# OPPOMKLab/u-LLaVA

Hardware: AMD Instinct MI355X
Metric: images/sec/GPU (ViT-L-336 + LLaMA-7B + SAM RES forward) at 1/2/4/8 MI355X (higher is better)
Workload: dtype bf16; 1 GPU; C4: ViT-L/14-336 + LLaMA-7B instruct forward, 336x336 image + 64-token prompt (S=643), batch 32/GPU; per_gpu_batch=32, global_batch=32, seq_len=643, image=336, parallelism=dp1, weights=random-init N(0,0.02), ViT-L/14 + LLaMA-7B (V=32011) shapes

## Files before the change

include/ullava_hip.h:

```cpp
#ifndef ULLAVA_HIP_H
#define ULLAVA_HIP_H
#include <stdint.h>
#ifdef __cplusplus
extern "C" {
#endif

#define ULL_DT_F32 0
#define ULL_DT_BF16 1
#define ULL_DT_F16 2

#define ULL_OK 0
#define ULL_ERR_ARG (-1)
#define ULL_ERR_SHAPE (-2)
#define ULL_ERR_LAUNCH (-3)
#define ULL_ERR_LDS (-4)

#define ULL_EPI_BIAS 1
#define ULL_EPI_ACT_QUICK_GELU (1 << 1)
#define ULL_EPI_ACT_GELU (2 << 1)
#define ULL_EPI_ACT_RELU (3 << 1)
#define ULL_EPI_RESID 8
#define ULL_EPI_SWIGLU 16
#define ULL_EPI_OUT_F32 32
#define ULL_EPI_W_TILED 64
#define ULL_EPI_X_TILED 128
#define ULL_EPI_BIAS_ROUNDED 256

#define ULL_GEMM_TUNE_GROUP_M(g) (((g) & 15) << 16)
#define ULL_GEMM_TUNE_SMALL_KERNEL (1 << 20)
#define ULL_GEMM_TUNE_WAVES8 (1 << 21)
#define ULL_GEMM_TUNE_WAVES4 (1 << 22)
#define ULL_GEMM_TUNE_STAGED_EPILOGUE 512
int ull_gemm_bf16(const void* X, int64_t ldx, const void* W, int64_t ldw, void* C, int64_t ldc, const void* bias, const void* R,
                  int64_t ldr, int64_t M, int64_t N, int64_t K, int flags, void* ws, int64_t ws_bytes, void* stream);

int ull_gemm_qkv_rope_bf16(const void* X, int64_t ldx, const void* W, int64_t ldw, void* C, int64_t ldc, int64_t M, int64_t N, int64_t K,
                           const void* rope_cos, const void* rope_sin, int64_t rope_cols, int64_t head_dim, int flags, void* ws,
                           int64_t ws_bytes, void* stream);

int ull_rope_table_bf16(const void* positions, const void* inv_freq, int64_t tokens, int64_t half, void* cos_out, void* sin_out,
                        void* stream);

int64_t ull_gemm_streamk_ws_bytes(void);

#define ULL_WF_ELEM 0
#define ULL_WF_FP8 1
#define ULL_WF_MXFP4 2

int ull_gemv_bf16(const void* X, int64_t ldx, const void* W, int64_t ldw, void* C, int64_t ldc, const void* bias, const void* R,
                  int64_t ldr, int64_t M, int64_t N, int64_t K, int flags, void* stream);

int ull_gemm_skinny_bf16(const void* X, int64_t ldx, const void* W, int64_t ldw, void* C, int64_t ldc, const void* bias, const void* R,
                         int64_t ldr, int64_t M, int64_t N, int64_t K, int flags, void* stream);

int ull_gemv_rmsnorm_bf16(const void* X, int64_t ldx, const void* norm_w, float eps, const void* W, int64_t ldw, void* C, int64_t ldc,
                          const void* bias, const void* R, int64_t ldr, int64_t M, int64_t N, int64_t K, int flags, void* stream);

int ull_gemv_qkv_rope_append_bf16(const void* X, int64_t ldx, const void* norm_w, float eps, const void* W, int64_t ldw, void* Q_out, int64_t ldq,
                                  const void* cos_tab, const void* sin_tab, void* k_cache, void* vt_cache, int64_t B, int64_t S, int64_t H,
                                  int64_t hd, int64_t K, int64_t smax, int64_t past, void* stream);

int ull_quantize_rows_fp8_bf16(const void* W, int64_t ldw, int64_t N, int64_t K, void* codes, void* scales, void* stream);
int ull_dequantize_rows_fp8_bf16(const void* codes, int64_t ldq, const void* scales, int64_t N, int64_t K, void* out, int tiled, void* stream);

int ull_quantize_rows_mxfp4_bf16(const void* W, int64_t ldw, int64_t N, int64_t K, void* codes, int64_t ldq, void* scales, int64_t lds, int resident,
                                 void* stream);
int ull_dequantize_rows_mxfp4_bf16(const void* codes, int64_t ldq, const void* scales, int64_t lds, int64_t N, int64_t K, void* out, int tiled,
                                   int resident, void* stream);

int ull_gemv_wq_bf16(const void* X, int64_t ldx, int wfmt, const void* Q, int64_t ldq, const void* scales, int64_t lds, void* C, int64_t ldc,
                     const void* bias, const void* R, int64_t ldr, int64_t M, int64_t N, int64_t K, int flags, void* stream);
int ull_gemm_skinny_wq_bf16(const void* X, int64_t ldx, int wfmt, const void* Q, int64_t ldq, const void* scales, int64_t lds, void* C, int64_t ldc,
                            const void* bias, const void* R, int64_t ldr, int64_t M, int64_t N, int64_t K, int flags, void* stream);
int ull_gemv_rmsnorm_wq_bf16(const void* X, int64_t ldx, const void* norm_w, float eps, int wfmt, const void* Q, int64_t ldq, const void* scales,
                             int64_t lds, void* C, int64_t ldc, const void* bias, const void* R, int64_t ldr, int64_t M, int64_t N, int64_t K,
                             int flags, void* stream);
int ull_gemv_qkv_rope_append_wq_bf16(const void* X, int64_t ldx, const void* norm_w, float eps, int wfmt, const void* Q, int64_t ldq,
                                     const void* scales, int64_t lds, void* Q_out, int64_t ldq_out, const void* cos_tab, const void* sin_tab,
                                     void* k_cache, void* vt_cache, int64_t B, int64_t S, int64_t H, int64_t hd, int64_t K, int64_t smax, int64_t past,
                                     void* stream);

int ull_gemm_a8w8_bf16(const void* Xq, int64_t ldxq, const void* x_scales, const void* Q, int64_t ldq, const void* w_scales, void* C, int64_t ldc,
                       const void* R, int64_t ldr, int64_t M, int64_t N, int64_t K, int flags, void* stream);

int ull_attention_kv8_bf16(const void* Q, int64_t q_bs, int64_t q_hs, int64_t q_ss, const void* k_stage, const void* vt_stage, const void* k8,
                           const void* vt8, const void* k_scale, const void* vt_scale, int64_t smax, void* O, int64_t o_bs, int64_t o_hs, int64_t o_ss,
                           const void* key_mask, int64_t B, int64_t H, int64_t Sq, int64_t Sk, int64_t hd, float scale, const void* zeros, void* stream);
int ull_kv8_quantize_bf16(const void* K, int64_t k_bs, int64_t k_hs, int64_t k_ss, const void* V, int64_t v_bs, int64_t v_hs, int64_t v_ss, int v_image,
                          int64_t src_p0, void* k8, void* vt8, void* k_scale, void* vt_scale, int64_t B, int64_t H, int64_t hd, int64_t smax, int64_t p0,
                          int64_t n, void* stream);
int ull_kv8_dequantize_bf16(const void* k8, const void* vt8, const void* k_scale, const void* vt_scale, int64_t B, int64_t H, int64_t hd, int64_t smax,
                            int64_t n, void* K_out, int64_t k_pitch, void* Vt_out, int64_t vt_pitch, void* stream);

int ull_rmsnorm_bf16(const void* x, int64_t ldx, const void* w, void* y, int64_t ldy, int64_t rows, int64_t D, float eps, void* stream);

int ull_shifted_cross_entropy_bf16(const void* logits, int64_t ld, const void* labels, int64_t B, int64_t S, int64_t V, void* out,
                                   void* stream);

int ull_layernorm_bf16(const void* x, int64_t ldx, const void* w, const void* b, void* y, int64_t ldy, int64_t rows, int64_t D, float eps,
                       void* stream);

int ull_clip_embed_ln_bf16(const void* patch, int64_t ldp, const void* cls, const void* pos, const void* w, const void* b, void* y,
                           int64_t ldy, int64_t n_img, int64_t tokens, int64_t D, float eps, void* stream);

int ull_attention_bf16(const void* Q, int64_t q_bs, int64_t q_hs, int64_t q_ss, const void* K, int64_t k_bs, int64_t k_hs, int64_t k_ss,
                       const void* Vt, int64_t vt_bs, int64_t vt_hs, int64_t vt_ds, int64_t vt_len, void* O, int64_t o_bs, int64_t o_hs,
                       int64_t o_ss, const void* key_mask, int64_t B, int64_t H, int64_t Sq, int64_t Sk, int64_t hd, int causal,
                       int scale_mode, float scale, float q_scale, const void* rel_h, const void* rel_w, int64_t rel_kh,
                       int64_t rel_kw, int rel_mode, const void* zeros, void* stream);

int ull_rope_inplace_bf16(void* x, int64_t row_stride, const void* positions, const void* inv_freq, int64_t tokens, int64_t n_heads,
                          int64_t hd, void* stream);

int ull_rope_append_bf16(void* qkv, int64_t row_stride, const void* positions, const void* inv_freq, int64_t B, int64_t S, int64_t H,
                         int64_t hd, void* k_cache, void* vt_cache, int64_t smax, int64_t past, void* stream);

int ull_transpose_v_bf16(const void* v, int64_t v_bs, int64_t v_ss, void* vt, int64_t B, int64_t S, int64_t H, int64_t hd, int64_t pitch,
                         void* stream);

int ull_im2col_bf16(const void* img, void* out, int64_t n_img, int64_t C, int64_t H, int64_t W, int64_t ps, int64_t Kp, void* stream);

int ull_mm_spans(const void* ids, int64_t B, int64_t S, int64_t img_start, int64_t img_end, int64_t vid_start, int64_t vid_end,
                 int64_t vocab, void* spans, void* stream);

int ull_greedy_step_bf16(const void* logits, int64_t row_stride, int64_t B, int64_t V, void* unfinished, const void* eos, int64_t n_eos,
                         int64_t pad, int has_pad, void* seq, int64_t seq_ld, int64_t pos, void* alive, void* stream);

#define ULL_SAMPLE_MAX_V 36608
int ull_sample_step(const void* logits, int logits_dtype, int64_t row_stride, int64_t B, int64_t V, const void* noise, float temperature,
                    int64_t top_k, float top_p, void* unfinished, const void* eos, int64_t n_eos, int64_t pad, int has_pad, void* seq,
                    int64_t seq_ld, int64_t pos, void* alive, void* stream);

int ull_embed_splice_bf16(const void* ids, const void* table, const void* img_feat, int64_t n_img_tok, int64_t img_pitch,
                          int64_t img_off, const void* vid_feat, int64_t n_vid_tok, const void* spans, void* out, int64_t B, int64_t S,
                          int64_t D, int64_t vocab, void* stream);

int ull_video_pool_bf16(const void* f, void* out, int64_t B, int64_t T, int64_t N, int64_t D, int64_t tok_pitch, int64_t tok_off,
                        void* stream);

int ull_gather_rows_bf16(const void* src, int64_t lds, const void* idx, void* dst, int64_t ldd, int64_t n, int64_t D, void* stream);

int ull_dropout_apply_bf16(const void* x, const void* keep, void* y, int64_t n, float scale, void* stream);

int ull_add_rows_bf16(const void* a, const void* b, void* out, int64_t rows, int64_t D, int64_t b_rows, void* stream);


int ull_window_partition_bf16(const void* x, void* out, int64_t B, int64_t H, int64_t W, int64_t C, int64_t ws, void* stream);

int ull_window_unpartition_add_bf16(const void* win, const void* shortcut, void* out, int64_t B, int64_t H, int64_t W, int64_t C, int64_t ws,
                                    void* stream);

int ull_sam_relpos_bf16(const void* q, int64_t q_bs, int64_t q_hs, int64_t q_ss, const void* rel_pos_h, const void* rel_pos_w, void* out_h,
                        void* out_w, int64_t NB, int64_t nH, int64_t KH, int64_t KW, int64_t hd, void* stream);

int ull_sam_window_attention_bf16(const void* qkv, int64_t ld, const void* pad_row, const void* rel_pos_h, const void* rel_pos_w, void* out,
                                  int64_t ldo, int64_t B, int64_t H, int64_t W, int64_t nH, int64_t hd, int64_t ws, float q_scale,
                                  const void* zeros, void* stream);

int ull_interp_rows_linear_bf16(const void* x, void* y, int64_t L, int64_t M, int64_t C, void* stream);

int ull_layernorm2d_cl_bf16(const void* x, const void* w, const void* b, void* y, int64_t rows, int64_t C, float eps, int gelu, void* stream);

int ull_neck_layernorm2d_f32in_f16(const void* xa, const void* xb, float xb_scale, const void* w, const void* b, void* y_hi, void* y_lo,
                                   int64_t rows, int64_t C, float eps, void* stream);

int ull_im2col3x3_bf16(const void* x, void* out, int64_t B, int64_t H, int64_t W, int64_t C, void* stream);

int ull_mask_matmul_bf16(const void* hyper, const void* up, void* masks, int64_t n, int64_t T, int64_t C, int64_t G, void* stream);

int ull_bilinear_f32(const void* in, int in_dtype, int64_t in_img_stride, int64_t in_row_stride, int64_t in_h, int64_t in_w, void* out,
                     int64_t n, int64_t out_h, int64_t out_w, void* stream);

int ull_patchify_bf16(const void* img, int64_t n_img, int64_t C, int64_t H, int64_t W, int64_t ps, const void* Wp, int64_t Kp,
                      const void* bias, void* out, int64_t ldc, int64_t N, const void* zeros, void* stream);


int ull_resample_u8(const void* src, int64_t H, int64_t W, int64_t C, int axis, int64_t out_size, const void* bounds, const void* coeffs,
                    int64_t ksize, void* dst, void* stream);

int ull_u8_lut_chw(const void* src, int64_t H, int64_t W, int64_t C, int64_t top, int64_t left, const void* lut, void* dst, int64_t OH,
                   int64_t OW, int64_t copy_h, int64_t copy_w, int out_dtype, void* stream);

int ull_mask_iou_counts(const void* logits, const void* target, int64_t n_masks, int64_t hw, int ignore_index, void* counts, void* stream);


int ull_mask_loss_sums_f32(const void* logits, const void* target, int64_t n_masks, int64_t hw, float scale, void* part, void* stream);

int ull_box_losses_f32(const void* pred, int pred_dtype, const void* gt, int64_t n, void* out, void* stream);


int ull_sam_self_attn_heads_bf16(const void* queries, const void* qpe, int64_t n, int64_t T, int first, const void* wq, const void* bq,
                                 const void* wk, const void* bk, const void* wv, const void* bv, void* att, void* stream);

int ull_sam_out_ln_bf16(const void* att, int64_t din, const void* res, const void* qpe, int64_t n, int64_t T, const void* wo, const void* bo,
                        const void* ln_w, const void* ln_b, float eps, void* out, const void* const* projs, const int* add_pe, void* stream);

int ull_sam_token_mlp_ln_bf16(const void* queries, const void* qpe, int64_t n, int64_t T, int64_t hidden, const void* w1, const void* b1,
                              const void* w2, const void* b2, const void* ln_w, const void* ln_b, float eps, void* part_ws, void* out,
                              const void* const* projs, const int* add_pe, void* stream);

int ull_sam_small_mlps_bf16(const void* hs, int64_t n, int64_t T, const void* const* ptrs, int64_t n_mask_tokens, int64_t hyper_out,
                            int64_t n_iou, void* hyper, void* iou, void* stream);

int ull_sam_t2i_attention_bf16(const void* qproj, const void* keys, const void* pos, int64_t n, int64_t T, int64_t P, const void* wk,
                               const void* bk, const void* wv, const void* bv, int late_bias_kv, void* scores_ws, void* vproj_ws, void* att,
                               void* stream);

int ull_sam_i2t_attention_ln_bf16(const void* keys, const void* pos, const void* kproj, const void* vproj, int64_t n, int64_t T, int64_t P,
                                  const void* wq, const void* bq, const void* wo, const void* bo, int late_bias_q, const void* ln_w,
                                  const void* ln_b, float eps, void* out, void* stream);


int ull_rmsnorm_bwd_bf16(const void* x, int64_t ldx, const void* w, const void* dy, int64_t lddy, void* dx, int64_t lddx, void* dw,
                         int64_t rows, int64_t D, float eps, void* stream);

int ull_swiglu_fwd_bf16(const void* gu, void* a, int64_t M, int64_t I, int halves, void* stream);
int ull_swiglu_bwd_bf16(const void* gu, const void* da, void* dgu, int64_t M, int64_t I, int halves, void* stream);

int ull_relu_mask_bf16(const void* y, const void* dy, void* dx, int64_t n, void* stream);

int ull_rope_bwd_inplace_bf16(void* dx, int64_t row_stride, const void* positions, const void* inv_freq, int64_t tokens, int64_t n_heads,
                              int64_t hd, void* stream);

int ull_attention_bwd_bf16(const void* Q, const void* K, const void* V, const void* O, const void* dO, void* dQ, void* dK, void* dV,
                           const int64_t* strides, const void* key_mask, int64_t B, int64_t H, int64_t Sq, int64_t Sk, int64_t hd, int causal,
                           float mult, void* scratch, void* stream);

int ull_attention_bwd_mfma_bf16(const void* Q, const void* K, const void* V, const void* O, const void* dO, const void* Qt, const void* Kt,
                                const void* dOt, int64_t pitch, void* dQ, void* dK, void* dV, const int64_t* strides, const void* key_mask,
                                int64_t B, int64_t H, int64_t Sq, int64_t Sk, int64_t hd, int causal, float mult, void* scratch, void* stream);

int ull_shifted_cross_entropy_bwd_bf16(const void* logits, int64_t ld, const void* labels, int64_t B, int64_t S, int64_t V, const void* stats,
                                       const void* gout, void* dlogits, void* stream);

int ull_embed_splice_bwd_bf16(const void* ids, const void* demb, void* d_table, void* d_img, int64_t n_img_tok, int64_t img_pitch,
                              int64_t img_off, void* d_vid, int64_t n_vid_tok, const void* spans, int64_t B, int64_t S, int64_t D, int64_t vocab,
                              int detach_text, void* stream);

int ull_layernorm_bwd_bf16(const void* x, int64_t ldx, const void* w, const void* dy, int64_t lddy, void* dx, int64_t lddx, void* dw, void* db,
                           int64_t rows, int64_t D, float eps, void* stream);

int ull_layernorm2d_cl_bwd_bf16(const void* x, const void* w, const void* b, const void* dy, void* dx, void* dw, void* db, int64_t rows,
                                int64_t C, float eps, int gelu, void* stream);

int ull_gelu_fwd_bf16(const void* x, void* y, int64_t n, void* stream);
int ull_gelu_bwd_bf16(const void* x, const void* dy, void* dx, int64_t n, void* stream);

int ull_mask_matmul_bwd_bf16(const void* hyper, const void* up, const void* dmasks, void* dhyper, void* dup, int64_t n, int64_t T, int64_t C,
                             int64_t G, void* stream);

int ull_sum_slabs_bf16(const void* x, void* out, int64_t R, int64_t n, float scale, void* stream);

int ull_colsum_bf16(const void* x, int64_t ld, int64_t rows, int64_t N, void* out, void* stream);

int ull_transpose2d_bf16(const void* x, int64_t ldx, void* y, int64_t ldy, int64_t R, int64_t C, void* stream);

int ull_mask_loss_sums_bwd_f32(const void* logits, const void* target, const void* g, int64_t n_masks, int64_t hw, float scale, void* dlogits,
                               void* stream);
int ull_box_losses_bwd_f32(const void* pred, int pred_dtype, const void* gt, int64_t n, const void* gw, void* dpred, void* stream);
int ull_bilinear_bwd_f32(const void* dout, void* din, int64_t in_img_stride, int64_t in_row_stride, int64_t in_h, int64_t in_w, int64_t n,
                         int64_t out_h, int64_t out_w, void* stream);

int ull_adamw_step_f32(void* master, void* m, void* v, const void* grad, int grad_dtype, void* param_out, int param_dtype, int64_t n, float lr,
                       float beta1, float beta2, float eps, float weight_decay, int64_t step, float grad_scale, void* stream);

int ull_sumsq_f32(const void* g, int grad_dtype, int64_t n, void* out, void* stream);

typedef struct ull_linear {
    const void* w;
    const void* w_tiled;
    const void* bias;
    int64_t n, k, ldw;
    int format;
    const void* scales;
    int64_t lds;
} ull_linear;
typedef struct ull_llama_layer {
    const void* ln1;
    const void* ln2;
    ull_linear qkv, o, gu, down;
} ull_llama_layer;
typedef struct ull_clip_layer {
    const void *ln1_w, *ln1_b, *ln2_w, *ln2_b;
    ull_linear qkv, out, fc1, fc2;
} ull_clip_layer;
typedef struct ull_sam_block {
    const void *n1_w, *n1_b, *n2_w, *n2_b;
    ull_linear qkv, proj, lin1, lin2;
    const void* rel_pos_h;
    const void* rel_pos_w;
    int64_t window;
} ull_sam_block;

int ull_llama_prefill_layers_bf16(const ull_llama_layer* layers, int64_t n_layers, const void* x_in, void* const* x_out, void* x_mid, void* xn,
                                  void* qkv, void* att, void* act, const void* rope_cos, const void* rope_sin, const void* key_mask, int64_t B,
                                  int64_t S, int64_t H, int64_t hd, int64_t I, float eps, void* ws, int64_t ws_bytes, int64_t sk_min_k,
                                  const void* zeros, void* stream);

int ull_llama_decode_layers_bf16(const ull_llama_layer* layers, int64_t n_layers, const void* x_in, void* const* x_out, void* x_mid, void* xn,
                                 void* q, void* att, void* act, const void* rope_cos, const void* rope_sin, const void* key_mask,
                                 void* const* k_cache, void* const* vt_cache, int64_t B, int64_t S, int64_t H, int64_t hd, int64_t I, int64_t smax,
                                 int64_t past, float eps, const void* zeros, void* stream);

int ull_llama_decode_layers_kv8_bf16(const ull_llama_layer* layers, int64_t n_layers, const void* x_in, void* const* x_out, void* x_mid, void* xn,
                                     void* q, void* att, void* act, const void* rope_cos, const void* rope_sin, const void* key_mask, void* const* k8,
                                     void* const* vt8, void* const* k_scale, void* const* vt_scale, void* k_stage, void* vt_stage, int64_t B, int64_t S,
                                     int64_t H, int64_t hd, int64_t I, int64_t smax, int64_t past, float eps, const void* zeros, void* stream);

int ull_clip_layers_bf16(const ull_clip_layer* layers, int64_t n_layers, void* h, void* h_mid, void* y, void* qkv, void* att, void* f, int64_t n_img,
                         int64_t S, int64_t H, int64_t hd, int64_t I, float eps, void* ws, int64_t ws_bytes, int64_t sk_min_k, const void* zeros,
                         void* stream);

int ull_sam_blocks_bf16(const ull_sam_block* blocks, int64_t n_blocks, void* x, void* x_mid, void* y, void* qkv, void* att, void* f, int64_t B,
                        int64_t g, int64_t nH, int64_t hd, int64_t I, float eps, void* ws, int64_t ws_bytes, int64_t sk_min_k, const void* zeros,
                        void* stream);

int ull_gemm_f32(const void* X, int64_t ldx, const void* W, int64_t ldw, void* C, int64_t ldc, const void* bias, const void* R, int64_t ldr, int64_t M, int64_t N, int64_t K, int flags, void* ws, int64_t ws_bytes, void* stream);
int ull_attention_f32(const void* Q, int64_t q_bs, int64_t q_hs, int64_t q_ss, const void* K, int64_t k_bs, int64_t k_hs, int64_t k_ss, const void* Vt, int64_t vt_bs, int64_t vt_hs, int64_t vt_ds, int64_t vt_len, void* O, int64_t o_bs, int64_t o_hs, int64_t o_ss, const void* key_mask, int64_t B, int64_t H, int64_t Sq, int64_t Sk, int64_t hd, int causal, int scale_mode, float scale, float q_scale, const void* rel_h, const void* rel_w, int64_t rel_kh, int64_t rel_kw, int rel_mode, const void* zeros, void* stream);
int ull_transpose_v_f32(const void* v, int64_t v_bs, int64_t v_ss, void* vt, int64_t B, int64_t S, int64_t H, int64_t hd, int64_t pitch, void* stream);
int ull_transpose2d_f32(const void* x, int64_t ldx, void* y, int64_t ldy, int64_t R, int64_t C, void* stream);
int ull_rmsnorm_f32(const void* x, int64_t ldx, const void* w, void* y, int64_t ldy, int64_t rows, int64_t D, float eps, void* stream);
int ull_layernorm_f32(const void* x, int64_t ldx, const void* w, const void* b, void* y, int64_t ldy, int64_t rows, int64_t D, float eps, void* stream);
int ull_clip_embed_ln_f32(const void* patch, int64_t ldp, const void* cls, const void* pos, const void* w, const void* b, void* y, int64_t ldy, int64_t n_img, int64_t tokens, int64_t D, float eps, void* stream);
int ull_layernorm2d_cl_f32(const void* x, const void* w, const void* b, void* y, int64_t rows, int64_t C, float eps, int gelu, void* stream);
int ull_rope_inplace_f32(void* x, int64_t row_stride, const void* positions, const void* inv_freq, int64_t tokens, int64_t n_heads, int64_t hd, void* stream);
int ull_rope_append_f32(void* qkv, int64_t row_stride, const void* positions, const void* inv_freq, int64_t B, int64_t S, int64_t H, int64_t hd, void* k_cache, void* vt_cache, int64_t smax, int64_t past, void* stream);
int ull_im2col_f32(const void* img, void* out, int64_t n_img, int64_t C, int64_t H, int64_t W, int64_t ps, int64_t Kp, void* stream);
int ull_im2col3x3_f32(const void* x, void* out, int64_t B, int64_t H, int64_t W, int64_t C, void* stream);
int ull_video_pool_f32(const void* f, void* out, int64_t B, int64_t T, int64_t N, int64_t D, int64_t tok_pitch, int64_t tok_off, void* stream);
int ull_add_rows_f32(const void* a, const void* b, void* out, int64_t rows, int64_t D, int64_t b_rows, void* stream);
int ull_window_unpartition_add_f32(const void* win, const void* shortcut, void* out, int64_t B, int64_t H, int64_t W, int64_t C, int64_t ws, void* stream);
int ull_sam_relpos_f32(const void* q, int64_t q_bs, int64_t q_hs, int64_t q_ss, const void* rel_pos_h, const void* rel_pos_w, void* out_h, void* out_w, int64_t NB, int64_t nH, int64_t KH, int64_t KW, int64_t hd, void* stream);
int ull_interp_rows_linear_f32(const void* x, void* y, int64_t L, int64_t M, int64_t C, void* stream);
int ull_mask_matmul_f32(const void* hyper, const void* up, void* masks, int64_t n, int64_t T, int64_t C, int64_t G, void* stream);
int ull_greedy_step_f32(const void* logits, int64_t row_stride, int64_t B, int64_t V, void* unfinished, const void* eos, int64_t n_eos, int64_t pad, int has_pad, void* seq, int64_t seq_ld, int64_t pos, void* alive, void* stream);
int ull_shifted_cross_entropy_f32(const void* logits, int64_t ld, const void* labels, int64_t B, int64_t S, int64_t V, void* out, void* stream);

int ull_gemm_f16(const void* X, int64_t ldx, const void* W, int64_t ldw, void* C, int64_t ldc, const void* bias, const void* R, int64_t ldr, int64_t M, int64_t N, int64_t K, int flags, void* ws, int64_t ws_bytes, void* stream);
int ull_gemm_qkv_rope_f16(const void* X, int64_t ldx, const void* W, int64_t ldw, void* C, int64_t ldc, int64_t M, int64_t N, int64_t K, const void* rope_cos, const void* rope_sin, int64_t rope_cols, int64_t head_dim, int flags, void* ws, int64_t ws_bytes, void* stream);
int ull_rope_table_f16(const void* positions, const void* inv_freq, int64_t tokens, int64_t half, void* cos_out, void* sin_out, void* stream);
int ull_gemv_f16(const void* X, int64_t ldx, const void* W, int64_t ldw, void* C, int64_t ldc, const void* bias, const void* R, int64_t ldr, int64_t M, int64_t N, int64_t K, int flags, void* stream);
int ull_gemm_skinny_f16(const void* X, int64_t ldx, const void* W, int64_t ldw, void* C, int64_t ldc, const void* bias, const void* R, int64_t ldr, int64_t M, int64_t N, int64_t K, int flags, void* stream);
int ull_gemv_rmsnorm_f16(const void* X, int64_t ldx, const void* norm_w, float eps, const void* W, int64_t ldw, void* C, int64_t ldc, const void* bias, const void* R, int64_t ldr, int64_t M, int64_t N, int64_t K, int flags, void* stream);
int ull_gemv_qkv_rope_append_f16(const void* X, int64_t ldx, const void* norm_w, float eps, const void* W, int64_t ldw, void* Q_out, int64_t ldq, const void* cos_tab, const void* sin_tab, void* k_cache, void* vt_cache, int64_t B, int64_t S, int64_t H, int64_t hd, int64_t K, int64_t smax, int64_t past, void* stream);
int ull_rmsnorm_f16(const void* x, int64_t ldx, const void* w, void* y, int64_t ldy, int64_t rows, int64_t D, float eps, void* stream);
int ull_shifted_cross_entropy_f16(const void* logits, int64_t ld, const void* labels, int64_t B, int64_t S, int64_t V, void* out, void* stream);
int ull_layernorm_f16(const void* x, int64_t ldx, const void* w, const void* b, void* y, int64_t ldy, int64_t rows, int64_t D, float eps, void* stream);
int ull_clip_embed_ln_f16(const void* patch, int64_t ldp, const void* cls, const void* pos, const void* w, const void* b, void* y, int64_t ldy, int64_t n_img, int64_t tokens, int64_t D, float eps, void* stream);
int ull_attention_f16(const void* Q, int64_t q_bs, int64_t q_hs, int64_t q_ss, const void* K, int64_t k_bs, int64_t k_hs, int64_t k_ss, const void* Vt, int64_t vt_bs, int64_t vt_hs, int64_t vt_ds, int64_t vt_len, void* O, int64_t o_bs, int64_t o_hs, int64_t o_ss, const void* key_mask, int64_t B, int64_t H, int64_t Sq, int64_t Sk, int64_t hd, int causal, int scale_mode, float scale, float q_scale, const void* rel_h, const void* rel_w, int64_t rel_kh, int64_t rel_kw, int rel_mode, const void* zeros, void* stream);
int ull_rope_inplace_f16(void* x, int64_t row_stride, const void* positions, const void* inv_freq, int64_t tokens, int64_t n_heads, int64_t hd, void* stream);
int ull_rope_append_f16(void* qkv, int64_t row_stride, const void* positions, const void* inv_freq, int64_t B, int64_t S, int64_t H, int64_t hd, void* k_cache, void* vt_cache, int64_t smax, int64_t past, void* stream);
int ull_transpose_v_f16(const void* v, int64_t v_bs, int64_t v_ss, void* vt, int64_t B, int64_t S, int64_t H, int64_t hd, int64_t pitch, void* stream);
int ull_im2col_f16(const void* img, void* out, int64_t n_img, int64_t C, int64_t H, int64_t W, int64_t ps, int64_t Kp, void* stream);
int ull_greedy_step_f16(const void* logits, int64_t row_stride, int64_t B, int64_t V, void* unfinished, const void* eos, int64_t n_eos, int64_t pad, int has_pad, void* seq, int64_t seq_ld, int64_t pos, void* alive, void* stream);
int ull_embed_splice_f16(const void* ids, const void* table, const void* img_feat, int64_t n_img_tok, int64_t img_pitch, int64_t img_off, const void* vid_feat, int64_t n_vid_tok, const void* spans, void* out, int64_t B, int64_t S, int64_t D, int64_t vocab, void* stream);
int ull_video_pool_f16(const void* f, void* out, int64_t B, int64_t T, int64_t N, int64_t D, int64_t tok_pitch, int64_t tok_off, void* stream);
int ull_gather_rows_f16(const void* src, int64_t lds, const void* idx, void* dst, int64_t ldd, int64_t n, int64_t D, void* stream);
int ull_dropout_apply_f16(const void* x, const void* keep, void* y, int64_t n, float scale, void* stream);
int ull_add_rows_f16(const void* a, const void* b, void* out, int64_t rows, int64_t D, int64_t b_rows, void* stream);
int ull_window_partition_f16(const void* x, void* out, int64_t B, int64_t H, int64_t W, int64_t C, int64_t ws, void* stream);
int ull_window_unpartition_add_f16(const void* win, const void* shortcut, void* out, int64_t B, int64_t H, int64_t W, int64_t C, int64_t ws, void* stream);
int ull_sam_relpos_f16(const void* q, int64_t q_bs, int64_t q_hs, int64_t q_ss, const void* rel_pos_h, const void* rel_pos_w, void* out_h, void* out_w, int64_t NB, int64_t nH, int64_t KH, int64_t KW, int64_t hd, void* stream);
int ull_sam_window_attention_f16(const void* qkv, int64_t ld, const void* pad_row, const void* rel_pos_h, const void* rel_pos_w, void* out, int64_t ldo, int64_t B, int64_t H, int64_t W, int64_t nH, int64_t hd, int64_t ws, float q_scale, const void* zeros, void* stream);
int ull_interp_rows_linear_f16(const void* x, void* y, int64_t L, int64_t M, int64_t C, void* stream);
int ull_layernorm2d_cl_f16(const void* x, const void* w, const void* b, void* y, int64_t rows, int64_t C, float eps, int gelu, void* stream);
int ull_im2col3x3_f16(const void* x, void* out, int64_t B, int64_t H, int64_t W, int64_t C, void* stream);
int ull_mask_matmul_f16(const void* hyper, const void* up, void* masks, int64_t n, int64_t T, int64_t C, int64_t G, void* stream);
int ull_patchify_f16(const void* img, int64_t n_img, int64_t C, int64_t H, int64_t W, int64_t ps, const void* Wp, int64_t Kp, const void* bias, void* out, int64_t ldc, int64_t N, const void* zeros, void* stream);
int ull_sam_self_attn_heads_f16(const void* queries, const void* qpe, int64_t n, int64_t T, int first, const void* wq, const void* bq, const void* wk, const void* bk, const void* wv, const void* bv, void* att, void* stream);
int ull_sam_out_ln_f16(const void* att, int64_t din, const void* res, const void* qpe, int64_t n, int64_t T, const void* wo, const void* bo, const void* ln_w, const void* ln_b, float eps, void* out, const void* const* projs, const int* add_pe, void* stream);
int ull_sam_token_mlp_ln_f16(const void* queries, const void* qpe, int64_t n, int64_t T, int64_t hidden, const void* w1, const void* b1, const void* w2, const void* b2, const void* ln_w, const void* ln_b, float eps, void* part_ws, void* out, const void* const* projs, const int* add_pe, void* stream);
int ull_sam_small_mlps_f16(const void* hs, int64_t n, int64_t T, const void* const* ptrs, int64_t n_mask_tokens, int64_t hyper_out, int64_t n_iou, void* hyper, void* iou, void* stream);
int ull_sam_t2i_attention_f16(const void* qproj, const void* keys, const void* pos, int64_t n, int64_t T, int64_t P, const void* wk, const void* bk, const void* wv, const void* bv, int late_bias_kv, void* scores_ws, void* vproj_ws, void* att, void* stream);
int ull_sam_i2t_attention_ln_f16(const void* keys, const void* pos, const void* kproj, const void* vproj, int64_t n, int64_t T, int64_t P, const void* wq, const void* bq, const void* wo, const void* bo, int late_bias_q, const void* ln_w, const void* ln_b, float eps, void* out, void* stream);
int ull_rmsnorm_bwd_f16(const void* x, int64_t ldx, const void* w, const void* dy, int64_t lddy, void* dx, int64_t lddx, void* dw, int64_t rows, int64_t D, float eps, void* stream);
int ull_swiglu_fwd_f16(const void* gu, void* a, int64_t M, int64_t I, int halves, void* stream);
int ull_swiglu_bwd_f16(const void* gu, const void* da, void* dgu, int64_t M, int64_t I, int halves, void* stream);
int ull_relu_mask_f16(const void* y, const void* dy, void* dx, int64_t n, void* stream);
int ull_rope_bwd_inplace_f16(void* dx, int64_t row_stride, const void* positions, const void* inv_freq, int64_t tokens, int64_t n_heads, int64_t hd, void* stream);
int ull_attention_bwd_f16(const void* Q, const void* K, const void* V, const void* O, const void* dO, void* dQ, void* dK, void* dV, const int64_t* strides, const void* key_mask, int64_t B, int64_t H, int64_t Sq, int64_t Sk, int64_t hd, int causal, float mult, void* scratch, void* stream);
int ull_attention_bwd_mfma_f16(const void* Q, const void* K, const void* V, const void* O, const void* dO, const void* Qt, const void* Kt, const void* dOt, int64_t pitch, void* dQ, void* dK, void* dV, const int64_t* strides, const void* key_mask, int64_t B, int64_t H, int64_t Sq, int64_t Sk, int64_t hd, int causal, float mult, void* scratch, void* stream);
int ull_shifted_cross_entropy_bwd_f16(const void* logits, int64_t ld, const void* labels, int64_t B, int64_t S, int64_t V, const void* stats, const void* gout, void* dlogits, void* stream);
int ull_embed_splice_bwd_f16(const void* ids, const void* demb, void* d_table, void* d_img, int64_t n_img_tok, int64_t img_pitch, int64_t img_off, void* d_vid, int64_t n_vid_tok, const void* spans, int64_t B, int64_t S, int64_t D, int64_t vocab, int detach_text, void* stream);
int ull_layernorm_bwd_f16(const void* x, int64_t ldx, const void* w, const void* dy, int64_t lddy, void* dx, int64_t lddx, void* dw, void* db, int64_t rows, int64_t D, float eps, void* stream);
int ull_layernorm2d_cl_bwd_f16(const void* x, const void* w, const void* b, const void* dy, void* dx, void* dw, void* db, int64_t rows, int64_t C, float eps, int gelu, void* stream);
int ull_gelu_fwd_f16(const void* x, void* y, int64_t n, void* stream);
int ull_gelu_bwd_f16(const void* x, const void* dy, void* dx, int64_t n, void* stream);
int ull_mask_matmul_bwd_f16(const void* hyper, const void* up, const void* dmasks, void* dhyper, void* dup, int64_t n, int64_t T, int64_t C, int64_t G, void* stream);
int ull_sum_slabs_f16(const void* x, void* out, int64_t R, int64_t n, float scale, void* stream);
int ull_colsum_f16(const void* x, int64_t ld, int64_t rows, int64_t N, void* out, void* stream);
int ull_transpose2d_f16(const void* x, int64_t ldx, void* y, int64_t ldy, int64_t R, int64_t C, void* stream);
int ull_llama_prefill_layers_f16(const ull_llama_layer* layers, int64_t n_layers, const void* x_in, void* const* x_out, void* x_mid, void* xn, void* qkv, void* att, void* act, const void* rope_cos, const void* rope_sin, const void* key_mask, int64_t B, int64_t S, int64_t H, int64_t hd, int64_t I, float eps, void* ws, int64_t ws_bytes, int64_t sk_min_k, const void* zeros, void* stream);
int ull_llama_decode_layers_f16(const ull_llama_layer* layers, int64_t n_layers, const void* x_in, void* const* x_out, void* x_mid, void* xn, void* q, void* att, void* act, const void* rope_cos, const void* rope_sin, const void* key_mask, void* const* k_cache, void* const* vt_cache, int64_t B, int64_t S, int64_t H, int64_t hd, int64_t I, int64_t smax, int64_t past, float eps, const void* zeros, void* stream);
int ull_clip_layers_f16(const ull_clip_layer* layers, int64_t n_layers, void* h, void* h_mid, void* y, void* qkv, void* att, void* f, int64_t n_img, int64_t S, int64_t H, int64_t hd, int64_t I, float eps, void* ws, int64_t ws_bytes, int64_t sk_min_k, const void* zeros, void* stream);
int ull_sam_blocks_f16(const ull_sam_block* blocks, int64_t n_blocks, void* x, void* x_mid, void* y, void* qkv, void* att, void* f, int64_t B, int64_t g, int64_t nH, int64_t hd, int64_t I, float eps, void* ws, int64_t ws_bytes, int64_t sk_min_k, const void* zeros, void* stream);

#ifdef __cplusplus
}
#endif
#endif
```

u-llava_amd/_lib.py:

```python
import ctypes
import os

_HERE = os.path.dirname(os.path.abspath(__file__))
LIB_PATH = os.environ.get("ULL_LIB_PATH", os.path.join(_HERE, "csrc", "libullava_hip.so"))

_i64, _i32, _f32, _ptr = ctypes.c_int64, ctypes.c_int, ctypes.c_float, ctypes.c_void_p


WF_ELEM, WF_FP8, WF_MXFP4 = 0, 1, 2


class Linear(ctypes.Structure):
    _fields_ = [("w", _ptr), ("w_tiled", _ptr), ("bias", _ptr), ("n", _i64), ("k", _i64), ("ldw", _i64), ("format", _i32), ("scales", _ptr), ("lds", _i64)]


class LlamaLayer(ctypes.Structure):
    _fields_ = [("ln1", _ptr), ("ln2", _ptr), ("qkv", Linear), ("o", Linear), ("gu", Linear), ("down", Linear)]


class ClipLayer(ctypes.Structure):
    _fields_ = [("ln1_w", _ptr), ("ln1_b", _ptr), ("ln2_w", _ptr), ("ln2_b", _ptr), ("qkv", Linear), ("out", Linear), ("fc1", Linear), ("fc2", Linear)]


class SamBlock(ctypes.Structure):
    _fields_ = [("n1_w", _ptr), ("n1_b", _ptr), ("n2_w", _ptr), ("n2_b", _ptr), ("qkv", Linear), ("proj", Linear), ("lin1", Linear), ("lin2", Linear),
                ("rel_pos_h", _ptr), ("rel_pos_w", _ptr), ("window", _i64)]


SIGNATURES = {
    "ull_gemm_bf16": [_ptr, _i64, _ptr, _i64, _ptr, _i64, _ptr, _ptr, _i64, _i64, _i64, _i64, _i32, _ptr, _i64, _ptr],
    "ull_gemm_streamk_ws_bytes": [],
    "ull_gemm_qkv_rope_bf16": [_ptr, _i64, _ptr, _i64, _ptr, _i64, _i64, _i64, _i64, _ptr, _ptr, _i64, _i64, _i32, _ptr, _i64, _ptr],
    "ull_rope_table_bf16": [_ptr, _ptr, _i64, _i64, _ptr, _ptr, _ptr],
    "ull_sam_self_attn_heads_bf16": [_ptr, _ptr, _i64, _i64, _i32] + [_ptr] * 7 + [_ptr],
    "ull_sam_out_ln_bf16": [_ptr, _i64, _ptr, _ptr, _i64, _i64, _ptr, _ptr, _ptr, _ptr, _f32, _ptr, ctypes.POINTER(_ptr), ctypes.POINTER(_i32), _ptr],
    "ull_sam_token_mlp_ln_bf16": [_ptr, _ptr, _i64, _i64, _i64] + [_ptr] * 6 + [_f32, _ptr, _ptr, ctypes.POINTER(_ptr), ctypes.POINTER(_i32), _ptr],
    "ull_sam_small_mlps_bf16": [_ptr, _i64, _i64, ctypes.POINTER(_ptr), _i64, _i64, _i64, _ptr, _ptr, _ptr],
    "ull_sam_t2i_attention_bf16": [_ptr, _ptr, _ptr, _i64, _i64, _i64, _ptr, _ptr, _ptr, _ptr, _i32, _ptr, _ptr, _ptr, _ptr],
    "ull_sam_i2t_attention_ln_bf16": [_ptr] * 4 + [_i64] * 3 + [_ptr] * 4 + [_i32, _ptr, _ptr, _f32, _ptr, _ptr],
    "ull_rmsnorm_bwd_bf16": [_ptr, _i64, _ptr, _ptr, _i64, _ptr, _i64, _ptr, _i64, _i64, _f32, _ptr],
    "ull_swiglu_fwd_bf16": [_ptr, _ptr, _i64, _i64, _i32, _ptr],
    "ull_swiglu_bwd_bf16": [_ptr, _ptr, _ptr, _i64, _i64, _i32, _ptr],
    "ull_relu_mask_bf16": [_ptr, _ptr, _ptr, _i64, _ptr],
    "ull_rope_bwd_inplace_bf16": [_ptr, _i64, _ptr, _ptr, _i64, _i64, _i64, _ptr],
    "ull_attention_bwd_bf16": [_ptr, _ptr, _ptr, _ptr, _ptr, _ptr, _ptr, _ptr, ctypes.POINTER(_i64), _ptr, _i64, _i64, _i64, _i64, _i64, _i32,
                               _f32, _ptr, _ptr],
    "ull_attention_bwd_mfma_bf16": [_ptr, _ptr, _ptr, _ptr, _ptr, _ptr, _ptr, _ptr, _i64, _ptr, _ptr, _ptr, ctypes.POINTER(_i64), _ptr, _i64, _i64,
                                    _i64, _i64, _i64, _i32, _f32, _ptr, _ptr],
    "ull_shifted_cross_entropy_bwd_bf16": [_ptr, _i64, _ptr, _i64, _i64, _i64, _ptr, _ptr, _ptr, _ptr],
    "ull_embed_splice_bwd_bf16": [_ptr, _ptr, _ptr, _ptr, _i64, _i64, _i64, _ptr, _i64, _ptr, _i64, _i64, _i64, _i64, _i32, _ptr],
    "ull_colsum_bf16": [_ptr, _i64, _i64, _i64, _ptr, _ptr],
    "ull_transpose2d_bf16": [_ptr, _i64, _ptr, _i64, _i64, _i64, _ptr],
    "ull_sum_slabs_bf16": [_ptr, _ptr, _i64, _i64, _f32, _ptr],
    "ull_layernorm_bwd_bf16": [_ptr, _i64, _ptr, _ptr, _i64, _ptr, _i64, _ptr, _ptr, _i64, _i64, _f32, _ptr],
    "ull_layernorm2d_cl_bwd_bf16": [_ptr, _ptr, _ptr, _ptr, _ptr, _ptr, _ptr, _i64, _i64, _f32, _i32, _ptr],
    "ull_gelu_fwd_bf16": [_ptr, _ptr, _i64, _ptr],
    "ull_gelu_bwd_bf16": [_ptr, _ptr, _ptr, _i64, _ptr],
    "ull_mask_matmul_bwd_bf16": [_ptr, _ptr, _ptr, _ptr, _ptr, _i64, _i64, _i64, _i64, _ptr],
    "ull_mask_loss_sums_bwd_f32": [_ptr, _ptr, _ptr, _i64, _i64, _f32, _ptr, _ptr],
    "ull_box_losses_bwd_f32": [_ptr, _i32, _ptr, _i64, _ptr, _ptr, _ptr],
    "ull_bilinear_bwd_f32": [_ptr, _ptr, _i64, _i64, _i64, _i64, _i64, _i64, _i64, _ptr],
    "ull_gemv_bf16": [_ptr, _i64, _ptr, _i64, _ptr, _i64, _ptr, _ptr, _i64, _i64, _i64, _i64, _i32, _ptr],
    "ull_dropout_apply_bf16": [_ptr, _ptr, _ptr, _i64, _f32, _ptr],
    "ull_gemm_skinny_bf16": [_ptr, _i64, _ptr, _i64, _ptr, _i64, _ptr, _ptr, _i64, _i64, _i64, _i64, _i32, _ptr],
    "ull_gemv_rmsnorm_bf16": [_ptr, _i64, _ptr, _f32, _ptr, _i64, _ptr, _i64, _ptr, _ptr, _i64, _i64, _i64, _i64, _i32, _ptr],
    "ull_gemv_qkv_rope_append_bf16": [_ptr, _i64, _ptr, _f32, _ptr, _i64, _ptr, _i64, _ptr, _ptr, _ptr, _ptr, _i64, _i64, _i64, _i64, _i64, _i64, _i64,
                                      _ptr],
    "ull_rmsnorm_bf16": [_ptr, _i64, _ptr, _ptr, _i64, _i64, _i64, _f32, _ptr],
    "ull_llama_prefill_layers_bf16": [_ptr, _i64, _ptr, _ptr, _ptr, _ptr, _ptr, _ptr, _ptr, _ptr, _ptr, _ptr, _i64, _i64, _i64, _i64, _i64, _f32, _ptr,
                                      _i64, _i64, _ptr, _ptr],
    "ull_llama_decode_layers_bf16": [_ptr, _i64, _ptr, _ptr, _ptr, _ptr, _ptr, _ptr, _ptr, _ptr, _ptr, _ptr, _ptr, _ptr, _i64, _i64, _i64, _i64, _i64,
                                     _i64, _i64, _f32, _ptr, _ptr],
    "ull_clip_layers_bf16": [_ptr, _i64, _ptr, _ptr, _ptr, _ptr, _ptr, _ptr, _i64, _i64, _i64, _i64, _i64, _f32, _ptr, _i64, _i64, _ptr, _ptr],
    "ull_sam_blocks_bf16": [_ptr, _i64, _ptr, _ptr, _ptr, _ptr, _ptr, _ptr, _i64, _i64, _i64, _i64, _i64, _f32, _ptr, _i64, _i64, _ptr, _ptr],
    "ull_shifted_cross_entropy_bf16": [_ptr, _i64, _ptr, _i64, _i64, _i64, _ptr, _ptr],
    "ull_layernorm_bf16": [_ptr, _i64, _ptr, _ptr, _ptr, _i64, _i64, _i64, _f32, _ptr],
    "ull_clip_embed_ln_bf16": [_ptr, _i64, _ptr, _ptr, _ptr, _ptr, _ptr, _i64, _i64, _i64, _i64, _f32, _ptr],
    "ull_attention_bf16": [_ptr, _i64, _i64, _i64, _ptr, _i64, _i64, _i64, _ptr, _i64, _i64, _i64, _i64, _ptr, _i64, _i64, _i64,
                           _ptr, _i64, _i64, _i64, _i64, _i64, _i32, _i32, _f32, _f32, _ptr, _ptr, _i64, _i64, _i32, _ptr, _ptr],
    "ull_rope_inplace_bf16": [_ptr, _i64, _ptr, _ptr, _i64, _i64, _i64, _ptr],
    "ull_rope_append_bf16": [_ptr, _i64, _ptr, _ptr, _i64, _i64, _i64, _i64, _ptr, _ptr, _i64, _i64, _ptr],
    "ull_transpose_v_bf16": [_ptr, _i64, _i64, _ptr, _i64, _i64, _i64, _i64, _i64, _ptr],
    "ull_sam_window_attention_bf16": [_ptr, _i64, _ptr, _ptr, _ptr, _ptr, _i64, _i64, _i64, _i64, _i64, _i64, _i64, _f32, _ptr, _ptr],
    "ull_interp_rows_linear_bf16": [_ptr, _ptr, _i64, _i64, _i64, _ptr],
    "ull_im2col_bf16": [_ptr, _ptr, _i64, _i64, _i64, _i64, _i64, _i64, _ptr],
    "ull_mm_spans": [_ptr, _i64, _i64, _i64, _i64, _i64, _i64, _i64, _ptr, _ptr],
    "ull_greedy_step_bf16": [_ptr, _i64, _i64, _i64, _ptr, _ptr, _i64, _i64, _i32, _ptr, _i64, _i64, _ptr, _ptr],
    "ull_embed_splice_bf16": [_ptr, _ptr, _ptr, _i64, _i64, _i64, _ptr, _i64, _ptr, _ptr, _i64, _i64, _i64, _i64, _ptr],
    "ull_video_pool_bf16": [_ptr, _ptr, _i64, _i64, _i64, _i64, _i64, _i64, _ptr],
    "ull_gather_rows_bf16": [_ptr, _i64, _ptr, _ptr, _i64, _i64, _i64, _ptr],
    "ull_add_rows_bf16": [_ptr, _ptr, _ptr, _i64, _i64, _i64, _ptr],
    "ull_window_partition_bf16": [_ptr, _ptr, _i64, _i64, _i64, _i64, _i64, _ptr],
    "ull_window_unpartition_add_bf16": [_ptr, _ptr, _ptr, _i64, _i64, _i64, _i64, _i64, _ptr],
    "ull_sam_relpos_bf16": [_ptr, _i64, _i64, _i64, _ptr, _ptr, _ptr, _ptr, _i64, _i64, _i64, _i64, _i64, _ptr],
    "ull_layernorm2d_cl_bf16": [_ptr, _ptr, _ptr, _ptr, _i64, _i64, _f32, _i32, _ptr],
    "ull_im2col3x3_bf16": [_ptr, _ptr, _i64, _i64, _i64, _i64, _ptr],
    "ull_mask_matmul_bf16": [_ptr, _ptr, _ptr, _i64, _i64, _i64, _i64, _ptr],
    "ull_bilinear_f32": [_ptr, _i32, _i64, _i64, _i64, _i64, _ptr, _i64, _i64, _i64, _ptr],
    "ull_patchify_bf16": [_ptr, _i64, _i64, _i64, _i64, _i64, _ptr, _i64, _ptr, _ptr, _i64, _i64, _ptr, _ptr],
    "ull_resample_u8": [_ptr, _i64, _i64, _i64, _i32, _i64, _ptr, _ptr, _i64, _ptr, _ptr],
    "ull_u8_lut_chw": [_ptr, _i64, _i64, _i64, _i64, _i64, _ptr, _ptr, _i64, _i64, _i64, _i64, _i32, _ptr],
    "ull_mask_iou_counts": [_ptr, _ptr, _i64, _i64, _i32, _ptr, _ptr],
    "ull_mask_loss_sums_f32": [_ptr, _ptr, _i64, _i64, _f32, _ptr, _ptr],
    "ull_box_losses_f32": [_ptr, _i32, _ptr, _i64, _ptr, _ptr],
    "ull_adamw_step_f32": [_ptr, _ptr, _ptr, _ptr, _i32, _ptr, _i32, _i64, _f32, _f32, _f32, _f32, _f32, _i64, _f32, _ptr],
    "ull_sumsq_f32": [_ptr, _i32, _i64, _ptr, _ptr],
    "ull_sample_step": [_ptr, _i32, _i64, _i64, _i64, _ptr, _f32, _i64, _f32, _ptr, _ptr, _i64, _i64, _i32, _ptr, _i64, _i64, _ptr, _ptr],
}

SIGNATURES.update({name[:-4] + "f16": args for name, args in list(SIGNATURES.items()) if name.endswith("_bf16")})

F32_TWINS = ['ull_gemm', 'ull_attention', 'ull_transpose_v', 'ull_transpose2d', 'ull_rmsnorm', 'ull_layernorm', 'ull_clip_embed_ln', 'ull_layernorm2d_cl', 'ull_rope_inplace', 'ull_rope_append', 'ull_im2col', 'ull_im2col3x3', 'ull_video_pool', 'ull_add_rows', 'ull_window_unpartition_add', 'ull_sam_relpos', 'ull_interp_rows_linear', 'ull_mask_matmul', 'ull_greedy_step', 'ull_shifted_cross_entropy']
SIGNATURES.update({name + "_f32": SIGNATURES[name + "_bf16"] for name in F32_TWINS})

SIGNATURES.update({
    "ull_quantize_rows_fp8_bf16": [_ptr, _i64, _i64, _i64, _ptr, _ptr, _ptr],
    "ull_dequantize_rows_fp8_bf16": [_ptr, _i64, _ptr, _i64, _i64, _ptr, _i32, _ptr],
    "ull_attention_kv8_bf16": [_ptr, _i64, _i64, _i64, _ptr, _ptr, _ptr, _ptr, _ptr, _ptr, _i64, _ptr, _i64, _i64, _i64, _ptr, _i64, _i64, _i64, _i64,
                               _i64, _f32, _ptr, _ptr],
    "ull_kv8_quantize_bf16": [_ptr, _i64, _i64, _i64, _ptr, _i64, _i64, _i64, _i32, _i64, _ptr, _ptr, _ptr, _ptr, _i64, _i64, _i64, _i64, _i64, _i64, _ptr],
    "ull_kv8_dequantize_bf16": [_ptr, _ptr, _ptr, _ptr, _i64, _i64, _i64, _i64, _i64, _ptr, _i64, _ptr, _i64, _ptr],
    "ull_llama_decode_layers_kv8_bf16": [_ptr, _i64] + [_ptr] * 16 + [_i64] * 7 + [_f32, _ptr, _ptr],
})

SIGNATURES.update({
    "ull_quantize_rows_mxfp4_bf16": [_ptr, _i64, _i64, _i64, _ptr, _i64, _ptr, _i64, _i32, _ptr],
    "ull_dequantize_rows_mxfp4_bf16": [_ptr, _i64, _ptr, _i64, _i64, _i64, _ptr, _i32, _i32, _ptr],
    "ull_gemv_wq_bf16": [_ptr, _i64, _i32, _ptr, _i64, _ptr, _i64, _ptr, _i64, _ptr, _ptr, _i64, _i64, _i64, _i64, _i32, _ptr],
    "ull_gemm_skinny_wq_bf16": [_ptr, _i64, _i32, _ptr, _i64, _ptr, _i64, _ptr, _i64, _ptr, _ptr, _i64, _i64, _i64, _i64, _i32, _ptr],
    "ull_gemv_rmsnorm_wq_bf16": [_ptr, _i64, _ptr, _f32, _i32, _ptr, _i64, _ptr, _i64, _ptr, _i64, _ptr, _ptr, _i64, _i64, _i64, _i64, _i32, _ptr],
    "ull_gemv_qkv_rope_append_wq_bf16": [_ptr, _i64, _ptr, _f32, _i32, _ptr, _i64, _ptr, _i64, _ptr, _i64, _ptr, _ptr, _ptr, _ptr, _i64, _i64, _i64, _i64,
                                         _i64, _i64, _i64, _ptr],
})

SIGNATURES["ull_gemm_a8w8_bf16"] = [_ptr, _i64, _ptr, _ptr, _i64, _ptr, _ptr, _i64, _ptr, _i64, _i64, _i64, _i64, _i32, _ptr]

SIGNATURES["ull_neck_layernorm2d_f32in_f16"] = [_ptr, _ptr, _f32, _ptr, _ptr, _ptr, _ptr, _i64, _i64, _f32, _ptr]

VALUE_RETURNING = {"ull_gemm_streamk_ws_bytes": _i64}

ERRORS = {-1: "ULL_ERR_ARG (null pointer / bad size)", -2: "ULL_ERR_SHAPE (alignment or shape constraint)",
          -3: "ULL_ERR_LAUNCH (HIP launch failed)", -4: "ULL_ERR_LDS (does not fit the LDS budget)"}

_lib = None


def load():
    global _lib
    if _lib is not None:
        return _lib
    if not os.path.exists(LIB_PATH):
        raise RuntimeError(
            f"u-llava_amd: HIP library not built: {LIB_PATH} is missing. Run `python -c 'import __graft_entry__ as g; g.build()'` "
            "or `make -C u-llava_amd/csrc`. There is no CPU fallback.")
    lib = ctypes.CDLL(LIB_PATH)
    for name, argtypes in SIGNATURES.items():
        fn = getattr(lib, name)
        fn.argtypes = argtypes
        fn.restype = VALUE_RETURNING.get(name, ctypes.c_int)
    _lib = lib
    return lib


def call(name: str, *args):
    fn = getattr(load(), name, None)
    if fn is None or name not in SIGNATURES:
        raise RuntimeError(f"u-llava_amd: the library has no entry point `{name}` (no kernel build of this op for that element type)")
    rc = fn(*args)
    if rc != 0:
        raise RuntimeError(f"u-llava_amd: {name} failed: {ERRORS.get(rc, rc)}")


def query(name: str, *args):
    fn = getattr(load(), name, None)
    if fn is None or name not in SIGNATURES:
        raise RuntimeError(f"u-llava_amd: the library has no entry point `{name}` (no kernel build of this op for that element type)")
    return fn(*args)
```

u-llava_amd/csrc/f32.hip:

```cpp
#include "ull_common.h"

#define ULL_EPI_BIAS 1
#define ULL_EPI_ACT_MASK (3 << 1)
#define ULL_EPI_ACT_QUICK_GELU (1 << 1)
#define ULL_EPI_ACT_GELU (2 << 1)
#define ULL_EPI_ACT_RELU (3 << 1)
#define ULL_EPI_RESID 8
#define ULL_EPI_SWIGLU 16
#define ULL_EPI_W_TILED 64
#define ULL_EPI_X_TILED 128

namespace {

ULL_DEV float gelu_erf32(float x) { return 0.5f * x * (1.0f + erff(x * 0.70710678118654752440f)); }
ULL_DEV float sigmoid32(float x) { return 1.0f / (1.0f + expf(-x)); }
static inline unsigned grid_for(long n, long cap = 65535) { const long b = (n + 255) / 256; return (unsigned)(b < 1 ? 1 : (b < cap ? b : cap)); }

__global__ __launch_bounds__(256) void gemm_f32_kernel(const float* __restrict__ X, long ldx, const float* __restrict__ W, long ldw, float* __restrict__ C,
                                                       long ldc, const float* __restrict__ bias, const float* __restrict__ R, long ldr, int M, int N,
                                                       int K, int flags) {
    __shared__ float Xs[64][17], Ws[64][17];
    const int tid = threadIdx.x, lane = tid & 63, wave = tid >> 6;
    const long m0 = (long)blockIdx.y * 64, n0 = (long)blockIdx.x * 64;
    const int lr = tid >> 2, lk = (tid & 3) * 4;
    f32x4_t acc[4];
#pragma unroll
    for (int j = 0; j < 4; ++j) acc[j] = f32x4_t{0.f, 0.f, 0.f, 0.f};
    for (int k0 = 0; k0 < K; k0 += 16) {
#pragma unroll
        for (int j = 0; j < 4; ++j) {
            const int k = k0 + lk + j;
            Xs[lr][lk + j] = (m0 + lr < M && k < K) ? X[(m0 + lr) * ldx + k] : 0.f;
            Ws[lr][lk + j] = (n0 + lr < N && k < K) ? W[(n0 + lr) * ldw + k] : 0.f;
        }
        __syncthreads();
#pragma unroll
        for (int kk = 0; kk < 4; ++kk) {
            const float a = Xs[wave * 16 + (lane & 15)][kk * 4 + (lane >> 4)];
#pragma unroll
            for (int j = 0; j < 4; ++j) acc[j] = __builtin_amdgcn_mfma_f32_16x16x4f32(a, Ws[j * 16 + (lane & 15)][kk * 4 + (lane >> 4)], acc[j], 0, 0, 0);
        }
        __syncthreads();
    }
    const int act = flags & ULL_EPI_ACT_MASK;
    if (flags & ULL_EPI_SWIGLU) {
#pragma unroll
        for (int pr = 0; pr < 2; ++pr) {
            const long oc = (n0 / 32 + pr) * 16 + (lane & 15);
            if (n0 + pr * 32 + 16 + (lane & 15) >= N) continue;
#pragma unroll
            for (int i = 0; i < 4; ++i) {
                const long m = m0 + wave * 16 + 4 * (lane >> 4) + i;
                if (m >= M) continue;
                const float g = acc[2 * pr][i], u = acc[2 * pr + 1][i];
                float v = (g * sigmoid32(g)) * u;
                if (R) v = R[m * ldr + oc] + v;
                C[m * ldc + oc] = v;
            }
        }
        return;
    }
#pragma unroll
    for (int j = 0; j < 4; ++j) {
        const long n = n0 + j * 16 + (lane & 15);
        if (n >= N) continue;
        const float bv = (flags & ULL_EPI_BIAS) ? bias[n] : 0.f;
#pragma unroll
        for (int i = 0; i < 4; ++i) {
            const long m = m0 + wave * 16 + 4 * (lane >> 4) + i;
            if (m >= M) continue;
            float v = acc[j][i] + bv;
            if (act == ULL_EPI_ACT_QUICK_GELU) v = v * sigmoid32(1.702f * v);
            else if (act == ULL_EPI_ACT_GELU) v = gelu_erf32(v);
            else if (act == ULL_EPI_ACT_RELU) v = fmaxf(v, 0.f);
            if (flags & ULL_EPI_RESID) v = R[m * ldr + n] + v;
            C[m * ldc + n] = v;
        }
    }
}

struct AttnF32 {
    const float *Q, *K, *V;
    float* O;
    const int32_t* key_mask;
    const float *rel_h, *rel_w;
    long q_bs, q_hs, q_ss, k_bs, k_hs, k_ss, v_bs, v_hs, v_ds, v_len, o_bs, o_hs, o_ss;
    int B, H, Sq, Sk, hd, causal, scale_mode, KH, KW;
    float scale, q_scale;
};

ULL_DEV long vt_slot(long key) {
    const int w = (int)(key & 31);
    return (key & ~31L) + 8 * ((w >> 2) & 3) + 4 * (w >> 4) + (w & 3);
}

__global__ __launch_bounds__(256) void attn_f32_kernel(AttnF32 p) {
    constexpr int HDP = 128;
    __shared__ float Qs[16][HDP + 1], KVs[64][HDP + 1], Ss[16][65], alpha[16], rowm[16], rowl[16];
    const int tid = threadIdx.x, lane = tid & 63, wave = tid >> 6;
    const int q0 = blockIdx.x * 16;
    const int b = blockIdx.y / p.H, h = blockIdx.y % p.H;
    const int hd = p.hd, hd4 = (hd + 3) / 4, ndb = (hd + 15) / 16;
    const int koff = p.Sk - p.Sq;
    const float* qb = p.Q + (long)b * p.q_bs + (long)h * p.q_hs;
    const float* kb = p.K + (long)b * p.k_bs + (long)h * p.k_hs;
    const float* vb = p.V + (long)b * p.v_bs + (long)h * p.v_hs;
    for (int i = tid; i < 16 * HDP; i += 256) {
        const int r = i / HDP, d = i % HDP;
        const int q = min(q0 + r, p.Sq - 1);
        Qs[r][d] = d < hd ? qb[(long)q * p.q_ss + d] * p.q_scale : 0.f;
    }
    if (tid < 16) { rowm[tid] = -INFINITY; rowl[tid] = 0.f; }
    f32x4_t acc[2] = {f32x4_t{0.f, 0.f, 0.f, 0.f}, f32x4_t{0.f, 0.f, 0.f, 0.f}};
    int kend = p.Sk;
    if (p.causal) kend = max(1, min(p.Sk, q0 + 16 + koff));
    __syncthreads();
    for (int k0 = 0; k0 < kend; k0 += 64) {
        for (int i = tid; i < 64 * HDP; i += 256) {
            const int r = i / HDP, d = i % HDP;
            KVs[r][d] = (k0 + r < p.Sk && d < hd) ? kb[(long)(k0 + r) * p.k_ss + d] : 0.f;
        }
        __syncthreads();
        {
            f32x4_t s = {0.f, 0.f, 0.f, 0.f};
            for (int k4 = 0; k4 < hd4; ++k4)
                s = __builtin_amdgcn_mfma_f32_16x16x4f32(Qs[lane & 15][k4 * 4 + (lane >> 4)], KVs[wave * 16 + (lane & 15)][k4 * 4 + (lane >> 4)], s, 0, 0, 0);
            const int kl = wave * 16 + (lane & 15), key = k0 + kl;
#pragma unroll
            for (int i = 0; i < 4; ++i) {
                const int r = 4 * (lane >> 4) + i, q = min(q0 + r, p.Sq - 1);
                float v = s[i];
                if (p.scale_mode == 1) v *= p.scale;
                else if (p.scale_mode == 2) v /= p.scale;
                if (key >= p.Sk) v = -INFINITY;
                else {
                    if (p.rel_h) {
                        const long row = ((long)b * p.H + h) * p.Sq + q;
                        v = (v + p.rel_h[row * p.KH + key / p.KW]) + p.rel_w[row * p.KW + key % p.KW];
                    }
                    if ((p.causal && key > q + koff) || (p.key_mask && p.key_mask[(long)b * p.Sk + key] == 0)) v = -3.4028234663852886e38f;
                }
                Ss[r][kl] = v;
            }
        }
        __syncthreads();
        {
            const int r = tid >> 4, c = tid & 15;
            const float s0 = Ss[r][c], s1 = Ss[r][c + 16], s2 = Ss[r][c + 32], s3 = Ss[r][c + 48];
            const float mo = rowm[r];
            const float mn = fmaxf(mo, group_max(fmaxf(fmaxf(s0, s1), fmaxf(s2, s3)), 16));
            const float e0 = expf(s0 - mn), e1 = expf(s1 - mn), e2 = expf(s2 - mn), e3 = expf(s3 - mn);
            Ss[r][c] = e0; Ss[r][c + 16] = e1; Ss[r][c + 32] = e2; Ss[r][c + 48] = e3;
            const float sum = group_sum((e0 + e1) + (e2 + e3), 16);
            if (c == 0) {
                const float al = expf(mo - mn);
                alpha[r] = al;
                rowm[r] = mn;
                rowl[r] = rowl[r] * al + sum;
            }
        }
        for (int i = tid; i < 64 * HDP; i += 256) {
            const int r = i / HDP, d = i % HDP;
            float v = 0.f;
// ... 187 lines not shown
}

__global__ __launch_bounds__(256) void add_rows_f32_kernel(const float* __restrict__ a, const float* __restrict__ b, float* __restrict__ out, long rows,
                                                           int D, long b_rows) {
    const long total = rows * D;
    for (long i = (long)blockIdx.x * 256 + threadIdx.x; i < total; i += (long)gridDim.x * 256) out[i] = a[i] + b[((i / D) % b_rows) * D + i % D];
}

__global__ __launch_bounds__(256) void window_unpartition_add_f32_kernel(const float* __restrict__ win, const float* __restrict__ shortcut,
                                                                         float* __restrict__ out, int H, int W, int C, int ws, int nWh, int nWw, long total) {
    for (long i = (long)blockIdx.x * 256 + threadIdx.x; i < total; i += (long)gridDim.x * 256) {
        const int c = (int)(i % C);
        const long row = i / C;
        const int xx = (int)(row % W), y = (int)((row / W) % H);
        const long b = row / ((long)W * H);
        const long wrow = ((b * nWh + y / ws) * nWw + xx / ws) * (long)(ws * ws) + (y % ws) * ws + xx % ws;
        out[i] = shortcut[i] + win[wrow * C + c];
    }
}

__global__ __launch_bounds__(128) void relpos_f32_kernel(const float* __restrict__ q, long q_bs, long q_hs, long q_ss, const float* __restrict__ rph,
                                                         const float* __restrict__ rpw, float* __restrict__ out_h, float* __restrict__ out_w, int nH, int KH,
                                                         int KW, int hd) {
    __shared__ float qs[256];
    const int S = KH * KW;
    const long blk = blockIdx.x;
    const int s = (int)(blk % S);
    const long bh = blk / S;
    const float* qp = q + (bh / nH) * q_bs + (bh % nH) * q_hs + (long)s * q_ss;
    for (int c = threadIdx.x; c < hd; c += 128) qs[c] = qp[c];
    __syncthreads();
    const int qy = s / KW, qx = s % KW;
    for (int t = threadIdx.x; t < KH + KW; t += 128) {
        const float* r = (t < KH) ? rph + (long)(qy - t + KH - 1) * hd : rpw + (long)(qx - (t - KH) + KW - 1) * hd;
        float acc = 0.f;
        for (int c = 0; c < hd; ++c) acc += qs[c] * r[c];
        if (t < KH) out_h[(bh * S + s) * KH + t] = acc;
        else out_w[(bh * S + s) * KW + (t - KH)] = acc;
    }
}

__global__ __launch_bounds__(256) void interp_rows_f32_kernel(const float* __restrict__ x, float* __restrict__ y, int L, int M, int C) {
    const long i = (long)blockIdx.x * 256 + threadIdx.x;
    if (i >= (long)M * C) return;
    const int m = (int)(i / C), c = (int)(i % C);
    float src = __fsub_rn(__fmul_rn((float)L / (float)M, (float)m + 0.5f), 0.5f);
    if (src < 0.f) src = 0.f;
    const int i0 = min((int)src, L - 1), i1 = min(i0 + 1, L - 1);
    const float l1 = __fsub_rn(src, (float)i0), l0 = __fsub_rn(1.0f, l1);
    y[i] = __fadd_rn(__fmul_rn(l0, x[(long)i0 * C + c]), __fmul_rn(l1, x[(long)i1 * C + c]));
}

__global__ __launch_bounds__(256) void mask_matmul_f32_kernel(const float* __restrict__ hyper, const float* __restrict__ up, float* __restrict__ masks, int T,
                                                              int Cc, int G, long total) {
    for (long i = (long)blockIdx.x * 256 + threadIdx.x; i < total; i += (long)gridDim.x * 256) {
        const int d2 = (int)(i & 3), d1 = (int)((i >> 2) & 3);
        const long cell = i >> 4;
        const int xx = (int)(cell % G), y = (int)((cell / G) % G);
        const long n = cell / ((long)G * G);
        const float* u = up + i * Cc;
        const int Y = 4 * y + 2 * (d1 >> 1) + (d2 >> 1), X = 4 * xx + 2 * (d1 & 1) + (d2 & 1);
        const int HW = 4 * G;
        for (int t = 0; t < T; ++t) {
            const float* hp = hyper + (n * T + t) * Cc;
            float acc = 0.f;
            for (int c = 0; c < Cc; ++c) acc += hp[c] * u[c];
            masks[((n * T + t) * HW + Y) * (long)HW + X] = acc;
        }
    }
}

__global__ __launch_bounds__(1024) void greedy_step_f32_kernel(const float* __restrict__ logits, long row_stride, int V, int32_t* __restrict__ unfinished,
                                                               const int64_t* __restrict__ eos, int n_eos, long pad, int has_pad, int64_t* __restrict__ seq,
                                                               long seq_ld, int pos, int32_t* __restrict__ alive) {
    __shared__ float bv[16];
    __shared__ int bi[16];
    const int b = blockIdx.x;
    const float* row = logits + (long)b * row_stride;
    float best = -INFINITY;
    int idx = 0x7fffffff;
    for (int c = threadIdx.x; c < V; c += 1024) {
        const float v = row[c];
        if (v > best || (v == best && c < idx)) { best = v; idx = c; }
    }
    if (idx == 0x7fffffff) idx = threadIdx.x < V ? threadIdx.x : 0;
#pragma unroll
    for (int o = 32; o > 0; o >>= 1) {
        const float ov = __shfl_xor(best, o, 64);
        const int oi = __shfl_xor(idx, o, 64);
        if (ov > best || (ov == best && oi < idx)) { best = ov; idx = oi; }
    }
    if ((threadIdx.x & 63) == 0) { bv[threadIdx.x >> 6] = best; bi[threadIdx.x >> 6] = idx; }
    __syncthreads();
    if (threadIdx.x == 0) {
        for (int w = 1; w < 16; ++w)
            if (bv[w] > best || (bv[w] == best && bi[w] < idx)) { best = bv[w]; idx = bi[w]; }
        const int live = unfinished[b];
        long tok = idx;
        if (!live && has_pad) tok = pad;
        seq[(long)b * seq_ld + pos] = tok;
        int still = live;
        if (live)
            for (int e = 0; e < n_eos; ++e)
                if (eos[e] == tok) still = 0;
        unfinished[b] = still;
        if (still) atomicAdd(alive, 1);
    }
}

__global__ __launch_bounds__(256) void shifted_ce_f32_kernel(const float* __restrict__ logits, long ld, const int64_t* __restrict__ labels, int B, int S, int V,
                                                             float* __restrict__ out) {
    const int lane = threadIdx.x & 63;
    const long row = (long)blockIdx.x * 4 + (threadIdx.x >> 6);
    if (row >= (long)B * (S - 1)) return;
    const int b = (int)(row / (S - 1)), t = (int)(row % (S - 1));
    const int64_t lab = labels[(long)b * S + t + 1];
    if (lab < 0 || lab >= V) return;
    const float* lp = logits + ((long)b * S + t) * ld;
    float m = -INFINITY;
    for (int i = lane; i < V; i += 64) m = fmaxf(m, lp[i]);
    m = wave_max(m);
    float s = 0.f;
    for (int i = lane; i < V; i += 64) s += expf(lp[i] - m);
    s = wave_sum(s);
    if (lane == 0) {
        atomicAdd(out, m + logf(s) - lp[lab]);
        atomicAdd(out + 1, 1.0f);
    }
}

__global__ __launch_bounds__(256) void transpose2d_f32_kernel(const float* __restrict__ x, long ldx, float* __restrict__ y, long ldy, int R, int C) {
    __shared__ float t[64][65];
    const int r0 = blockIdx.y * 64, c0 = blockIdx.x * 64;
    for (int i = threadIdx.x; i < 64 * 64; i += 256) {
        const int r = i >> 6, c = i & 63;
        if (r0 + r < R && c0 + c < C) t[c][r] = x[(long)(r0 + r) * ldx + c0 + c];
    }
    __syncthreads();
    for (int i = threadIdx.x; i < 64 * 64; i += 256) {
        const int c = i >> 6, r = i & 63;
        if (r0 + r < R && c0 + c < C) y[(long)(c0 + c) * ldy + r0 + r] = t[c][r];
    }
}

}

#define ST ((hipStream_t)stream)

extern "C" int ull_gemm_f32(const void* X, int64_t ldx, const void* W, int64_t ldw, void* C, int64_t ldc, const void* bias, const void* R, int64_t ldr,
                            int64_t M, int64_t N, int64_t K, int flags, void* ws, int64_t ws_bytes, void* stream) {
    (void)ws; (void)ws_bytes;
    if (!X || !W || !C || M <= 0 || N <= 0 || K <= 0) return ULL_ERR_ARG;
    if (((flags & ULL_EPI_BIAS) && !bias) || ((flags & ULL_EPI_RESID) && !R)) return ULL_ERR_ARG;
    if (flags & (ULL_EPI_W_TILED | ULL_EPI_X_TILED)) return ULL_ERR_SHAPE;
    if ((flags & ULL_EPI_SWIGLU) && (N % 32)) return ULL_ERR_SHAPE;
    hipLaunchKernelGGL(gemm_f32_kernel, dim3((unsigned)((N + 63) / 64), (unsigned)((M + 63) / 64)), dim3(256), 0, ST, (const float*)X, (long)ldx,
                       (const float*)W, (long)ldw, (float*)C, (long)ldc, (const float*)bias, (flags & ULL_EPI_RESID) ? (const float*)R : nullptr, (long)ldr,
                       (int)M, (int)N, (int)K, flags);
    return ull_check_launch();
}

extern "C" int ull_attention_f32(const void* Q, int64_t q_bs, int64_t q_hs, int64_t q_ss, const void* K, int64_t k_bs, int64_t k_hs, int64_t k_ss,
                                 const void* Vt, int64_t vt_bs, int64_t vt_hs, int64_t vt_ds, int64_t vt_len, void* O, int64_t o_bs, int64_t o_hs,
                                 int64_t o_ss, const void* key_mask, int64_t B, int64_t H, int64_t Sq, int64_t Sk, int64_t hd, int causal, int scale_mode,
                                 float scale, float q_scale, const void* rel_h, const void* rel_w, int64_t rel_kh, int64_t rel_kw, int rel_mode,
                                 const void* zeros, void* stream) {
    (void)zeros;
    if (!Q || !K || !Vt || !O || B <= 0 || H <= 0 || Sq <= 0 || Sk <= 0 || hd <= 0) return ULL_ERR_ARG;
    if (hd > 128 || (rel_h && rel_mode != 1) || (rel_h && (!rel_w || rel_kh * rel_kw != Sk))) return ULL_ERR_SHAPE;
    AttnF32 p;
    p.Q = (const float*)Q; p.K = (const float*)K; p.V = (const float*)Vt; p.O = (float*)O;
    p.key_mask = (const int32_t*)key_mask;
    p.rel_h = (const float*)rel_h; p.rel_w = (const float*)rel_w;
    p.q_bs = q_bs; p.q_hs = q_hs; p.q_ss = q_ss; p.k_bs = k_bs; p.k_hs = k_hs; p.k_ss = k_ss;
    p.v_bs = vt_bs; p.v_hs = vt_hs; p.v_ds = vt_ds; p.v_len = vt_len; p.o_bs = o_bs; p.o_hs = o_hs; p.o_ss = o_ss;
    p.B = (int)B; p.H = (int)H; p.Sq = (int)Sq; p.Sk = (int)Sk; p.hd = (int)hd; p.causal = causal; p.scale_mode = scale_mode;
    p.KH = (int)rel_kh; p.KW = (int)(rel_kw > 0 ? rel_kw : 1);
    p.scale = scale; p.q_scale = q_scale;
    hipLaunchKernelGGL(attn_f32_kernel, dim3((unsigned)((Sq + 15) / 16), (unsigned)(B * H)), dim3(256), 0, ST, p);
    return ull_check_launch();
}

extern "C" int ull_transpose_v_f32(const void* v, int64_t v_bs, int64_t v_ss, void* vt, int64_t B, int64_t S, int64_t H, int64_t hd, int64_t pitch,
                                   void* stream) {
    if (!v || !vt || B <= 0 || S <= 0 || H <= 0 || hd <= 0) return ULL_ERR_ARG;
    if (pitch % 64 || pitch < S) return ULL_ERR_SHAPE;
    const long total = B * H * hd * pitch;
    hipLaunchKernelGGL(transpose_v_f32_kernel, dim3(grid_for(total)), dim3(256), 0, ST, (const float*)v, (long)v_bs, (long)v_ss, (float*)vt, (int)S, (int)H,
                       (int)hd, (int)pitch, total);
    return ull_check_launch();
}

extern "C" int ull_transpose2d_f32(const void* x, int64_t ldx, void* y, int64_t ldy, int64_t R, int64_t C, void* stream) {
    if (!x || !y || R <= 0 || C <= 0 || ldx < C || ldy < R) return ULL_ERR_ARG;
    if (R > 65535 * 64 || C > (1 << 30)) return ULL_ERR_SHAPE;
    hipLaunchKernelGGL(transpose2d_f32_kernel, dim3((unsigned)((C + 63) / 64), (unsigned)((R + 63) / 64)), dim3(256), 0, ST, (const float*)x, (long)ldx,
                       (float*)y, (long)ldy, (int)R, (int)C);
    return ull_check_launch();
}

extern "C" int ull_rmsnorm_f32(const void* x, int64_t ldx, const void* w, void* y, int64_t ldy, int64_t rows, int64_t D, float eps, void* stream) {
    if (!x || !w || !y || rows <= 0 || D <= 0) return ULL_ERR_ARG;
    hipLaunchKernelGGL((rownorm_f32_kernel<0>), dim3((unsigned)((rows + 3) / 4)), dim3(256), 0, ST, (const float*)x, (long)ldx, (const float*)w, nullptr,
                       (float*)y, (long)ldy, (long)rows, (int)D, eps, nullptr, nullptr, 0);
    return ull_check_launch();
}

extern "C" int ull_layernorm_f32(const void* x, int64_t ldx, const void* w, const void* b, void* y, int64_t ldy, int64_t rows, int64_t D, float eps,
                                 void* stream) {
    if (!x || !w || !b || !y || rows <= 0 || D <= 0) return ULL_ERR_ARG;
    hipLaunchKernelGGL((rownorm_f32_kernel<1>), dim3((unsigned)((rows + 3) / 4)), dim3(256), 0, ST, (const float*)x, (long)ldx, (const float*)w,
                       (const float*)b, (float*)y, (long)ldy, (long)rows, (int)D, eps, nullptr, nullptr, 0);
    return ull_check_launch();
}

extern "C" int ull_clip_embed_ln_f32(const void* patch, int64_t ldp, const void* cls, const void* pos, const void* w, const void* b, void* y, int64_t ldy,
                                     int64_t n_img, int64_t tokens, int64_t D, float eps, void* stream) {
    if (!patch || !cls || !pos || !w || !b || !y || tokens < 2 || n_img <= 0) return ULL_ERR_ARG;
    const long rows = n_img * tokens;
    hipLaunchKernelGGL((rownorm_f32_kernel<1>), dim3((unsigned)((rows + 3) / 4)), dim3(256), 0, ST, (const float*)patch, (long)ldp, (const float*)w,
                       (const float*)b, (float*)y, (long)ldy, rows, (int)D, eps, (const float*)cls, (const float*)pos, (int)tokens);
    return ull_check_launch();
}

extern "C" int ull_layernorm2d_cl_f32(const void* x, const void* w, const void* b, void* y, int64_t rows, int64_t C, float eps, int gelu, void* stream) {
    if (!x || !w || !b || !y || rows <= 0 || C <= 0) return ULL_ERR_ARG;
    hipLaunchKernelGGL(layernorm2d_f32_kernel, dim3((unsigned)((rows + 3) / 4)), dim3(256), 0, ST, (const float*)x, (const float*)w, (const float*)b,
                       (float*)y, (long)rows, (int)C, eps, gelu);
    return ull_check_launch();
}

extern "C" int ull_rope_inplace_f32(void* x, int64_t row_stride, const void* positions, const void* inv_freq, int64_t tokens, int64_t n_heads, int64_t hd,
                                    void* stream) {
    if (!x || !positions || !inv_freq || tokens <= 0 || n_heads <= 0) return ULL_ERR_ARG;
    if (hd & 1) return ULL_ERR_SHAPE;
    hipLaunchKernelGGL(rope_inplace_f32_kernel, dim3((unsigned)tokens), dim3(256), 0, ST, (float*)x, (long)row_stride, (const int64_t*)positions,
                       (const float*)inv_freq, (int)n_heads, (int)hd);
    return ull_check_launch();
}

extern "C" int ull_rope_append_f32(void* qkv, int64_t row_stride, const void* positions, const void* inv_freq, int64_t B, int64_t S, int64_t H, int64_t hd,
                                   void* k_cache, void* vt_cache, int64_t smax, int64_t past, void* stream) {
    if (!qkv || !positions || !inv_freq || !k_cache || !vt_cache || B <= 0 || S <= 0 || H <= 0) return ULL_ERR_ARG;
    if ((hd & 1) || past + S > smax) return ULL_ERR_SHAPE;
    hipLaunchKernelGGL(rope_append_f32_kernel, dim3((unsigned)(B * S), (unsigned)H), dim3(128), 0, ST, (float*)qkv, (long)row_stride,
                       (const int64_t*)positions, (const float*)inv_freq, (int)S, (int)H, (int)hd, (float*)k_cache, (float*)vt_cache, (int)smax, (int)past);
    return ull_check_launch();
}

extern "C" int ull_im2col_f32(const void* img, void* out, int64_t n_img, int64_t C, int64_t H, int64_t W, int64_t ps, int64_t Kp, void* stream) {
    if (!img || !out || n_img <= 0 || ps <= 0) return ULL_ERR_ARG;
    if (H % ps || W % ps || Kp < C * ps * ps) return ULL_ERR_SHAPE;
    const int gh = (int)(H / ps), gw = (int)(W / ps);
    const long total = n_img * gh * gw * Kp;
    hipLaunchKernelGGL(im2col_f32_kernel, dim3(grid_for(total)), dim3(256), 0, ST, (const float*)img, (float*)out, (int)C, (int)H, (int)W, (int)ps, gh, gw,
                       (int)Kp, total);
    return ull_check_launch();
}

extern "C" int ull_im2col3x3_f32(const void* x, void* out, int64_t B, int64_t H, int64_t W, int64_t C, void* stream) {
    if (!x || !out || B <= 0 || H <= 0 || W <= 0 || C <= 0) return ULL_ERR_ARG;
    const long total = B * H * W * 9 * C;
    hipLaunchKernelGGL(im2col3x3_f32_kernel, dim3(grid_for(total)), dim3(256), 0, ST, (const float*)x, (float*)out, (int)H, (int)W, (int)C, total);
    return ull_check_launch();
}

extern "C" int ull_video_pool_f32(const void* f, void* out, int64_t B, int64_t T, int64_t N, int64_t D, int64_t tok_pitch, int64_t tok_off, void* stream) {
    if (!f || !out || B <= 0 || T <= 0 || N <= 0 || D <= 0) return ULL_ERR_ARG;
    hipLaunchKernelGGL(video_pool_f32_kernel, dim3((unsigned)(T + N), (unsigned)B), dim3(256), 0, ST, (const float*)f, (float*)out, (int)T, (int)N, (int)D,
                       (int)tok_pitch, (int)tok_off);
    return ull_check_launch();
}

extern "C" int ull_add_rows_f32(const void* a, const void* b, void* out, int64_t rows, int64_t D, int64_t b_rows, void* stream) {
    if (!a || !b || !out || rows <= 0 || D <= 0 || b_rows <= 0) return ULL_ERR_ARG;
    hipLaunchKernelGGL(add_rows_f32_kernel, dim3(grid_for(rows * D)), dim3(256), 0, ST, (const float*)a, (const float*)b, (float*)out, (long)rows, (int)D,
                       (long)b_rows);
    return ull_check_launch();
}

extern "C" int ull_window_unpartition_add_f32(const void* win, const void* shortcut, void* out, int64_t B, int64_t H, int64_t W, int64_t C, int64_t ws,
                                              void* stream) {
    if (!win || !shortcut || !out || B <= 0 || ws <= 0) return ULL_ERR_ARG;
    const int nWh = (int)((H + ws - 1) / ws), nWw = (int)((W + ws - 1) / ws);
    const long total = B * H * W * C;
    hipLaunchKernelGGL(window_unpartition_add_f32_kernel, dim3(grid_for(total)), dim3(256), 0, ST, (const float*)win, (const float*)shortcut, (float*)out,
                       (int)H, (int)W, (int)C, (int)ws, nWh, nWw, total);
    return ull_check_launch();
}

extern "C" int ull_sam_relpos_f32(const void* q, int64_t q_bs, int64_t q_hs, int64_t q_ss, const void* rel_pos_h, const void* rel_pos_w, void* out_h,
                                  void* out_w, int64_t NB, int64_t nH, int64_t KH, int64_t KW, int64_t hd, void* stream) {
    if (!q || !rel_pos_h || !rel_pos_w || !out_h || !out_w || NB <= 0) return ULL_ERR_ARG;
    if (hd > 256) return ULL_ERR_SHAPE;
    hipLaunchKernelGGL(relpos_f32_kernel, dim3((unsigned)(NB * nH * KH * KW)), dim3(128), 0, ST, (const float*)q, (long)q_bs, (long)q_hs, (long)q_ss,
                       (const float*)rel_pos_h, (const float*)rel_pos_w, (float*)out_h, (float*)out_w, (int)nH, (int)KH, (int)KW, (int)hd);
    return ull_check_launch();
}

extern "C" int ull_interp_rows_linear_f32(const void* x, void* y, int64_t L, int64_t M, int64_t C, void* stream) {
    if (!x || !y || L <= 0 || M <= 0 || C <= 0) return ULL_ERR_ARG;
    hipLaunchKernelGGL(interp_rows_f32_kernel, dim3((unsigned)((M * C + 255) / 256)), dim3(256), 0, ST, (const float*)x, (float*)y, (int)L, (int)M, (int)C);
    return ull_check_launch();
}

extern "C" int ull_mask_matmul_f32(const void* hyper, const void* up, void* masks, int64_t n, int64_t T, int64_t C, int64_t G, void* stream) {
    if (!hyper || !up || !masks || n <= 0 || T <= 0 || C <= 0 || G <= 0) return ULL_ERR_ARG;
// ... 22 lines not shown
```

u-llava_amd/csrc/gemm.hip:

```cpp
#include "ull_common.h"
#include <stdlib.h>
#include <type_traits>

namespace {

constexpr int BM = 128, BN = 128, BK = 64;
constexpr int TILE_BYTES = BM * BK * 2;
constexpr int BUF_BYTES = 2 * TILE_BYTES;
constexpr int GEMM_LDS = 2 * BUF_BYTES;
constexpr int GROUP_M = 8;

constexpr int EPI_BIAS = 1, EPI_ACT_SHIFT = 1, EPI_ACT_MASK = 3 << 1;
constexpr int EPI_RESID = 8, EPI_SWIGLU = 16, EPI_OUT_F32 = 32;
constexpr int EPI_W_TILED = 64, EPI_X_TILED = 128;
constexpr int EPI_BIAS_ROUNDED = 256;
constexpr int ULL_W4_FORCE_STAGED = 512;

struct GemmArgs {
    const elem_t* X; const elem_t* W; void* C;
    const elem_t* bias; const elem_t* R;
    long ldx, ldw, ldc, ldr;
    int M, N, K, flags;
    int nbm, nbn;
    int t_full, sk;
    float* ws;
    int group_m;
    const elem_t* rope_cos; const elem_t* rope_sin;
    int rope_cols;
};

ULL_DEV void glds16(const void* gsrc, uint32_t lds_byte_addr ) {
    uint32_t keep;
    asm volatile("s_mov_b32 %0, m0\n\ts_mov_b32 m0, %2\n\ts_nop 0\n\tglobal_load_lds_dwordx4 %1, off\n\ts_mov_b32 m0, %0"
                 : "=&s"(keep) : "v"(gsrc), "s"(lds_byte_addr) : "memory");
}

ULL_DEV void glds16s(const void* sbase , uint32_t voff, uint32_t lds_byte_addr ) {
    uint32_t keep;
    asm volatile("s_mov_b32 %0, m0\n\ts_mov_b32 m0, %3\n\ts_nop 0\n\tglobal_load_lds_dwordx4 %1, %2\n\ts_mov_b32 m0, %0"
                 : "=&s"(keep) : "v"(voff), "s"(sbase), "s"(lds_byte_addr) : "memory");
}

struct EpiCtx {
    const GemmArgs& p;
    int act, n_out;
    bool out_f32, has_res, bias_late, c_al, r_al;
};
ULL_DEV EpiCtx epi_ctx(const GemmArgs& p, bool swiglu) {
    const int flags = p.flags;
    const bool out_f32 = flags & EPI_OUT_F32;
    return EpiCtx{p, (flags & EPI_ACT_MASK) >> EPI_ACT_SHIFT, swiglu ? p.N / 2 : p.N, out_f32, (flags & EPI_RESID) != 0,
                  !swiglu && (flags & EPI_BIAS) && (flags & EPI_BIAS_ROUNDED), out_f32 ? (p.ldc & 3) == 0 : (p.ldc & 7) == 0, (p.ldr & 7) == 0};
}
ULL_DEV void big_finish8(const EpiCtx& c, float (&a)[8], int m, int n, bool has_pre = false, uint4 res_pre = uint4{0, 0, 0, 0}) {
        if (c.bias_late) {
#pragma unroll
            for (int e = 0; e < 8; ++e)
                if (n + e < c.n_out) a[e] = rnd(a[e] + e2f(c.p.bias[n + e]));
        }
        if (c.act == 1) {
#pragma unroll
            for (int e = 0; e < 8; ++e) a[e] = act_quick_gelu_e(a[e]);
        } else if (c.act == 2) {
#pragma unroll
            for (int e = 0; e < 8; e += 2) {
                const f32x2_t r = act_gelu_erf2(f32x2_t{a[e], a[e + 1]});
                a[e] = rnd(r.x); a[e + 1] = rnd(r.y);
            }
        } else if (c.act == 3) {
#pragma unroll
            for (int e = 0; e < 8; ++e) a[e] = fmaxf(a[e], 0.f);
        }
        const bool full = n + 8 <= c.n_out;
        if (c.has_res) {
            const elem_t* rp = c.p.R + (long)m * c.p.ldr + n;
            if (full && c.r_al) {
                float b[8];
                unpack8(has_pre ? res_pre : *(const uint4*)rp, b);
#pragma unroll
                for (int e = 0; e < 8; ++e) a[e] = rnd(b[e] + a[e]);
            } else {
#pragma unroll
                for (int e = 0; e < 8; ++e)
                    if (n + e < c.n_out) a[e] = rnd(e2f(rp[e]) + a[e]);
            }
        }
        if (c.out_f32) {
            float* cp = (float*)c.p.C + (long)m * c.p.ldc + n;
            if (full && c.c_al) {
                *(float4*)cp = make_float4(a[0], a[1], a[2], a[3]);
                *(float4*)(cp + 4) = make_float4(a[4], a[5], a[6], a[7]);
            } else {
#pragma unroll
                for (int e = 0; e < 8; ++e)
                    if (n + e < c.n_out) cp[e] = a[e];
            }
        } else {
            elem_t* cp = (elem_t*)c.p.C + (long)m * c.p.ldc + n;
            if (full && c.c_al) {
                *(uint4*)cp = pack8(a);
            } else if (full) {
                const uint4 pk = pack8(a);
                if ((((long)m * c.p.ldc + n) & 1) == 0) {
                    uint32_t* c4 = (uint32_t*)cp;
                    c4[0] = pk.x; c4[1] = pk.y; c4[2] = pk.z; c4[3] = pk.w;
                } else {
                    cp[0] = (elem_t)(pk.x & 0xffff);
                    uint32_t* c4 = (uint32_t*)(cp + 1);
                    c4[0] = (pk.x >> 16) | (pk.y << 16);
                    c4[1] = (pk.y >> 16) | (pk.z << 16);
                    c4[2] = (pk.z >> 16) | (pk.w << 16);
                    cp[7] = (elem_t)(pk.w >> 16);
                }
            } else {
#pragma unroll
                for (int e = 0; e < 8; ++e)
                    if (n + e < c.n_out) cp[e] = f2e(a[e]);
            }
        }
    }

template <bool SWIGLU, int JT, bool ROPE = false, int PHASE = 0, bool RAW1 = false, int UNR = 2, bool SW2 = false, int PERM = 0>
ULL_DEV void staged_epilogue(const GemmArgs& p, f32x4_t (&acc)[4][JT], char* reg, int lane, int mrow0, int nw0, const char* reg_partner = nullptr,
                             int sw_half = 0) {
    constexpr int ROWS = JT * 16;
    const int fr = lane & 15, fg = lane >> 4;
    const int flags = p.flags;
    const int act = (flags & EPI_ACT_MASK) >> EPI_ACT_SHIFT;
    const bool out_f32 = flags & EPI_OUT_F32;
    const bool has_res = flags & EPI_RESID;
    const int n_out = SWIGLU ? p.N / 2 : p.N;
    const bool bias_late = !SWIGLU && (flags & EPI_BIAS) && (flags & EPI_BIAS_ROUNDED);
    const bool raw_f32 = (PHASE == 0 || RAW1) && !SWIGLU && out_f32 && !act && !has_res && !bias_late;
    const bool c_al = out_f32 ? (p.ldc & 3) == 0 : (p.ldc & 7) == 0;
    const bool r_al = (p.ldr & 7) == 0;
    const int ncol0 = SWIGLU ? nw0 / 2 : nw0;

    const EpiCtx ectx = epi_ctx(p, SWIGLU);
    auto finish8 = [&](float (&a)[8], int m, int n) { big_finish8(ectx, a, m, n); };
    auto col_of = [&](int i) { return PERM ? 32 * (i >> 1) + 8 * fg + 4 * (i & 1) : i * 16 + fg * 4; };
    float bias_v[4][4];
#pragma unroll
    for (int i = 0; i < 4; ++i)
#pragma unroll
        for (int r = 0; r < 4; ++r) {
            const int n = nw0 + col_of(i) + r;
            bias_v[i][r] = (!SWIGLU && (flags & EPI_BIAS) && !bias_late && n < p.N) ? e2f(p.bias[n]) : -0.0f;
        }

    if (!raw_f32) {
        constexpr int WCOLS = (SWIGLU && !SW2) ? 32 : 64;
        constexpr int PITCH = WCOLS * 2 + 16;
        if constexpr (PHASE != 2) {
        auto park_all = [&](auto with_bias) {
        constexpr bool WB = decltype(with_bias)::value;
#pragma clang loop unroll(full)
        for (int j = 0; j < JT; ++j) {
            if constexpr (SWIGLU) {
#pragma clang loop unroll(full)
                for (int ip = 0; ip < 2; ++ip) {
                    float v[4];
#pragma unroll
                    for (int r = 0; r < 4; ++r) {
                        const float g = rnd(acc[2 * ip][j][r]);
                        const float u = rnd(acc[2 * ip + 1][j][r]);
                        v[r] = rnd(act_silu(g)) * u;
                    }
// ... 534 lines not shown
        const int r = (wave * 4 + i) * 8 + srow;
        xsrc[i] = x_tiled ? p.X + (((long)bm * nk_total) * BM + r) * BK + schunk * 8
                          : p.X + (long)min(m0 + r, p.M - 1) * p.ldx + schunk * 8;
        wsrc[i] = w_tiled ? p.W + (((long)bn * nk_total) * BN + r) * BK + schunk * 8
                          : p.W + (long)min(n0 + r, p.N - 1) * p.ldw + schunk * 8;
    }
    const long xstep = x_tiled ? BM * BK : BK, wstep = w_tiled ? BN * BK : BK;
    const uint32_t lds_base = __builtin_amdgcn_readfirstlane((uint32_t)(uintptr_t)(__attribute__((address_space(3))) char*)smem);
    const uint32_t piece_off = wave * 4 * 1024;
    auto stage = [&](int kt) {
        const uint32_t bx = lds_base + (kt & 1) * SLOT_BYTES + piece_off;
        const long kox = (long)kt * xstep, kow = (long)kt * wstep;
#pragma unroll
        for (int i = 0; i < 4; ++i) {
            glds16(xsrc[i] + kox, bx + i * 1024);
            glds16(wsrc[i] + kow, bx + OP_BYTES + i * 1024);
        }
    };

    const int fr = lane & 15, fg = lane >> 4;
    int swz[2];
    swz[0] = ((0 + fg) ^ (lane & 7)) << 4;
    swz[1] = ((4 + fg) ^ (lane & 7)) << 4;
    const int xoff = (wm * 128 + fr) * (BK * 2);
    const int woff = OP_BYTES + (wn * 64 + fr) * (BK * 2);
    auto read_frags = [&](int kt, int kk, Frags& f) {
        const char* base = smem + (kt & 1) * SLOT_BYTES + swz[kk];
#pragma unroll
        for (int i = 0; i < 4; ++i) f.w[i] = *(const uint4*)(base + woff + i * 16 * (BK * 2));
#pragma unroll
        for (int j = 0; j < 8; ++j) f.x[j] = *(const uint4*)(base + xoff + j * 16 * (BK * 2));
    };

    f32x4_t acc[4][8];
#pragma unroll
    for (int i = 0; i < 4; ++i)
#pragma unroll
        for (int j = 0; j < 8; ++j) acc[i][j] = f32x4_t{0.f, 0.f, 0.f, 0.f};
    int nk = p.K / BK;
    if (split) {
        const int kt0 = (int)((long)nk * slice / p.sk), kt1 = (int)((long)nk * (slice + 1) / p.sk);
#pragma unroll
        for (int i = 0; i < 4; ++i) { xsrc[i] += (long)kt0 * xstep; wsrc[i] += (long)kt0 * wstep; }
        nk = kt1 - kt0;
    }
constexpr int ULL_W8_BAR_A = 14;
constexpr int ULL_W8_DMA_STRIDE = 6;
constexpr int ULL_W8_BAR_B = 40;
constexpr int ULL_W8_FA_STRIDE = 2;
    constexpr int W8_BAR_A = ULL_W8_BAR_A, W8_DMA_STRIDE = ULL_W8_DMA_STRIDE, W8_BAR_B = ULL_W8_BAR_B, W8_FA_STRIDE = ULL_W8_FA_STRIDE;
    constexpr int W8_ISSUED = (W8_BAR_B - W8_BAR_A + W8_DMA_STRIDE - 1) / W8_DMA_STRIDE;
    constexpr int W8_INFLIGHT = W8_ISSUED > 8 ? 8 : W8_ISSUED;
    static_assert(W8_BAR_A >= 12 && W8_BAR_B >= W8_BAR_A && W8_BAR_A + 7 * W8_DMA_STRIDE < 64 && W8_BAR_B + 11 * W8_FA_STRIDE < 64, "schedule");
    constexpr int USE_ORDER[12] = {0, 4, 1, 2, 3, 5, 6, 7, 8, 9, 10, 11};
    auto read1 = [&](int kt, int kk, Frags& f, int r) {
        const char* base = smem + (kt & 1) * SLOT_BYTES + swz[kk];
        if (r < 4) f.w[r] = *(const uint4*)(base + woff + r * 16 * (BK * 2));
        else f.x[r - 4] = *(const uint4*)(base + xoff + (r - 4) * 16 * (BK * 2));
    };
    auto mma1 = [&](const Frags& f, int s) {
        const int j = s >> 2, i = s & 3;
        acc[i][j] = mfma16(f.w[i], f.x[j], acc[i][j]);
    };
    stage(0);
    stage(1);
    asm volatile("s_waitcnt vmcnt(8)" ::: "memory");
    __builtin_amdgcn_s_barrier();
    Frags fa, fb;
    read_frags(0, 0, fa);
    const uint32_t dump = lds_base + LDS_BYTES;
#pragma clang loop unroll(disable)
    for (int kt = 0; kt < nk; ++kt) {
        const bool with_dma = kt + 2 < nk;
        const int ktd = with_dma ? kt + 2 : nk - 1;
        const long kox = (long)ktd * xstep, kow = (long)ktd * wstep;
        const uint32_t bx = with_dma ? lds_base + (kt & 1) * SLOT_BYTES + piece_off : dump;
        const uint32_t bw = with_dma ? bx + OP_BYTES : dump + 4096;
#pragma clang loop unroll(full)
        for (int s = 0; s < 64; ++s) {
            if (s == W8_BAR_A) {
                asm volatile("s_waitcnt lgkmcnt(0)" ::: "memory");
                __builtin_amdgcn_s_barrier();
            }
            if (s == W8_BAR_B) {
                asm volatile("s_waitcnt vmcnt(%0)" :: "n"(W8_INFLIGHT) : "memory");
                __builtin_amdgcn_s_barrier();
            }
            if (s < 12) read1(kt, 1, fb, s);
            if (s >= W8_BAR_B && (s - W8_BAR_B) % W8_FA_STRIDE == 0 && (s - W8_BAR_B) / W8_FA_STRIDE < 12)
                read1(kt + 1, 0, fa, USE_ORDER[(s - W8_BAR_B) / W8_FA_STRIDE]);
            if (s >= W8_BAR_A && (s - W8_BAR_A) % W8_DMA_STRIDE == 0 && (s - W8_BAR_A) / W8_DMA_STRIDE < 8) {
                const int pc = (s - W8_BAR_A) / W8_DMA_STRIDE;
                if (pc < 4) glds16(xsrc[pc] + kox, bx + pc * 1024);
                else glds16(wsrc[pc - 4] + kow, bw + (pc - 4) * 1024);
            }
            mma1(s < 32 ? fa : fb, s & 31);
            __builtin_amdgcn_sched_barrier(0);
        }
    }

    if (split) {
        float* slab = p.ws + ((long)(bid - p.t_full) * p.sk + slice) * (BM * BN);
#pragma clang loop unroll(full)
        for (int j = 0; j < 8; ++j)
#pragma clang loop unroll(full)
            for (int i = 0; i < 4; ++i)
                *(f32x4_t*)(slab + (wm * 128 + j * 16 + fr) * BN + wn * 64 + i * 16 + fg * 4) = acc[i][j];
        return;
    }
    __builtin_amdgcn_s_barrier();
    staged_epilogue<SWIGLU, 8, ROPE>(p, acc, smem + wave * (128 * 144), lane, m0 + wm * 128, n0 + wn * 64, smem + (wave ^ 1) * (128 * 144));
}


struct Frags4 { uint4 w[8]; uint4 x[8]; };

#ifdef ULL_ELEM_F16
#define ULL_MFMA16_ASM "v_mfma_f32_16x16x32_f16"
#else
#define ULL_MFMA16_ASM "v_mfma_f32_16x16x32_bf16"
#endif
typedef uint32_t u32x4_t __attribute__((ext_vector_type(4)));
ULL_DEV void mfma16_inplace(f32x4_t& c, const uint4& a, const uint4& b) {
    const u32x4_t av = {a.x, a.y, a.z, a.w}, bv = {b.x, b.y, b.z, b.w};
    asm volatile(ULL_MFMA16_ASM " %0, %1, %2, %0" : "+a"(c) : "v"(av), "v"(bv));
}


template <bool SWIGLU> ULL_DEV int w4_row_swizzle(int row) {
    return SWIGLU ? (((row >> 1) & 1) | (((row >> 3) & 1) << 1) | (((row >> 5) & 1) << 2)) : (((row >> 1) & 1) | (((row >> 3) & 3) << 1));
}
template <bool SWIGLU> ULL_DEV constexpr int w4_frag_row(int c) {
    return SWIGLU ? 64 * (c >> 2) + 16 * (c & 1) + 4 * ((c >> 1) & 1) : 32 * (c >> 1) + 4 * (c & 1);
}
template <bool SWIGLU> ULL_DEV int w4_lane_row(int fr) {
    return SWIGLU ? 32 * (fr >> 3) + 8 * ((fr >> 2) & 1) + (fr & 3) : 8 * (fr >> 2) + (fr & 3);
}
template <bool SWIGLU> ULL_DEV int w4_acc_row(int h, int i, int fg) {
    return SWIGLU ? h * 64 + 32 * (fg >> 1) + 16 * (i & 1) + 8 * (fg & 1) + 4 * (i >> 1) : h * 64 + 32 * (i >> 1) + 8 * fg + 4 * (i & 1);
}

ULL_DEV f32x4_t w4_acc_to_vgpr(const f32x4_t& a) {
    f32x4_t t = a;
    asm volatile("" : "+v"(t));
    return t;
}

template <bool SWIGLU, bool ROPE, int NH = 2, int RPF = 8>
ULL_DEV void w4_direct_epilogue(const GemmArgs& p, f32x4_t (&acc)[NH][4][8], int lane, int mrow0, int nw0) {
    static_assert(NH == 2 || (!SWIGLU && !ROPE), "SwiGLU and RoPE pair columns across the two halves");
    const int fr = lane & 15, fg = lane >> 4;
    if constexpr (SWIGLU) {
        const int n_out = p.N / 2, nb = nw0 / 2 + 8 * fg;
        elem_t* cb = (elem_t*)p.C + nb;
#pragma clang loop unroll(full)
        for (int j = 0; j < 8; ++j) {
            const int m = mrow0 + j * 16 + fr;
#pragma clang loop unroll(full)
            for (int h = 0; h < 2; ++h) {
                float v[8];
#pragma clang loop unroll(full)
                for (int pp = 0; pp < 2; ++pp) {
                    const f32x4_t ag = w4_acc_to_vgpr(acc[h][2 * pp][j]), au = w4_acc_to_vgpr(acc[h][2 * pp + 1][j]);
#pragma unroll
                    for (int r = 0; r < 4; ++r) {
                        const float g = rnd(ag[r]);
                        const float u = rnd(au[r]);
                        v[4 * pp + r] = rnd(act_silu(g)) * u;
                    }
                }
                if (m < p.M && nb + h * 32 + 8 <= n_out) *(uint4*)(cb + (long)m * p.ldc + h * 32) = pack8(v);
            }
            __builtin_amdgcn_sched_barrier(0);
        }
    } else {
        const int flags = p.flags;
        const bool has_bias = flags & EPI_BIAS, has_res = flags & EPI_RESID;
        const bool rope_on = ROPE && nw0 < p.rope_cols;
        const int nb = nw0 + 8 * fg;
        uint4 bvp[NH][2];
#pragma unroll
        for (int h = 0; h < NH; ++h)
#pragma unroll
            for (int pp = 0; pp < 2; ++pp) {
                const int n = nb + h * 64 + pp * 32;
                bvp[h][pp] = (has_bias && n + 8 <= p.N) ? *(const uint4*)(p.bias + n) : uint4{0, 0, 0, 0};
            }
        elem_t* cb = (elem_t*)p.C + nb;
        const elem_t* rb = p.R + nb;
        auto body = [&](auto with_bias, auto with_res, auto act_kind) {
            constexpr bool WB = decltype(with_bias)::value, WR = decltype(with_res)::value;
            constexpr int ACT = decltype(act_kind)::value;
            constexpr int NB_ = ROPE ? 2 : RPF;
            uint4 rv[NB_][NH][2], tc[NB_][2], ts[NB_][2];
            auto fetch = [&](int j, int buf) {
                const long mc = min(mrow0 + j * 16 + fr, p.M - 1);
                if constexpr (WR) {
#pragma unroll
                    for (int h = 0; h < NH; ++h)
#pragma unroll
                        for (int pp = 0; pp < 2; ++pp) rv[buf][h][pp] = *(const uint4*)(rb + mc * p.ldr + h * 64 + pp * 32);
                }
                if constexpr (ROPE) {
                    if (rope_on) {
#pragma unroll
                        for (int pp = 0; pp < 2; ++pp) {
                            tc[buf][pp] = *(const uint4*)(p.rope_cos + mc * 64 + pp * 32 + 8 * fg);
                            ts[buf][pp] = *(const uint4*)(p.rope_sin + mc * 64 + pp * 32 + 8 * fg);
                        }
                    }
                }
            };
            if constexpr (ROPE || NB_ < 8) fetch(0, 0);
            else if constexpr (WR) {
#pragma clang loop unroll(full)
                for (int j = 0; j < 8; ++j) fetch(j, j);
                __builtin_amdgcn_sched_barrier(0);
            }
#pragma clang loop unroll(full)
            for (int j = 0; j < 8; ++j) {
                const int m = mrow0 + j * 16 + fr;
                if constexpr (ROPE || NB_ < 8) { if (j + 1 < 8) fetch(j + 1, (j + 1) % NB_); }
                uint4 o[NH][2];
#pragma unroll
                for (int h = 0; h < NH; ++h)
#pragma unroll
                    for (int pp = 0; pp < 2; ++pp) {
                        float v[8], bv[8];
                        if constexpr (WB) unpack8(bvp[h][pp], bv);
                        const f32x4_t a0 = w4_acc_to_vgpr(acc[h][2 * pp][j]), a1 = w4_acc_to_vgpr(acc[h][2 * pp + 1][j]);
#pragma unroll
                        for (int e = 0; e < 8; ++e) {
                            const float a = e < 4 ? a0[e & 3] : a1[e & 3];
                            v[e] = WB ? a + bv[e] : a;
                        }
                        o[h][pp] = pack8(v);
                        if constexpr (ACT != 0) {
                            float a[8];
                            unpack8(o[h][pp], a);
                            if constexpr (ACT == 2) {
#pragma unroll
                                for (int e = 0; e < 8; e += 2) {
                                    const f32x2_t r = act_gelu_erf2(f32x2_t{a[e], a[e + 1]});
                                    a[e] = r.x; a[e + 1] = r.y;
                                }
                            } else {
#pragma unroll
                                for (int e = 0; e < 8; ++e) a[e] = ACT == 1 ? act_quick_gelu_e(a[e]) : fmaxf(a[e], 0.f);
                            }
                            o[h][pp] = pack8(a);
                        }
                    }
                if constexpr (ROPE) {
                    if (rope_on) {
#pragma unroll
                        for (int pp = 0; pp < 2; ++pp) {
                            float x0[8], x1[8], cs[8], sn[8];
                            unpack8(o[0][pp], x0); unpack8(o[1][pp], x1);
                            unpack8(tc[j % NB_][pp], cs); unpack8(ts[j % NB_][pp], sn);
                            float y0[8], y1[8];
#pragma unroll
                            for (int e = 0; e < 8; ++e) {
                                y0[e] = rnd(x0[e] * cs[e]) + rnd(-x1[e] * sn[e]);
                                y1[e] = rnd(x1[e] * cs[e]) + rnd(x0[e] * sn[e]);
                            }
                            o[0][pp] = pack8(y0); o[1][pp] = pack8(y1);
                        }
                    }
                }
#pragma unroll
                for (int h = 0; h < NH; ++h)
#pragma unroll
                    for (int pp = 0; pp < 2; ++pp) {
                        if constexpr (WR) {
                            float a[8], b[8];
                            unpack8(o[h][pp], a); unpack8(rv[j % NB_][h][pp], b);
#pragma unroll
                            for (int e = 0; e < 8; ++e) a[e] = rnd(b[e] + a[e]);
                            o[h][pp] = pack8(a);
                        }
                        if (m < p.M && nb + h * 64 + pp * 32 + 8 <= p.N) *(uint4*)(cb + (long)m * p.ldc + h * 64 + pp * 32) = o[h][pp];
                    }
                __builtin_amdgcn_sched_barrier(0);
            }
        };
        using I0 = std::integral_constant<int, 0>;
        const int act = (flags & EPI_ACT_MASK) >> EPI_ACT_SHIFT;
        if constexpr (!ROPE) {
            if (act) {
                if (act == 1) { if (has_bias) body(std::true_type{}, std::false_type{}, std::integral_constant<int, 1>{}); else body(std::false_type{}, std::false_type{}, std::integral_constant<int, 1>{}); }
                else if (act == 2) { if (has_bias) body(std::true_type{}, std::false_type{}, std::integral_constant<int, 2>{}); else body(std::false_type{}, std::false_type{}, std::integral_constant<int, 2>{}); }
                else { if (has_bias) body(std::true_type{}, std::false_type{}, std::integral_constant<int, 3>{}); else body(std::false_type{}, std::false_type{}, std::integral_constant<int, 3>{}); }
                return;
            }
        }
        if (has_bias) { if (has_res) body(std::true_type{}, std::true_type{}, I0{}); else body(std::true_type{}, std::false_type{}, I0{}); }
        else { if (has_res) body(std::false_type{}, std::true_type{}, I0{}); else body(std::false_type{}, std::false_type{}, I0{}); }
    }
}

template <bool SWIGLU, bool ROPE = false>
__global__ __launch_bounds__(256) void gemm256w4_kernel(GemmArgs p) {
    extern __shared__ __attribute__((aligned(16))) char smem[];
    ULL_STAMP(0); ULL_STAMP(7);
    const int tid = threadIdx.x, lane = tid & 63;
    const int wave = __builtin_amdgcn_readfirstlane(tid >> 6);
    const int wn = wave & 1, wm = wave >> 1;
    int bid = blockIdx.x;
    int slice = 0;
    const bool split = bid >= p.t_full;
    if (!split) {
        const int nwg = p.t_full;
        const int q = nwg >> 3, r = nwg & 7, xcd = bid & 7, k = bid >> 3;
        bid = (xcd < r ? xcd * (q + 1) : r * (q + 1) + (xcd - r) * q) + k;
    } else {
        const int r = bid - p.t_full;
        bid = p.t_full + r / p.sk;
        slice = r % p.sk;
    }
    const int per_group = p.group_m * p.nbn;
    const int gid = bid / per_group;
    const int first_m = gid * p.group_m;
    const int gsz = min(p.nbm - first_m, p.group_m);
    const int bm = first_m + (bid % per_group) % gsz;
// ... 401 lines not shown
        const char* base = smem + (kt & 1) * SLOT_BYTES;
        if (r < 4) f.w[r] = *(const uint4*)(base + wswz[kk] + woff + w4_frag_row<false>(r) * (BK * 2));
        else f.x[r - 4] = *(const uint4*)(base + swz[kk] + xoff + (r - 4) * 16 * (BK * 2));
    };
    auto mma1 = [&](const Frags& f, int s) {
        const int j = s >> 2, i = s & 3;
        acc[0][i][j] = mfma16(f.w[i], f.x[j], acc[0][i][j]);
    };
    stage(0);
    stage(1);
    asm volatile("s_waitcnt vmcnt(8)" ::: "memory");
    __builtin_amdgcn_s_barrier();
    Frags fa, fb;
    read_frags(0, 0, fa);
    const uint32_t dump = lds_base + LDS_BYTES;
#pragma clang loop unroll(disable)
    for (int kt = 0; kt < nk; ++kt) {
        const bool with_dma = kt + 2 < nk;
        const int ktd = with_dma ? kt + 2 : nk - 1;
        const long kox = (long)ktd * xstep, kow = (long)ktd * wstep;
        const uint32_t bx = with_dma ? lds_base + (kt & 1) * SLOT_BYTES + piece_off : dump;
        const uint32_t bw = with_dma ? bx + OP_BYTES : dump + 4096;
#pragma clang loop unroll(full)
        for (int s = 0; s < 64; ++s) {
            if (s == W8_BAR_A) {
                asm volatile("s_waitcnt lgkmcnt(0)" ::: "memory");
                __builtin_amdgcn_s_barrier();
            }
            if (s == W8_BAR_B) {
                asm volatile("s_waitcnt vmcnt(%0)" :: "n"(W8_INFLIGHT) : "memory");
                __builtin_amdgcn_s_barrier();
            }
            if (s < 12) read1(kt, 1, fb, s);
            if (s >= W8_BAR_B && (s - W8_BAR_B) % W8_FA_STRIDE == 0 && (s - W8_BAR_B) / W8_FA_STRIDE < 12)
                read1(kt + 1, 0, fa, USE_ORDER[(s - W8_BAR_B) / W8_FA_STRIDE]);
            if (s >= W8_BAR_A && (s - W8_BAR_A) % W8_DMA_STRIDE == 0 && (s - W8_BAR_A) / W8_DMA_STRIDE < 8) {
                const int pc = (s - W8_BAR_A) / W8_DMA_STRIDE;
                if (pc < 4) glds16(xsrc[pc] + kox, bx + pc * 1024);
                else glds16(wsrc[pc - 4] + kow, bw + (pc - 4) * 1024);
            }
            mma1(s < 32 ? fa : fb, s & 31);
            __builtin_amdgcn_sched_barrier(0);
        }
    }

    if (split) {
        float* slab = p.ws + ((long)(bid - p.t_full) * p.sk + slice) * (BM * BN);
#pragma clang loop unroll(full)
        for (int j = 0; j < 8; ++j)
#pragma clang loop unroll(full)
            for (int i = 0; i < 4; ++i)
                *(f32x4_t*)(slab + (wm * 128 + j * 16 + fr) * BN + wn * 64 + w4_acc_row<false>(0, i, fg)) = acc[0][i][j];
        return;
    }
    {
        const int fl = p.flags;
        const bool direct = !(fl & (EPI_OUT_F32 | EPI_BIAS_ROUNDED)) && (!(fl & EPI_ACT_MASK) || !(fl & EPI_RESID)) && (p.ldc & 7) == 0 && (p.N & 7) == 0 &&
                            (!(fl & EPI_RESID) || (p.ldr & 7) == 0) && !(fl & ULL_W4_FORCE_STAGED);
        if (direct) {
            w4_direct_epilogue<false, false, 1>(p, acc, lane, m0 + wm * 128, n0 + wn * 64);
            return;
        }
    }
    __builtin_amdgcn_s_barrier();
    staged_epilogue<false, 8, false, 0, false, 2, false, 1>(p, acc[0], smem + wave * (128 * 144), lane, m0 + wm * 128, n0 + wn * 64);
}




template <int BM, int BN, bool LINEAR>
__global__ __launch_bounds__(256) void splitk_finalize_any_kernel(GemmArgs p) {
    const int flags = p.flags;
    const bool swiglu = flags & EPI_SWIGLU;
    const int act = (flags & EPI_ACT_MASK) >> EPI_ACT_SHIFT;
    const bool out_f32 = flags & EPI_OUT_F32;
    const int n_out_total = swiglu ? p.N / 2 : p.N;
    const int tile_r = blockIdx.y;
    int m0, n0;
    if constexpr (LINEAR) {
        m0 = (tile_r / p.nbn) * BM;
        n0 = (tile_r % p.nbn) * BN;
    } else {
        const int pid = p.t_full + tile_r;
        const int per_group = p.group_m * p.nbn;
        const int gid = pid / per_group;
        const int first_m = gid * p.group_m;
        const int gsz = min(p.nbm - first_m, p.group_m);
        m0 = (first_m + (pid % per_group) % gsz) * BM;
        n0 = ((pid % per_group) / gsz) * BN;
    }
    const float* slab0 = p.ws + (long)tile_r * p.sk * (BM * BN);
    const int quads_per_row = swiglu ? BN / 8 : BN / 4;
    for (int q = blockIdx.x * 256 + threadIdx.x; q < BM * quads_per_row; q += gridDim.x * 256) {
        const int ml = q / quads_per_row, qc = q % quads_per_row;
        const int m = m0 + ml;
        if (m >= p.M) continue;
        float v[4];
        int n;
        if (swiglu) {
            const int grp = qc / 4, off = (qc % 4) * 4;
            float g[4] = {0.f, 0.f, 0.f, 0.f}, u[4] = {0.f, 0.f, 0.f, 0.f};
            for (int s = 0; s < p.sk; ++s) {
                const float* row = slab0 + (long)s * (BM * BN) + ml * BN + grp * 32 + off;
                const f32x4_t a = *(const f32x4_t*)row, b = *(const f32x4_t*)(row + 16);
#pragma unroll
                for (int r = 0; r < 4; ++r) { g[r] += a[r]; u[r] += b[r]; }
            }
            n = n0 / 2 + grp * 16 + off;
#pragma unroll
            for (int r = 0; r < 4; ++r) v[r] = rnd(rnd(act_silu(rnd(g[r]))) * rnd(u[r]));
        } else {
            float a4[4] = {0.f, 0.f, 0.f, 0.f};
            for (int s = 0; s < p.sk; ++s) {
                const f32x4_t a = *(const f32x4_t*)(slab0 + (long)s * (BM * BN) + ml * BN + qc * 4);
#pragma unroll
                for (int r = 0; r < 4; ++r) a4[r] += a[r];
            }
            n = n0 + qc * 4;
            if (p.rope_cos != nullptr && n < p.rope_cols) {
                const bool first_half = (n & 64) == 0;
                const int qp = first_half ? qc + 16 : qc - 16;
                float b4[4] = {0.f, 0.f, 0.f, 0.f};
                for (int s = 0; s < p.sk; ++s) {
                    const f32x4_t b = *(const f32x4_t*)(slab0 + (long)s * (BM * BN) + ml * BN + qp * 4);
#pragma unroll
                    for (int r = 0; r < 4; ++r) b4[r] += b[r];
                }
#pragma unroll
                for (int r = 0; r < 4; ++r) {
                    const float c = e2f(p.rope_cos[(long)m * 64 + ((n + r) & 63)]), sn = e2f(p.rope_sin[(long)m * 64 + ((n + r) & 63)]);
                    const float x = rnd(a4[r]), xp = rnd(b4[r]);
                    a4[r] = rnd(x * c) + rnd((first_half ? -xp : xp) * sn);
                }
            }
#pragma unroll
            for (int r = 0; r < 4; ++r) {
                float t = a4[r];
                if ((flags & EPI_BIAS) && (flags & EPI_BIAS_ROUNDED)) t = rnd(t);
                if ((flags & EPI_BIAS) && n + r < p.N) t += e2f(p.bias[n + r]);
                if (!out_f32 || act || (flags & EPI_RESID)) t = rnd(t);
                if (act == 1) t = act_quick_gelu_e(t);
                else if (act == 2) t = rnd(act_gelu_erf(t));
                else if (act == 3) t = fmaxf(t, 0.f);
                v[r] = t;
            }
        }
#pragma unroll
        for (int r = 0; r < 4; ++r) {
            if (n + r >= n_out_total) continue;
            float t = v[r];
            if (flags & EPI_RESID) t = rnd(e2f(p.R[(long)m * p.ldr + n + r]) + t);
            if (out_f32) ((float*)p.C)[(long)m * p.ldc + n + r] = t;
            else ((elem_t*)p.C)[(long)m * p.ldc + n + r] = f2e(t);
        }
    }
}

}

}

static int gemm_device_state(int* n_cu_out) {
    constexpr int MAX_DEV = 64;
    static int n_cu[MAX_DEV];
    int dev = 0;
    if (hipGetDevice(&dev) != hipSuccess || dev < 0 || dev >= MAX_DEV) return ULL_ERR_LAUNCH;
    if (!n_cu[dev]) {
        hipDeviceProp_t prop;
        const int n = (hipGetDeviceProperties(&prop, dev) == hipSuccess && prop.multiProcessorCount > 0) ? prop.multiProcessorCount : 256;
        (void)hipFuncSetAttribute((const void*)big::gemm256_kernel<false>, hipFuncAttributeMaxDynamicSharedMemorySize, big::LDS_BYTES_W4);
        (void)hipFuncSetAttribute((const void*)big::gemm256_kernel<true>, hipFuncAttributeMaxDynamicSharedMemorySize, big::LDS_BYTES_W4);
        (void)hipFuncSetAttribute((const void*)big::gemm256_kernel<false, true>, hipFuncAttributeMaxDynamicSharedMemorySize, big::LDS_BYTES_W4);
        (void)hipFuncSetAttribute((const void*)big::gemm256d_kernel, hipFuncAttributeMaxDynamicSharedMemorySize, big::LDS_BYTES_W4);
        (void)hipFuncSetAttribute((const void*)big::gemm256w4_kernel<false>, hipFuncAttributeMaxDynamicSharedMemorySize, big::LDS_BYTES_W4);
        (void)hipFuncSetAttribute((const void*)big::gemm256w4_kernel<true>, hipFuncAttributeMaxDynamicSharedMemorySize, big::LDS_BYTES_W4);
        (void)hipFuncSetAttribute((const void*)big::gemm256w4_kernel<false, true>, hipFuncAttributeMaxDynamicSharedMemorySize, big::LDS_BYTES_W4);
        (void)hipFuncSetAttribute((const void*)gemm128_kernel<false, true>, hipFuncAttributeMaxDynamicSharedMemorySize, GEMM_LDS);
        (void)hipFuncSetAttribute((const void*)gemm128_kernel<false>, hipFuncAttributeMaxDynamicSharedMemorySize, GEMM_LDS);
        (void)hipFuncSetAttribute((const void*)gemm128_kernel<true>, hipFuncAttributeMaxDynamicSharedMemorySize, GEMM_LDS);
        (void)hipFuncSetAttribute((const void*)patchify_gemm_kernel<0>, hipFuncAttributeMaxDynamicSharedMemorySize, GEMM_LDS);
#ifndef ULL_ELEM_F16
        (void)hipFuncSetAttribute((const void*)gemm128_a8w8_kernel<false>, hipFuncAttributeMaxDynamicSharedMemorySize, GEMM_LDS);
        (void)hipFuncSetAttribute((const void*)gemm128_a8w8_kernel<true>, hipFuncAttributeMaxDynamicSharedMemorySize, GEMM_LDS);
#endif
        (void)hipFuncSetAttribute((const void*)big::patchify_strip_kernel<9>, hipFuncAttributeMaxDynamicSharedMemorySize, 2 * (288 + 256) * 128 + 256);
        (void)hipFuncSetAttribute((const void*)big::patchify_strip_kernel<4>, hipFuncAttributeMaxDynamicSharedMemorySize, 2 * (128 + 256) * 128 + 256);
        n_cu[dev] = n;
    }
    *n_cu_out = n_cu[dev];
    return ULL_OK;
}

#ifndef ULL_ELEM_F16
extern "C" int64_t ull_gemm_streamk_ws_bytes(void) { return (int64_t)256 * big::BM * big::BN * sizeof(float); }
#endif

static int gemm_dispatch(const void* X, int64_t ldx, const void* W, int64_t ldw, void* C, int64_t ldc, const void* bias, const void* R,
                         int64_t ldr, int64_t M, int64_t N, int64_t K, int flags, void* ws, int64_t ws_bytes, void* stream,
                         const elem_t* rope_cos, const elem_t* rope_sin, int rope_cols) {
    if (!X || !W || !C || M <= 0 || N <= 0 || K <= 0 || ws_bytes < 0) return ULL_ERR_ARG;
    if (K % BK != 0 || (ldx & 7) || (ldw & 7)) return ULL_ERR_SHAPE;
    if ((flags & EPI_BIAS) && !bias) return ULL_ERR_ARG;
    if ((flags & EPI_RESID) && !R) return ULL_ERR_ARG;
    if ((flags & EPI_SWIGLU) && ((N & 31) || (flags & (EPI_BIAS | EPI_ACT_MASK)))) return ULL_ERR_SHAPE;
    if (M > (1 << 30) || N > (1 << 30)) return ULL_ERR_SHAPE;
    int n_cu = 0;
    if (const int rc = gemm_device_state(&n_cu)) return rc;
    const int tune_group_m = (flags >> 16) & 15;
    const bool force_small = flags & (1 << 20);
    const bool force_waves8 = flags & (1 << 21);
    const bool force_waves4 = (flags & (1 << 22)) && ldx < (1 << 21) && ldw < (1 << 21);
    flags &= 0xffff;
    if ((flags & EPI_BIAS_ROUNDED) && (flags & EPI_SWIGLU)) return ULL_ERR_SHAPE;
    GemmArgs a;
    a.X = (const elem_t*)X; a.W = (const elem_t*)W; a.C = C;
    a.bias = (const elem_t*)bias; a.R = (const elem_t*)R;
    a.ldx = ldx; a.ldw = ldw; a.ldc = ldc; a.ldr = ldr;
    a.M = (int)M; a.N = (int)N; a.K = (int)K; a.flags = flags;
    a.rope_cos = rope_cos; a.rope_sin = rope_sin; a.rope_cols = rope_cols;
    const bool rope = rope_cos != nullptr;
    const bool short_and_few = K <= 768 && ((M + 255) / 256) * ((N + 255) / 256) < 512 && !(flags & (EPI_W_TILED | EPI_X_TILED));
    if (!force_small && !short_and_few && M >= 1024 && N >= 512 && K >= 128) {
        a.nbm = (int)((M + big::BM - 1) / big::BM); a.nbn = (int)((N + big::BN - 1) / big::BN);
        constexpr long SLAB = (long)big::BM * big::BN * sizeof(float);
        const int max_slabs = ws ? (int)(ws_bytes / SLAB < 4096 ? ws_bytes / SLAB : 4096) : 0;
        const int T = a.nbm * a.nbn;
        const int rem = T % n_cu;
        int sk = 1;
        if (max_slabs && T > n_cu && rem > 0 && rem <= n_cu / 2 && rem <= max_slabs) {
            sk = n_cu / rem;
            if (sk > 16) sk = 16;
            const int nk = (int)(K / big::BK);
            while (sk > 1 && nk / sk < 2) --sk;
            if (rem * sk > max_slabs) sk = max_slabs / rem;
        }
        a.sk = sk > 1 ? sk : 1;
        a.t_full = sk > 1 ? T - rem : T;
        a.ws = (float*)ws;
        a.group_m = tune_group_m ? tune_group_m : 4;
        const int grid = a.sk > 1 ? a.t_full + rem * a.sk : T;
        const bool c_rows_aligned = (flags & EPI_OUT_F32) ? (ldc & 3) == 0 : (ldc & 7) == 0;
        const int n_out_cols = (flags & EPI_SWIGLU) ? (int)(N / 2) : (int)N;
        const bool direct = rope || (!(flags & (EPI_OUT_F32 | EPI_BIAS_ROUNDED | ULL_W4_FORCE_STAGED)) && (!(flags & EPI_ACT_MASK) || !(flags & EPI_RESID)) &&
                                     (ldc & 7) == 0 && (n_out_cols & 7) == 0 && (!(flags & EPI_RESID) || (ldr & 7) == 0));
        const bool fits32 = ldx < (1 << 21) && ldw < (1 << 21);
        const bool waves4 = force_waves4 || (!force_waves8 && fits32 && (direct || (K >= 3072 && c_rows_aligned)));
        const bool waves8_direct = !force_waves4 && !force_waves8 && direct && !rope && !(flags & EPI_SWIGLU) && (flags & EPI_ACT_MASK) &&
                                   ((flags & EPI_ACT_MASK) >> EPI_ACT_SHIFT) != 3 && K < 3072;
        if (waves8_direct) {
            hipLaunchKernelGGL(big::gemm256d_kernel, dim3(grid), dim3(512), big::LDS_BYTES_W4, (hipStream_t)stream, a);
        } else if (waves4) {
            if (flags & EPI_SWIGLU)
                hipLaunchKernelGGL(big::gemm256w4_kernel<true>, dim3(grid), dim3(256), big::LDS_BYTES_W4, (hipStream_t)stream, a);
            else if (rope)
                hipLaunchKernelGGL((big::gemm256w4_kernel<false, true>), dim3(grid), dim3(256), big::LDS_BYTES_W4, (hipStream_t)stream, a);
            else
                hipLaunchKernelGGL(big::gemm256w4_kernel<false>, dim3(grid), dim3(256), big::LDS_BYTES_W4, (hipStream_t)stream, a);
        } else if (flags & EPI_SWIGLU)
            hipLaunchKernelGGL(big::gemm256_kernel<true>, dim3(grid), dim3(512), big::LDS_BYTES_W4, (hipStream_t)stream, a);
        else if (rope)
            hipLaunchKernelGGL((big::gemm256_kernel<false, true>), dim3(grid), dim3(512), big::LDS_BYTES_W4, (hipStream_t)stream, a);
        else
            hipLaunchKernelGGL(big::gemm256_kernel<false>, dim3(grid), dim3(512), big::LDS_BYTES_W4, (hipStream_t)stream, a);
        if (a.sk > 1) hipLaunchKernelGGL((big::splitk_finalize_any_kernel<big::BM, big::BN, false>), dim3(32, rem), dim3(256), 0, (hipStream_t)stream, a);
        return ull_check_launch();
    }
    if (flags & (EPI_W_TILED | EPI_X_TILED)) return ULL_ERR_SHAPE;
    a.nbm = (int)((M + BM - 1) / BM); a.nbn = (int)((N + BN - 1) / BN);
    a.t_full = 0; a.sk = 1; a.ws = nullptr; a.group_m = GROUP_M;
    const int T = a.nbm * a.nbn, nk = (int)(K / BK), slots = 2 * n_cu;
    if (ws && !force_small && T <= slots / 2 && nk >= 16) {
        constexpr long SLAB = (long)BM * BN * sizeof(float);
        int sk = slots / T;
        if (sk > nk / 8) sk = nk / 8;
        if (sk > 8) sk = 8;
        if ((long)T * sk * SLAB > ws_bytes) sk = (int)(ws_bytes / (T * SLAB));
        if (sk > 1) { a.sk = sk; a.ws = (float*)ws; }
    }
    const int grid = T * a.sk;
    if (flags & EPI_SWIGLU)
        hipLaunchKernelGGL(gemm128_kernel<true>, dim3(grid), dim3(256), GEMM_LDS, (hipStream_t)stream, a);
    else if (rope)
        hipLaunchKernelGGL((gemm128_kernel<false, true>), dim3(grid), dim3(256), GEMM_LDS, (hipStream_t)stream, a);
    else
        hipLaunchKernelGGL(gemm128_kernel<false>, dim3(grid), dim3(256), GEMM_LDS, (hipStream_t)stream, a);
    if (a.sk > 1) hipLaunchKernelGGL((big::splitk_finalize_any_kernel<BM, BN, true>), dim3(16, T), dim3(256), 0, (hipStream_t)stream, a);
    return ull_check_launch();
}

extern "C" int ULL_FN(ull_gemm_)(const void* X, int64_t ldx, const void* W, int64_t ldw, void* C, int64_t ldc,
                             const void* bias, const void* R, int64_t ldr,
                             int64_t M, int64_t N, int64_t K, int flags, void* ws, int64_t ws_bytes, void* stream) {
    return gemm_dispatch(X, ldx, W, ldw, C, ldc, bias, R, ldr, M, N, K, flags, ws, ws_bytes, stream, nullptr, nullptr, 0);
}

#ifndef ULL_ELEM_F16
extern "C" int ull_gemm_a8w8_bf16(const void* Xq, int64_t ldxq, const void* x_scales, const void* Q, int64_t ldq, const void* w_scales, void* C,
                                  int64_t ldc, const void* R, int64_t ldr, int64_t M, int64_t N, int64_t K, int flags, void* stream) {
    if (!Xq || !x_scales || !Q || !w_scales || !C || M <= 0 || N <= 0 || K <= 0) return ULL_ERR_ARG;
    if (flags & ~(EPI_RESID | EPI_SWIGLU | EPI_OUT_F32)) return ULL_ERR_ARG;
    if ((flags & EPI_RESID) && !R) return ULL_ERR_ARG;
    if (K % BK8 != 0 || (ldxq & 15) || (ldq & 15) || ldxq < K || ldq < K || (((uintptr_t)Xq | (uintptr_t)Q) & 15)) return ULL_ERR_SHAPE;
    if ((flags & EPI_SWIGLU) && (N & 31)) return ULL_ERR_SHAPE;
    if (ldc < ((flags & EPI_SWIGLU) ? N / 2 : N) || ((flags & EPI_RESID) && ldr < ((flags & EPI_SWIGLU) ? N / 2 : N))) return ULL_ERR_SHAPE;
    if (M > (1 << 30) || N > (1 << 30) || K > (1 << 30)) return ULL_ERR_SHAPE;
    int n_cu = 0;
    if (const int rc = gemm_device_state(&n_cu)) return rc;
    GemmArgs a;
    a.X = nullptr; a.W = nullptr; a.C = C; a.bias = nullptr; a.R = (const elem_t*)R;
    a.ldx = 0; a.ldw = 0; a.ldc = ldc; a.ldr = ldr;
    a.M = (int)M; a.N = (int)N; a.K = (int)K; a.flags = flags;
    a.nbm = (int)((M + BM - 1) / BM); a.nbn = (int)((N + BN - 1) / BN);
    a.t_full = 0; a.sk = 1; a.ws = nullptr; a.group_m = GROUP_M;
    a.rope_cos = a.rope_sin = nullptr; a.rope_cols = 0;
    if ((long)a.nbm * a.nbn > (1L << 30)) return ULL_ERR_SHAPE;
    const A8Args q{(const uint8_t*)Xq, (const uint8_t*)Q, (const float*)x_scales, (const float*)w_scales, (long)ldxq, (long)ldq};
    if (flags & EPI_SWIGLU)
        hipLaunchKernelGGL(gemm128_a8w8_kernel<true>, dim3(a.nbm * a.nbn), dim3(256), GEMM_LDS, (hipStream_t)stream, a, q);
    else
        hipLaunchKernelGGL(gemm128_a8w8_kernel<false>, dim3(a.nbm * a.nbn), dim3(256), GEMM_LDS, (hipStream_t)stream, a, q);
    return ull_check_launch();
}
#endif

extern "C" int ULL_FN(ull_gemm_qkv_rope_)(const void* X, int64_t ldx, const void* W, int64_t ldw, void* C, int64_t ldc, int64_t M, int64_t N,
                                      int64_t K, const void* rope_cos, const void* rope_sin, int64_t rope_cols, int64_t head_dim, int flags,
                                      void* ws, int64_t ws_bytes, void* stream) {
    if (!rope_cos || !rope_sin) return ULL_ERR_ARG;
    if (head_dim != 128 || rope_cols <= 0 || rope_cols > N || (rope_cols & 127) || (N & 127) || (ldc & 7)) return ULL_ERR_SHAPE;
    if (flags & (EPI_BIAS | EPI_ACT_MASK | EPI_RESID | EPI_SWIGLU | EPI_OUT_F32 | EPI_BIAS_ROUNDED)) return ULL_ERR_ARG;
    return gemm_dispatch(X, ldx, W, ldw, C, ldc, nullptr, nullptr, 0, M, N, K, flags, ws, ws_bytes, stream, (const elem_t*)rope_cos,
                         (const elem_t*)rope_sin, (int)rope_cols);
}

extern "C" int ULL_FN(ull_patchify_)(const void* img, int64_t n_img, int64_t C, int64_t H, int64_t W, int64_t ps, const void* Wp, int64_t Kp,
                                 const void* bias, void* out, int64_t ldc, int64_t N, const void* zeros, void* stream) {
    if (!img || !Wp || !out || !zeros || n_img <= 0 || C <= 0 || H <= 0 || W < 16 || N <= 0) return ULL_ERR_ARG;
    if (ps <= 0 || ps > 16 || (ps & 1) || H % ps || W % ps || Kp % BK || Kp < C * ps * 16 || (ldc & 7)) return ULL_ERR_SHAPE;
    GemmArgs a;
    PatchArgs q;
    q.img = (const elem_t*)img; q.zeros = (const elem_t*)zeros;
    q.img_end = (const elem_t*)img + n_img * C * H * W;
    q.C = (int)C; q.H = (int)H; q.W = (int)W; q.ps = (int)ps; q.gw = (int)(W / ps); q.gh = (int)(H / ps); q.nseg = (int)(C * ps);
    q.xcd_raster = 0;
    const int64_t M = n_img * q.gw * q.gh;
    if (M > (1 << 30)) return ULL_ERR_SHAPE;
    a.X = nullptr; a.W = (const elem_t*)Wp; a.C = out; a.bias = (const elem_t*)bias; a.R = nullptr;
    a.ldx = 0; a.ldw = Kp; a.ldc = ldc; a.ldr = 0;
    a.M = (int)M; a.N = (int)N; a.K = (int)Kp; a.flags = bias ? EPI_BIAS : 0;
    a.nbm = (int)((M + BM - 1) / BM); a.nbn = (int)((N + BN - 1) / BN);
    a.t_full = 0; a.sk = 1; a.ws = nullptr; a.group_m = GROUP_M;
    a.rope_cos = a.rope_sin = nullptr; a.rope_cols = 0;
    int n_cu = 0;
    if (const int rc = gemm_device_state(&n_cu)) return rc;
    if ((N & 255) == 0 && (ldc & 7) == 0 && Kp <= 1024 && C * H * W < (1LL << 31)) {
        const int nbn = (int)(N / 256);
        for (const int wmb : {9}) {
            const int tm = 32 * wmb;
            if (M % tm) continue;
            const long tiles = (M / tm) * nbn;
            if (tiles > n_cu || tiles * 2 <= n_cu) continue;
            a.nbm = (int)(M / tm); a.nbn = nbn;
            q.xcd_raster = a.nbm % 8 == 0;
            const int lds = 2 * (tm + 256) * 128 + 256;
            if (wmb == 9) hipLaunchKernelGGL(big::patchify_strip_kernel<9>, dim3((unsigned)tiles), dim3(512), lds, (hipStream_t)stream, a, q);
            else hipLaunchKernelGGL(big::patchify_strip_kernel<4>, dim3((unsigned)tiles), dim3(512), lds, (hipStream_t)stream, a, q);
            return ull_check_launch();
        }
    }
    hipLaunchKernelGGL(patchify_gemm_kernel<0>, dim3(a.nbm * a.nbn), dim3(256), GEMM_LDS, (hipStream_t)stream, a, q);
    return ull_check_launch();
}
```

u-llava_amd/csrc/layers.hip:

```cpp
#include <stdint.h>
#include <math.h>

#include "../../include/ullava_hip.h"

#ifdef ULL_ELEM_F16
#define FN(base) base##f16
#else
#define FN(base) base##bf16
#endif
#define TRY(call)                 \
    do {                          \
        const int rc_ = (call);   \
        if (rc_ != ULL_OK) return rc_; \
    } while (0)

namespace {

struct SK {
    void* ws;
    int64_t bytes;
    int64_t min_k;
};

struct Tiled {
    const void* w;
    int64_t ldw;
    int flags;
    void* ws;
    int64_t wsb;
};
inline Tiled tiled(const ull_linear* L, int64_t M, const SK& sk) {
    const bool big = M >= 1024 && L->n >= 512 && L->k >= 128;
    Tiled t{L->w, L->ldw, 0, nullptr, 0};
    if (big && L->w_tiled) { t.w = L->w_tiled; t.ldw = L->k; t.flags = ULL_EPI_W_TILED; }
    if (big && sk.min_k >= 0 && L->k >= sk.min_k) { t.ws = sk.ws; t.wsb = sk.bytes; }
    return t;
}

inline int lin(const void* x, int64_t ldx, const ull_linear* L, void* out, int64_t ldc, const void* R, int64_t ldr, int64_t M, int flags,
               const SK& sk, void* stream) {
    const Tiled t = tiled(L, M, sk);
    if (L->bias) flags |= ULL_EPI_BIAS;
    if (R) flags |= ULL_EPI_RESID;
    return FN(ull_gemm_)(x, ldx, t.w, t.ldw, out, ldc, L->bias, R, ldr, M, L->n, L->k, flags | t.flags, t.ws, t.wsb, stream);
}

inline bool quantized(const ull_linear* L) { return L->format != ULL_WF_ELEM; }
inline bool format_ok(const ull_linear* L) {
#ifndef ULL_ELEM_F16
    if (L->format == ULL_WF_FP8 || L->format == ULL_WF_MXFP4) return true;
#endif
    return !quantized(L);
}
inline bool has_weight(const ull_linear* L) { return L->w && (!quantized(L) || L->scales); }
inline bool pitch_ok(const ull_linear* L) {
    if (L->format == ULL_WF_MXFP4) return L->k % 32 == 0 && L->ldw >= L->k / 2 && L->ldw % 16 == 0 && L->lds >= L->k / 32 && L->lds % 4 == 0;
    return L->ldw >= L->k;
}
inline const void* bias_of(const ull_linear* L) { return quantized(L) ? nullptr : L->bias; }
inline int64_t ldw_of(const ull_linear* L) { return L->format == ULL_WF_MXFP4 ? L->k : L->ldw; }
inline int gemm_skinny(const void* x, int64_t ldx, const ull_linear* L, void* out, int64_t ldc, const void* R, int64_t ldr, int64_t M, int flags,
                       void* stream) {
#ifndef ULL_ELEM_F16
    if (quantized(L))
        return ull_gemm_skinny_wq_bf16(x, ldx, L->format, L->w, L->ldw, L->scales, L->lds, out, ldc, bias_of(L), R, ldr, M, L->n, L->k, flags, stream);
#endif
    return FN(ull_gemm_skinny_)(x, ldx, L->w, L->ldw, out, ldc, bias_of(L), R, ldr, M, L->n, L->k, flags, stream);
}
inline int gemv(const void* x, int64_t ldx, const ull_linear* L, void* out, int64_t ldc, const void* R, int64_t ldr, int64_t M, int flags, void* stream) {
#ifndef ULL_ELEM_F16
    if (quantized(L)) return ull_gemv_wq_bf16(x, ldx, L->format, L->w, L->ldw, L->scales, L->lds, out, ldc, bias_of(L), R, ldr, M, L->n, L->k, flags, stream);
#endif
    return FN(ull_gemv_)(x, ldx, L->w, L->ldw, out, ldc, bias_of(L), R, ldr, M, L->n, L->k, flags, stream);
}
inline int gemv_rmsnorm(const void* x, int64_t ldx, const void* rms_w, float eps, const ull_linear* L, void* out, int64_t ldc, const void* R,
                        int64_t ldr, int64_t M, int flags, void* stream) {
#ifndef ULL_ELEM_F16
    if (quantized(L))
        return ull_gemv_rmsnorm_wq_bf16(x, ldx, rms_w, eps, L->format, L->w, L->ldw, L->scales, L->lds, out, ldc, bias_of(L), R, ldr, M, L->n, L->k, flags,
                                        stream);
#endif
    return FN(ull_gemv_rmsnorm_)(x, ldx, rms_w, eps, L->w, L->ldw, out, ldc, bias_of(L), R, ldr, M, L->n, L->k, flags, stream);
}
inline int gemv_qkv_rope_append(const void* x, int64_t ldx, const void* rms_w, float eps, const ull_linear* L, void* q, int64_t ldq, const void* cs,
                                const void* sn, void* kc, void* vtc, int64_t B, int64_t S, int64_t H, int64_t hd, int64_t smax, int64_t past,
                                void* stream) {
#ifndef ULL_ELEM_F16
    if (quantized(L))
        return ull_gemv_qkv_rope_append_wq_bf16(x, ldx, rms_w, eps, L->format, L->w, L->ldw, L->scales, L->lds, q, ldq, cs, sn, kc, vtc, B, S, H, hd, L->k,
                                                smax, past, stream);
#endif
    return FN(ull_gemv_qkv_rope_append_)(x, ldx, rms_w, eps, L->w, L->ldw, q, ldq, cs, sn, kc, vtc, B, S, H, hd, L->k, smax, past, stream);
}

inline int lin_decode(const void* x, int64_t ldx, const void* rms_w, float eps, void* xn_scratch, const ull_linear* L, void* out, int64_t ldc,
                      const void* R, int64_t ldr, int64_t M, int flags, void* stream) {
    const bool skinny = M >= 3 && L->k % 32 == 0 && L->n * L->k >= ((int64_t)1 << 22) && ldw_of(L) % 8 == 0;
    if (bias_of(L)) flags |= ULL_EPI_BIAS;
    if (R) flags |= ULL_EPI_RESID;
    if (rms_w && (skinny || !(L->k % 8 == 0 && M * L->k <= 16384))) {
        TRY(FN(ull_rmsnorm_)(x, ldx, rms_w, xn_scratch, L->k, M, L->k, eps, stream));
        x = xn_scratch;
        ldx = L->k;
        rms_w = nullptr;
    }
    if (skinny) return gemm_skinny(x, ldx, L, out, ldc, R, ldr, M, flags, stream);
    if (rms_w) return gemv_rmsnorm(x, ldx, rms_w, eps, L, out, ldc, R, ldr, M, flags, stream);
    return gemv(x, ldx, L, out, ldc, R, ldr, M, flags, stream);
}

}

extern "C" int FN(ull_llama_prefill_layers_)(const ull_llama_layer* layers, int64_t n_layers, const void* x_in, void* const* x_out, void* x_mid,
                                             void* xn, void* qkv, void* att, void* act, const void* rope_cos, const void* rope_sin,
                                             const void* key_mask, int64_t B, int64_t S, int64_t H, int64_t hd, int64_t I, float eps, void* ws,
                                             int64_t ws_bytes, int64_t sk_min_k, const void* zeros, void* stream) {
    if (!layers || !x_in || !x_out || !x_mid || !xn || !qkv || !att || !act || !rope_cos || !rope_sin || !zeros || n_layers <= 0) return ULL_ERR_ARG;
    const int64_t D = H * hd, T = B * S;
    if (hd != 128 || T <= 16 || S <= 16 || S > 1024 || D % 64 || I % 64) return ULL_ERR_SHAPE;
    const SK sk{ws, ws_bytes, sk_min_k};
    const float scale = 1.0f / sqrtf((float)hd);
    const char* q = (const char*)qkv;
    const void* x = x_in;
    for (int64_t l = 0; l < n_layers; ++l) {
        const ull_llama_layer& w = layers[l];
        if (w.qkv.n != 3 * D || w.qkv.k != D || w.o.n != D || w.o.k != D || w.gu.n != 2 * I || w.gu.k != D || w.down.n != D || w.down.k != I || !x_out[l] ||
            quantized(&w.qkv) || quantized(&w.o) || quantized(&w.gu) || quantized(&w.down))
            return ULL_ERR_ARG;
        TRY(FN(ull_rmsnorm_)(x, D, w.ln1, xn, D, T, D, eps, stream));
        {
            const Tiled t = tiled(&w.qkv, T, sk);
            TRY(FN(ull_gemm_qkv_rope_)(xn, D, t.w, t.ldw, qkv, 3 * D, T, 3 * D, D, rope_cos, rope_sin, 2 * D, hd, t.flags, t.ws, t.wsb, stream));
        }
        TRY(FN(ull_attention_)(q, S * 3 * D, hd, 3 * D, q + D * 2, S * 3 * D, hd, 3 * D, q + 2 * D * 2, S * 3 * D, hd, 3 * D, 0, att, S * D, hd, D, key_mask,
                               B, H, S, S, hd, 1, 1, scale, 1.0f, nullptr, nullptr, 0, 0, 0, zeros, stream));
        TRY(lin(att, D, &w.o, x_mid, D, x, D, T, 0, sk, stream));
        TRY(FN(ull_rmsnorm_)(x_mid, D, w.ln2, xn, D, T, D, eps, stream));
        TRY(lin(xn, D, &w.gu, act, I, nullptr, 0, T, ULL_EPI_SWIGLU, sk, stream));
        TRY(lin(act, I, &w.down, x_out[l], D, x_mid, D, T, 0, sk, stream));
        x = x_out[l];
    }
    return ULL_OK;
}

namespace {

struct BfCache {
    void* const* k; void* const* vt;
};
inline bool cache_layer_ok(const BfCache& c, int64_t l) { return c.k[l] && c.vt[l]; }
inline bool cache_shape_ok(const BfCache& c, int64_t, int64_t) { return c.k && c.vt; }
inline int append_and_attend(const BfCache& c, int64_t l, const void* x, int64_t D, const void* ln1, float eps, const ull_linear* qkv, void* q, const void* cs,
                             const void* sn, void* att, const void* key_mask, int64_t B, int64_t S, int64_t H, int64_t hd, int64_t smax, int64_t past,
                             float scale, const void* zeros, void* stream) {
    TRY(gemv_qkv_rope_append(x, D, ln1, eps, qkv, q, D, cs, sn, c.k[l], c.vt[l], B, S, H, hd, smax, past, stream));
    return FN(ull_attention_)(q, S * D, hd, D, c.k[l], H * smax * hd, smax * hd, hd, c.vt[l], H * hd * smax, hd * smax, smax, smax, att, S * D, hd, D,
                              key_mask, B, H, S, past + S, hd, 1, 1, scale, 1.0f, nullptr, nullptr, 0, 0, 0, zeros, stream);
}

#ifndef ULL_ELEM_F16
struct Kv8Cache {
    void* const* k8; void* const* vt8; void* const* ks; void* const* vs;
    void* k_stage; void* vt_stage;
};
inline bool cache_layer_ok(const Kv8Cache& c, int64_t l) { return c.k8[l] && c.vt8[l] && c.ks[l] && c.vs[l]; }
inline bool cache_shape_ok(const Kv8Cache& c, int64_t S, int64_t past) {
    return c.k8 && c.vt8 && c.ks && c.vs && c.k_stage && c.vt_stage && S <= 16 && past + S > 64 && past + S <= 4096;
}
inline int append_and_attend(const Kv8Cache& c, int64_t l, const void* x, int64_t D, const void* ln1, float eps, const ull_linear* qkv, void* q, const void* cs,
                             const void* sn, void* att, const void* key_mask, int64_t B, int64_t S, int64_t H, int64_t hd, int64_t smax, int64_t past,
                             float scale, const void* zeros, void* stream) {
    TRY(gemv_qkv_rope_append(x, D, ln1, eps, qkv, q, D, cs, sn, c.k_stage, c.vt_stage, B, S, H, hd, 128, past & 63, stream));
    return ull_attention_kv8_bf16(q, S * D, hd, D, c.k_stage, c.vt_stage, c.k8[l], c.vt8[l], c.ks[l], c.vs[l], smax, att, S * D, hd, D, key_mask, B, H, S,
                                  past + S, hd, scale, zeros, stream);
}
#endif

template <class Cache>
int llama_decode_layers(const ull_llama_layer* layers, int64_t n_layers, const void* x_in, void* const* x_out, void* x_mid, void* xn, void* q, void* att, void* act,
                        const void* rope_cos, const void* rope_sin, const void* key_mask, const Cache& cache, int64_t B, int64_t S, int64_t H,
                        int64_t hd, int64_t I, int64_t smax, int64_t past, float eps, const void* zeros, void* stream) {
    if (!layers || !x_in || !x_out || !x_mid || !xn || !q || !att || !act || !rope_cos || !rope_sin || !zeros || n_layers <= 0) return ULL_ERR_ARG;
    const int64_t D = H * hd, T = B * S;
    if (T > 4 || T <= 0 || past <= 0 || (hd & 1) || D % 8 || I <= 0 || I % 8 || T * D * 2 > 32768 || past + S > smax) return ULL_ERR_SHAPE;
    if (!cache_shape_ok(cache, S, past)) return ULL_ERR_ARG;
    for (int64_t l = 0; l < n_layers; ++l) {
        const ull_llama_layer& w = layers[l];
        if (w.qkv.n != 3 * D || w.qkv.k != D || w.o.n != D || w.o.k != D || w.gu.n != 2 * I || w.gu.k != D || w.down.n != D || w.down.k != I)
            return ULL_ERR_SHAPE;
        for (const auto* L : {&w.qkv, &w.o, &w.gu, &w.down})
            if (!format_ok(L) || !has_weight(L) || !pitch_ok(L)) return ULL_ERR_ARG;
        if (!w.ln1 || !w.ln2 || !cache_layer_ok(cache, l) || !x_out[l]) return ULL_ERR_ARG;
    }
    const float scale = 1.0f / sqrtf((float)hd);
    const void* x = x_in;
    for (int64_t l = 0; l < n_layers; ++l) {
        const ull_llama_layer& w = layers[l];
        TRY(append_and_attend(cache, l, x, D, w.ln1, eps, &w.qkv, q, rope_cos, rope_sin, att, key_mask, B, S, H, hd, smax, past, scale, zeros, stream));
        TRY(lin_decode(att, D, nullptr, 0.f, xn, &w.o, x_mid, D, x, D, T, 0, stream));
        TRY(lin_decode(x_mid, D, w.ln2, eps, xn, &w.gu, act, I, nullptr, 0, T, ULL_EPI_SWIGLU, stream));
        TRY(lin_decode(act, I, nullptr, 0.f, xn, &w.down, x_out[l], D, x_mid, D, T, 0, stream));
        x = x_out[l];
    }
    return ULL_OK;
}

}

extern "C" int FN(ull_llama_decode_layers_)(const ull_llama_layer* layers, int64_t n_layers, const void* x_in, void* const* x_out, void* x_mid,
                                            void* xn, void* q, void* att, void* act, const void* rope_cos, const void* rope_sin,
                                            const void* key_mask, void* const* k_cache, void* const* vt_cache, int64_t B, int64_t S, int64_t H,
                                            int64_t hd, int64_t I, int64_t smax, int64_t past, float eps, const void* zeros, void* stream) {
    return llama_decode_layers(layers, n_layers, x_in, x_out, x_mid, xn, q, att, act, rope_cos, rope_sin, key_mask, BfCache{k_cache, vt_cache}, B, S, H,
                               hd, I, smax, past, eps, zeros, stream);
}

#ifndef ULL_ELEM_F16
extern "C" int ull_llama_decode_layers_kv8_bf16(const ull_llama_layer* layers, int64_t n_layers, const void* x_in, void* const* x_out, void* x_mid,
                                                void* xn, void* q, void* att, void* act, const void* rope_cos, const void* rope_sin,
                                                const void* key_mask, void* const* k8, void* const* vt8, void* const* k_scale, void* const* vt_scale,
                                                void* k_stage, void* vt_stage, int64_t B, int64_t S, int64_t H, int64_t hd, int64_t I, int64_t smax,
                                                int64_t past, float eps, const void* zeros, void* stream) {
    return llama_decode_layers(layers, n_layers, x_in, x_out, x_mid, xn, q, att, act, rope_cos, rope_sin, key_mask,
                               Kv8Cache{k8, vt8, k_scale, vt_scale, k_stage, vt_stage}, B, S, H, hd, I, smax, past, eps, zeros, stream);
}

#endif

extern "C" int FN(ull_clip_layers_)(const ull_clip_layer* layers, int64_t n_layers, void* h, void* h_mid, void* y, void* qkv, void* att, void* f,
                                    int64_t n_img, int64_t S, int64_t H, int64_t hd, int64_t I, float eps, void* ws, int64_t ws_bytes,
                                    int64_t sk_min_k, const void* zeros, void* stream) {
    if (!layers || !h || !h_mid || !y || !qkv || !att || !f || !zeros || n_layers < 0) return ULL_ERR_ARG;
    const int64_t D = H * hd, T = n_img * S;
    if (hd != 64 || T <= 16 || S <= 16 || S > 704 || D % 64 || I % 64) return ULL_ERR_SHAPE;
    const SK sk{ws, ws_bytes, sk_min_k};
    const float scale = 1.0f / sqrtf((float)hd);
    const char* q = (const char*)qkv;
    for (int64_t l = 0; l < n_layers; ++l) {
        const ull_clip_layer& w = layers[l];
        if (w.qkv.n != 3 * D || w.qkv.k != D || w.out.n != D || w.out.k != D || w.fc1.n != I || w.fc1.k != D || w.fc2.n != D || w.fc2.k != I ||
            quantized(&w.qkv) || quantized(&w.out) || quantized(&w.fc1) || quantized(&w.fc2))
            return ULL_ERR_ARG;
        TRY(FN(ull_layernorm_)(h, D, w.ln1_w, w.ln1_b, y, D, T, D, eps, stream));
        TRY(lin(y, D, &w.qkv, qkv, 3 * D, nullptr, 0, T, 0, sk, stream));
        TRY(FN(ull_attention_)(q, S * 3 * D, hd, 3 * D, q + D * 2, S * 3 * D, hd, 3 * D, q + 2 * D * 2, S * 3 * D, hd, 3 * D, 0, att, S * D, hd, D, nullptr,
                               n_img, H, S, S, hd, 0, 1, scale, 1.0f, nullptr, nullptr, 0, 0, 0, zeros, stream));
        TRY(lin(att, D, &w.out, h_mid, D, h, D, T, 0, sk, stream));
        TRY(FN(ull_layernorm_)(h_mid, D, w.ln2_w, w.ln2_b, y, D, T, D, eps, stream));
        TRY(lin(y, D, &w.fc1, f, I, nullptr, 0, T, ULL_EPI_ACT_QUICK_GELU, sk, stream));
        TRY(lin(f, I, &w.fc2, h, D, h_mid, D, T, 0, sk, stream));
    }
    return ULL_OK;
}

extern "C" int FN(ull_sam_blocks_)(const ull_sam_block* blocks, int64_t n_blocks, void* x, void* x_mid, void* y, void* qkv, void* att, void* f,
                                   int64_t B, int64_t g, int64_t nH, int64_t hd, int64_t I, float eps, void* ws, int64_t ws_bytes, int64_t sk_min_k,
                                   const void* zeros, void* stream) {
    if (!blocks || !x || !x_mid || !y || !qkv || !att || !f || !zeros || n_blocks <= 0) return ULL_ERR_ARG;
    const int64_t C = nH * hd, T = B * g * g, S = g * g;
    if (hd != 80 || g != 64 || C % 64 || I % 64) return ULL_ERR_SHAPE;
    const SK sk{ws, ws_bytes, sk_min_k};
    const float q_scale = 1.0f / sqrtf((float)hd);
    const char* q = (const char*)qkv;
    for (int64_t i = 0; i < n_blocks; ++i) {
        const ull_sam_block& w = blocks[i];
        if (w.qkv.n != 3 * C || w.qkv.k != C || !w.qkv.bias || w.proj.n != C || w.proj.k != C || w.lin1.n != I || w.lin1.k != C || w.lin2.n != C ||
            w.lin2.k != I || !w.rel_pos_h || !w.rel_pos_w || (w.window != 0 && w.window != 14) || quantized(&w.qkv) || quantized(&w.proj) || quantized(&w.lin1) ||
            quantized(&w.lin2))
            return ULL_ERR_ARG;
        TRY(FN(ull_layernorm_)(x, C, w.n1_w, w.n1_b, y, C, T, C, eps, stream));
        TRY(lin(y, C, &w.qkv, qkv, 3 * C, nullptr, 0, T, 0, sk, stream));
        if (w.window)
            TRY(FN(ull_sam_window_attention_)(qkv, 3 * C, w.qkv.bias, w.rel_pos_h, w.rel_pos_w, att, C, B, g, g, nH, hd, w.window, q_scale, zeros, stream));
        else
            TRY(FN(ull_attention_)(q, S * 3 * C, hd, 3 * C, q + C * 2, S * 3 * C, hd, 3 * C, q + 2 * C * 2, S * 3 * C, hd, 3 * C, 0, att, S * C, hd, C,
                                   nullptr, B, nH, S, S, hd, 0, 0, 1.0f, q_scale, w.rel_pos_h, w.rel_pos_w, g, g, 2, zeros, stream));
        TRY(lin(att, C, &w.proj, x_mid, C, x, C, T, 0, sk, stream));
        TRY(FN(ull_layernorm_)(x_mid, C, w.n2_w, w.n2_b, y, C, T, C, eps, stream));
        TRY(lin(y, C, &w.lin1, f, I, nullptr, 0, T, ULL_EPI_ACT_GELU, sk, stream));
        TRY(lin(f, I, &w.lin2, x, C, x_mid, C, T, 0, sk, stream));
    }
    return ULL_OK;
}
```

u-llava_amd/csrc/norm.hip:

```cpp
#include "ull_common.h"

namespace {

template <int NCH, int MODE>
__global__ __launch_bounds__(256) void rownorm_kernel(const elem_t* __restrict__ x, long ldx, const elem_t* __restrict__ w,
                                                      const elem_t* __restrict__ b, elem_t* __restrict__ y, long ldy,
                                                      long rows, int D, float eps, int lpr,
                                                      const elem_t* __restrict__ cls, const elem_t* __restrict__ pos, int tokens) {
    const int lane = threadIdx.x & 63;
    const int sub = lane & (lpr - 1);
    const int rows_per_wave = 64 / lpr;
    const long row = ((long)blockIdx.x * 4 + (threadIdx.x >> 6)) * rows_per_wave + lane / lpr;
    const bool row_ok = row < rows;
    const int nchunk = D >> 3;
    float v[NCH][8];
    const elem_t* xr;
    const elem_t* pr = nullptr;
    if (cls != nullptr) {
        const long img = row / tokens;
        const int t = (int)(row - img * tokens);
        xr = (t == 0) ? cls : x + (img * (tokens - 1) + (t - 1)) * ldx;
        pr = pos + (long)t * D;
    } else {
        xr = x + row * ldx;
    }
    float s1 = 0.f, s2 = 0.f;
#pragma unroll
    for (int i = 0; i < NCH; ++i) {
        const int c = sub + i * lpr;
        if (row_ok && c < nchunk) {
            unpack8(*(const uint4*)(xr + c * 8), v[i]);
            if (pr != nullptr) {
                float pv[8];
                unpack8(*(const uint4*)(pr + c * 8), pv);
#pragma unroll
                for (int j = 0; j < 8; ++j) v[i][j] = rnd(v[i][j] + pv[j]);
            }
        } else {
#pragma unroll
            for (int j = 0; j < 8; ++j) v[i][j] = 0.f;
        }
#pragma unroll
        for (int j = 0; j < 8; ++j) { s1 += v[i][j]; s2 += v[i][j] * v[i][j]; }
    }
    const float invD = 1.0f / (float)D;
    float mean = 0.f, rstd;
    if (MODE == 0) {
        s2 = group_sum(s2, lpr);
        rstd = rsqrtf(s2 * invD + eps);
    } else {
        s1 = group_sum(s1, lpr);
        mean = s1 * invD;
        float q = 0.f;
#pragma unroll
        for (int i = 0; i < NCH; ++i) {
            const int c = sub + i * lpr;
            if (c < nchunk) {
#pragma unroll
                for (int j = 0; j < 8; ++j) { const float d = v[i][j] - mean; q += d * d; }
            }
        }
        q = group_sum(q, lpr);
        rstd = 1.0f / sqrtf(q * invD + eps);
    }
    if (!row_ok) return;
    elem_t* yr = y + row * ldy;
#pragma unroll
    for (int i = 0; i < NCH; ++i) {
        const int c = sub + i * lpr;
        if (c < nchunk) {
            float wv[8], o[8];
            unpack8(*(const uint4*)(w + c * 8), wv);
            if (MODE == 0) {
#pragma unroll
                for (int j = 0; j < 8; ++j) o[j] = wv[j] * rnd(v[i][j] * rstd);
            } else {
                float bv[8];
                unpack8(*(const uint4*)(b + c * 8), bv);
#pragma unroll
                for (int j = 0; j < 8; ++j) o[j] = ((v[i][j] - mean) * rstd) * wv[j] + bv[j];
            }
            *(uint4*)(yr + c * 8) = pack8(o);
        }
    }
}

template <int MODE>
int launch_rownorm(const elem_t* x, long ldx, const elem_t* w, const elem_t* b, elem_t* y, long ldy, long rows, int D, float eps,
                   const elem_t* cls, const elem_t* pos, int tokens, hipStream_t st) {
    if (D <= 0 || (D & 7) || (ldx & 7) || (ldy & 7) || rows <= 0) return ULL_ERR_SHAPE;
    const int nchunk = D >> 3;
    int lpr = 1;
    while (lpr < 64 && lpr < nchunk) lpr <<= 1;
    const int nch = (nchunk + lpr - 1) / lpr;
    const long rows_per_block = 4 * (64 / lpr);
    const dim3 grid((unsigned)((rows + rows_per_block - 1) / rows_per_block));
#define ULL_RN(N) hipLaunchKernelGGL((rownorm_kernel<N, MODE>), grid, dim3(256), 0, st, x, ldx, w, b, y, ldy, rows, D, eps, lpr, cls, pos, tokens)
    if (nch <= 1) ULL_RN(1);
    else if (nch <= 2) ULL_RN(2);
    else if (nch <= 4) ULL_RN(4);
    else if (nch <= 8) ULL_RN(8);
    else if (nch <= 16) ULL_RN(16);
    else return ULL_ERR_SHAPE;
#undef ULL_RN
    return ull_check_launch();
}

}

extern "C" int ULL_FN(ull_rmsnorm_)(const void* x, int64_t ldx, const void* w, void* y, int64_t ldy, int64_t rows, int64_t D, float eps,
                                void* stream) {
    if (!x || !w || !y) return ULL_ERR_ARG;
    return launch_rownorm<0>((const elem_t*)x, ldx, (const elem_t*)w, nullptr, (elem_t*)y, ldy, rows, (int)D, eps, nullptr, nullptr, 0,
                             (hipStream_t)stream);
}

extern "C" int ULL_FN(ull_layernorm_)(const void* x, int64_t ldx, const void* w, const void* b, void* y, int64_t ldy, int64_t rows, int64_t D,
                                  float eps, void* stream) {
    if (!x || !w || !b || !y) return ULL_ERR_ARG;
    return launch_rownorm<1>((const elem_t*)x, ldx, (const elem_t*)w, (const elem_t*)b, (elem_t*)y, ldy, rows, (int)D, eps, nullptr, nullptr,
                             0, (hipStream_t)stream);
}

extern "C" int ULL_FN(ull_clip_embed_ln_)(const void* patch, int64_t ldp, const void* cls, const void* pos, const void* w, const void* b,
                                      void* y, int64_t ldy, int64_t n_img, int64_t tokens, int64_t D, float eps, void* stream) {
    if (!patch || !cls || !pos || !w || !b || !y || tokens < 2) return ULL_ERR_ARG;
    return launch_rownorm<1>((const elem_t*)patch, ldp, (const elem_t*)w, (const elem_t*)b, (elem_t*)y, ldy, n_img * tokens, (int)D, eps,
                             (const elem_t*)cls, (const elem_t*)pos, (int)tokens, (hipStream_t)stream);
}

namespace {
__global__ __launch_bounds__(256) void shifted_ce_kernel(const elem_t* __restrict__ logits, long ld, const int64_t* __restrict__ labels, int B,
                                                         int S, int V, float* __restrict__ out ) {
    const int lane = threadIdx.x & 63;
    const long row = (long)blockIdx.x * 4 + (threadIdx.x >> 6);
    if (row >= (long)B * (S - 1)) return;
    const int b = (int)(row / (S - 1)), t = (int)(row % (S - 1));
    const int64_t lab = labels[(long)b * S + t + 1];
    if (lab < 0 || lab >= V) return;
    const elem_t* lp = logits + ((long)b * S + t) * ld;
    float m = -INFINITY;
    for (int i = lane; i < V; i += 64) m = fmaxf(m, e2f(lp[i]));
    m = wave_max(m);
    float s = 0.f;
    for (int i = lane; i < V; i += 64) s += __expf(e2f(lp[i]) - m);
    s = wave_sum(s);
    if (lane == 0) {
        atomicAdd(out, m + __logf(s) - e2f(lp[lab]));
        atomicAdd(out + 1, 1.0f);
    }
}
}

extern "C" int ULL_FN(ull_shifted_cross_entropy_)(const void* logits, int64_t ld, const void* labels, int64_t B, int64_t S, int64_t V, void* out,
                                              void* stream) {
    if (!logits || !labels || !out || B <= 0 || S <= 1 || V <= 0) return ULL_ERR_ARG;
    const long rows = B * (S - 1);
    hipLaunchKernelGGL(shifted_ce_kernel, dim3((unsigned)((rows + 3) / 4)), dim3(256), 0, (hipStream_t)stream, (const elem_t*)logits, ld,
                       (const int64_t*)labels, (int)B, (int)S, (int)V, (float*)out);
    return ull_check_launch();
}
```

u-llava_amd/ops.py:

```python
import weakref
from typing import Optional


import torch

from . import _lib

BF16 = torch.bfloat16
F16 = torch.float16
F32 = torch.float32
_SFX = {BF16: "bf16", F16: "f16", F32: "f32"}
DT_CODE = {torch.float32: 0, BF16: 1, F16: 2}
EPI_BIAS, EPI_QGELU, EPI_GELU, EPI_RELU, EPI_RESID, EPI_SWIGLU, EPI_F32 = 1, 1 << 1, 2 << 1, 3 << 1, 8, 16, 32
EPI_BIAS_ROUNDED = 256
ACTS = {None: 0, "quick_gelu": EPI_QGELU, "gelu": EPI_GELU, "relu": EPI_RELU}


_ZEROS = {}


def _zeros(device):
    z = _ZEROS.get(device)
    if z is None:
        z = _ZEROS[device] = torch.zeros(256, device=device, dtype=BF16)
    return z


def vt_unpermute_index(pitch: int) -> torch.Tensor:
    key = torch.arange(pitch)
    w = key % 32
    a, g, r = w // 16, (w % 16) // 4, w % 4
    return (key // 32) * 32 + 8 * g + 4 * a + r


def _stream():
    return torch.cuda.current_stream().cuda_stream


def _copy_sfx(dtype, D: int):
    if dtype == F32:
        if D % 4:
            raise RuntimeError("u-llava_amd: fp32 rows must be a multiple of 4 elements wide")
        return "bf16", 2 * D
    return _SFX[dtype], D


def _p(t: Optional[torch.Tensor]):
    return None if t is None else t.data_ptr()


def _chk(t: torch.Tensor, name: str, dtype=None):
    if not t.is_cuda:
        raise RuntimeError(f"u-llava_amd: `{name}` must live on the GPU (no CPU path exists)")
    if dtype is None:
        if t.dtype not in _SFX:
            raise RuntimeError(f"u-llava_amd: `{name}` must be torch.bfloat16, torch.float16 or torch.float32, got {t.dtype}")
    elif t.dtype != dtype:
        raise RuntimeError(f"u-llava_amd: `{name}` must be {dtype}, got {t.dtype}")
    if t.dim() and t.stride(-1) != 1:
        raise RuntimeError(f"u-llava_amd: `{name}` must be contiguous in its last dim")


def _rows(t: torch.Tensor):
    if t.dim() == 1:
        return 1, t.shape[0]
    if t.dim() == 2:
        return t.shape[0], t.stride(0)
    if t.is_contiguous():
        return t.numel() // t.shape[-1], t.shape[-1]
    if t.stride(-1) != 1 or any(t.stride(i) != t.shape[i + 1] * t.stride(i + 1) for i in range(t.dim() - 2)):
        raise RuntimeError("u-llava_amd: >2-D operands must be contiguous, or rows of one common pitch")
    return t.numel() // t.shape[-1], t.stride(-2)


EPI_W_TILED = 64
_TILED = {}


def tile_major(w: torch.Tensor) -> torch.Tensor:
    N, K = w.shape
    Np = (N + 255) // 256 * 256
    if Np != N:
        w = torch.cat([w, w.new_zeros(Np - N, K)])
    return w.view(Np // 256, 256, K // 64, 64).permute(0, 2, 1, 3).contiguous()


def register_tiled(w: torch.Tensor) -> None:
    if w.dim() == 2 and w.shape[1] % 64 == 0 and w.shape[0] >= 512 and w.shape[1] >= 128 and w.is_contiguous() and w.dtype != F32:
        ptr = w.data_ptr()
        _TILED[ptr] = [weakref.ref(w, lambda _r, _p=ptr: _TILED.pop(_p, None) if (_TILED.get(_p) or (None,))[0] is _r else None),
                       tile_major(w.detach()), w._version]


def _tiled_of(w: torch.Tensor):
    e = _TILED.get(w.data_ptr())
    if e is None:
        return None
    if e[0]() is not w:
        _TILED.pop(w.data_ptr(), None)
        return None
    if e[2] != w._version:
        N, K = w.shape
        if not e[1].is_inference() and not torch.is_inference_mode_enabled() and N % 256 == 0 and tuple(e[1].shape) == (N // 256, K // 64, 256, 64):
            with torch.no_grad():
                e[1].copy_(w.detach().view(N // 256, 256, K // 64, 64).permute(0, 2, 1, 3))
        else:
            e[1] = tile_major(w.detach())
        e[2] = w._version
    return e[1]


def unregister_tiled(w: torch.Tensor) -> None:
    e = _TILED.get(w.data_ptr())
    if e is not None and e[0]() is w:
        del _TILED[w.data_ptr()]


class Fp8Weight:
    __slots__ = ("codes", "scales", "_kpad")
    fmt_name, wf = "fp8", _lib.WF_FP8

    def __init__(self, codes: torch.Tensor, scales: torch.Tensor):
        if codes.dtype != torch.uint8 or codes.dim() != 2 or codes.stride(1) != 1 or scales.dtype != F32 or scales.shape != (codes.shape[0],):
            raise RuntimeError("u-llava_amd.Fp8Weight: codes uint8 [N, K] (rows contiguous), scales fp32 [N]")
        self.codes, self.scales = codes, scales
        self._kpad = None

    @property
    def shape(self):
        return self.codes.shape

    @property
    def device(self):
        return self.codes.device

    def nbytes(self) -> int:
        return self.codes.numel() + 4 * self.scales.numel()

    @property
    def route_pitch(self) -> int:
        return self.codes.stride(0)

    def c_args(self):
        return self.wf, self.codes.data_ptr(), self.codes.stride(0), self.scales.data_ptr(), 0

    def dequantize_into(self, out: torch.Tensor, tiled: bool) -> None:
        N, K = self.shape
        _lib.call("ull_dequantize_rows_fp8_bf16", _p(self.codes), self.codes.stride(0), _p(self.scales), N, K, _p(out), int(tiled), _stream())


def quantize_fp8(w: torch.Tensor) -> Fp8Weight:
    _chk(w, "w", BF16)
    if w.dim() != 2:
        raise RuntimeError("u-llava_amd.quantize_fp8: w must be 2-D")
    N, K = w.shape
    codes = torch.empty(N, K, device=w.device, dtype=torch.uint8)
    scales = torch.empty(N, device=w.device, dtype=F32)
    _lib.call("ull_quantize_rows_fp8_bf16", _p(w), w.stride(0), N, K, _p(codes), _p(scales), _stream())
    return Fp8Weight(codes, scales)


def dequantize(q, tiled: bool = False, out: Optional[torch.Tensor] = None) -> torch.Tensor:
    N, K = q.shape
    rows = -(-N // 256) * 256 if tiled else N
    if out is None:
        out = torch.empty(rows * K, device=q.device, dtype=BF16)
    elif out.dtype != BF16 or out.numel() < rows * K or not out.is_contiguous():
        raise RuntimeError(f"u-llava_amd.dequantize_{q.fmt_name}: `out` must be a contiguous bf16 buffer of at least the result's size")
    q.dequantize_into(out, tiled)
    return out[:rows * K].view(rows // 256, K // 64, 256, 64) if tiled else out[:N * K].view(N, K)


dequantize_fp8 = dequantize_mxfp4 = dequantize


_MX_PERM = {}


def _mx_perm(K: int, device):
    key = (K, str(device))
    e = _MX_PERM.get(key)
    if e is None:
        nsb = K // 2048
        c = torch.arange(K // 8, device=device)
        cpos = torch.where(c < nsb * 256, (c >> 8) * 1024 + (c & 63) * 16 + ((c >> 6) & 3) * 4, c * 4)
        cidx = (cpos[:, None] + torch.arange(4, device=device)).reshape(-1)
        b = torch.arange(K // 32, device=device)
        sidx = torch.where(b < nsb * 64, (b >> 6) * 64 + (b & 15) * 4 + ((b >> 4) & 3), b)
        e = _MX_PERM[key] = (cidx, sidx)
    return e


class Mxfp4Weight:
    __slots__ = ("codes", "scales", "K")
    fmt_name, wf = "mxfp4", _lib.WF_MXFP4

    def __init__(self, codes: torch.Tensor, scales: torch.Tensor, K: int):
        if (codes.dtype != torch.uint8 or codes.dim() != 2 or K % 32 or codes.shape[1] != K // 2 or not codes.is_contiguous() or
                scales.dtype != torch.uint8 or scales.shape != (codes.shape[0], self.scale_pitch(K)) or not scales.is_contiguous()):
            raise RuntimeError("u-llava_amd.Mxfp4Weight: codes uint8 [N, K / 2], scales uint8 [N, K / 32 rounded up to 4], contiguous, K % 32 == 0")
        self.codes, self.scales, self.K = codes, scales, K

    @staticmethod
    def scale_pitch(K: int) -> int:
        return -(-(K // 32) // 4) * 4

    @property
    def shape(self):
        return torch.Size((self.codes.shape[0], self.K))

    @property
    def device(self):
        return self.codes.device

    def nbytes(self) -> int:
        return self.codes.numel() + self.scales.numel()

    @property
    def route_pitch(self) -> int:
        return self.K

    def c_args(self):
        return self.wf, self.codes.data_ptr(), self.codes.stride(0), self.scales.data_ptr(), self.scales.stride(0)

    def dequantize_into(self, out: torch.Tensor, tiled: bool) -> None:
        N, K = self.shape
        _lib.call("ull_dequantize_rows_mxfp4_bf16", _p(self.codes), self.codes.stride(0), _p(self.scales), self.scales.stride(0), N, K, _p(out),
                  int(tiled), 1, _stream())
# ... 947 lines not shown
              float(eps), _p(ws), _p(out), pa, fa, _stream())
    return out, outs


def sam_small_mlps(hs, hyper_mlps, iou_head):
    import ctypes
    _chk(hs, "hs")
    n, T, _ = hs.shape
    ptrs = []
    for m in list(hyper_mlps) + [iou_head]:
        ptrs += _lin_ptrs(*m.layers)
    arr = (ctypes.c_void_p * 30)(*ptrs)
    C, n_iou = hyper_mlps[0].layers[2].weight.shape[0], iou_head.layers[2].weight.shape[0]
    hyper = torch.empty(n, 4, C, device=hs.device, dtype=hs.dtype)
    iou = torch.empty(n, n_iou, device=hs.device, dtype=hs.dtype)
    _lib.call("ull_sam_small_mlps_" + _SFX[hs.dtype], _p(hs), n, T, arr, 4, C, n_iou, _p(hyper), _p(iou), _stream())
    return hyper, iou


def sam_t2i_attention(qproj, keys, pos, a, late_bias_kv: bool):
    _chk(qproj, "qproj"); _chk(keys, "keys", qproj.dtype); _chk(pos, "pos", qproj.dtype)
    n, T, _ = qproj.shape
    P = keys.shape[1]
    ws_s = torch.empty(n * 8 * 8 * P, device=keys.device, dtype=keys.dtype)
    ws_v = torch.empty(n * P * 128, device=keys.device, dtype=keys.dtype)
    att = torch.empty(n, T, 128, device=keys.device, dtype=keys.dtype)
    _lib.call("ull_sam_t2i_attention_" + _SFX[qproj.dtype], _p(qproj), _p(keys), _p(pos), n, T, P, *_lin_ptrs(a.k_proj, a.v_proj), int(late_bias_kv),
              _p(ws_s), _p(ws_v), _p(att), _stream())
    return att


def sam_i2t_attention_ln(keys, pos, kproj, vproj, a, ln, late_bias_q: bool, eps: float = 1e-5):
    _chk(keys, "keys"); _chk(pos, "pos", keys.dtype); _chk(kproj, "kproj", keys.dtype); _chk(vproj, "vproj", keys.dtype)
    n, T, _ = kproj.shape
    P = keys.shape[1]
    out = torch.empty_like(keys)
    _lib.call("ull_sam_i2t_attention_ln_" + _SFX[keys.dtype], _p(keys), _p(pos), _p(kproj), _p(vproj), n, T, P, *_lin_ptrs(a.q_proj, a.out_proj),
              int(late_bias_q), _p(ln.weight), _p(ln.bias), float(eps), _p(out), _stream())
    return out


def adamw_step(master: torch.Tensor, m: torch.Tensor, v: torch.Tensor, grad: torch.Tensor, param_out: Optional[torch.Tensor], lr: float,
               beta1: float, beta2: float, eps: float, weight_decay: float, step: int, grad_scale: float = 1.0) -> None:
    for t, n in ((master, "master"), (m, "m"), (v, "v")):
        _chk(t, n, torch.float32)
    if not grad.is_cuda or grad.dtype not in DT_CODE or not grad.is_contiguous() or grad.numel() != master.numel():
        raise RuntimeError("u-llava_amd.adamw_step: grad must be a contiguous GPU tensor of the shard's size (fp32 / bf16 / fp16)")
    pd = 0
    if param_out is not None:
        if not param_out.is_cuda or param_out.dtype not in DT_CODE or not param_out.is_contiguous() or param_out.numel() != master.numel():
            raise RuntimeError("u-llava_amd.adamw_step: param_out must be a contiguous GPU tensor of the shard's size")
        pd = DT_CODE[param_out.dtype]
    _lib.call("ull_adamw_step_f32", _p(master), _p(m), _p(v), _p(grad), DT_CODE[grad.dtype], _p(param_out), pd, master.numel(), float(lr), float(beta1),
              float(beta2), float(eps), float(weight_decay), int(step), float(grad_scale), _stream())


def sumsq(g: torch.Tensor, out: torch.Tensor) -> None:
    _chk(out, "out", torch.float32)
    if not g.is_cuda or g.dtype not in DT_CODE or not g.is_contiguous():
        raise RuntimeError("u-llava_amd.sumsq: contiguous GPU tensor (fp32 / bf16 / fp16) required")
    if g.numel():
        _lib.call("ull_sumsq_f32", _p(g), DT_CODE[g.dtype], g.numel(), _p(out), _stream())


COARSE = [True]


class per_op_layers:
    def __init__(self, on: bool = True):
        self.on = on

    def __enter__(self):
        self.prev = COARSE[0]
        COARSE[0] = not self.on
        return self

    def __exit__(self, *exc):
        COARSE[0] = self.prev
        return False


def coarse_ok() -> bool:
    return COARSE[0] and not _SMALL_M_SPLIT_K[0]


class LayerStack:

    def __init__(self, kind, layers):
        self.kind, self.layers = kind, layers
        self.arr = (kind * len(layers))()
        lin = [(d, n) for d in layers for n, t in kind._fields_ if t is _lib.Linear]
        self._w16 = [(d, n) for d, n in lin if not isinstance(d[n][0] if type(d[n]) is tuple else d[n], QuantWeight)]
        self.quantized = len(self._w16) < len(lin)
        self._seen = None
        self.refresh()

    def _fingerprint(self):
        fp = []
        for d, n in self._w16:
            w = d[n]
            if type(w) is tuple:
                w = w[0]
            fp += (w.data_ptr(), w._version)
        return fp

    @staticmethod
    def _linear(v):
        w, b = v if type(v) is tuple else (v, None)
        if isinstance(w, QuantWeight):
            wf, q, ldq, scales, lds = w.c_args()
            return _lib.Linear(q, None, None, w.shape[0], w.shape[1], ldq, wf, scales, lds)
        if w.dim() != 2 or w.stride(1) != 1:
            raise RuntimeError("u-llava_amd: coarse entries need row-major 2-D weights")
        wt = _tiled_of(w)
        return _lib.Linear(w.data_ptr(), None if wt is None else wt.data_ptr(), _p(b), w.shape[0], w.shape[1], w.stride(0))

    def refresh(self):
        fp = self._fingerprint()
        if fp == self._seen:
            return self.arr
        for i, d in enumerate(self.layers):
            s = self.arr[i]
            for n, t in self.kind._fields_:
                v = d[n]
                if t is _lib.Linear:
                    setattr(s, n, self._linear(v))
                elif isinstance(v, int):
                    setattr(s, n, v)
                else:
                    setattr(s, n, v.data_ptr())
        self._seen = fp
        return self.arr


def _sk_args(device):
    min_k = _SK_MIN_K[0]
    if min_k is None:
        return None, 0, -1
    ws = _streamk_ws(device, _stream())
    return ws.data_ptr(), ws.numel(), int(min_k)


def _ptr_array(tensors):
    import ctypes
    return (ctypes.c_void_p * len(tensors))(*[t.data_ptr() for t in tensors])


def llama_prefill_layers(stack: LayerStack, x_in: torch.Tensor, x_out, rope_cos, rope_sin, key_mask, B: int, S: int, H: int, hd: int, I: int,
                         eps: float):
    _chk(x_in, "x_in")
    T, D = x_in.shape
    dev, dt = x_in.device, x_in.dtype
    x_mid = torch.empty(T, D, device=dev, dtype=dt)
    xn = torch.empty(T, D, device=dev, dtype=dt)
    qkv = torch.empty(T, 3 * D, device=dev, dtype=dt)
    att = torch.empty(T, D, device=dev, dtype=dt)
    act = torch.empty(T, I, device=dev, dtype=dt)
    ws, wsb, mk = _sk_args(dev)
    _lib.call("ull_llama_prefill_layers_" + _SFX[dt], stack.refresh(), len(stack.layers), _p(x_in), _ptr_array(x_out), _p(x_mid), _p(xn), _p(qkv), _p(att),
              _p(act), _p(rope_cos), _p(rope_sin), _p(key_mask), B, S, H, hd, I, float(eps), ws, wsb, mk, _zeros(dev).data_ptr(), _stream())


def llama_decode_layers(stack: LayerStack, x_in: torch.Tensor, x_out, rope_cos, rope_sin, key_mask, k_ptrs, vt_ptrs, B: int, S: int, H: int, hd: int,
                        I: int, smax: int, past: int, eps: float, kv8=None):
    _chk(x_in, "x_in", BF16 if (stack.quantized or kv8 is not None) else None)
    T, D = x_in.shape
    dev, dt = x_in.device, x_in.dtype
    scratch = torch.empty(T * (4 * D + 2 * max(D, I)), device=dev, dtype=dt)
    x_mid, q, att = scratch[:T * D], scratch[T * D:2 * T * D], scratch[2 * T * D:3 * T * D]
    xn = scratch[3 * T * D:3 * T * D + T * max(D, I)]
    act = scratch[3 * T * D + T * max(D, I):3 * T * D + T * max(D, I) + T * I]
    if kv8 is not None:
        k8, vt8, ks, vs, k_stage, vt_stage = kv8
        _lib.call("ull_llama_decode_layers_kv8_bf16", stack.refresh(), len(stack.layers), _p(x_in), _ptr_array(x_out),
                  _p(x_mid), _p(xn), _p(q), _p(att), _p(act), _p(rope_cos), _p(rope_sin), _p(key_mask), k8, vt8, ks, vs, _p(k_stage), _p(vt_stage),
                  B, S, H, hd, I, smax, past, float(eps), _zeros(dev).data_ptr(), _stream())
        return
    _lib.call("ull_llama_decode_layers_" + _SFX[dt], stack.refresh(), len(stack.layers), _p(x_in), _ptr_array(x_out), _p(x_mid),
              _p(xn), _p(q), _p(att), _p(act), _p(rope_cos), _p(rope_sin), _p(key_mask), k_ptrs, vt_ptrs, B, S, H, hd, I, smax, past, float(eps),
              _zeros(dev).data_ptr(), _stream())


def clip_layers(stack: LayerStack, n_layers: int, h: torch.Tensor, n_img: int, S: int, H: int, hd: int, I: int, eps: float):
    _chk(h, "h")
    T, D = h.shape
    dev, dt = h.device, h.dtype
    h_mid = torch.empty(T, D, device=dev, dtype=dt)
    y = torch.empty(T, D, device=dev, dtype=dt)
    qkv = torch.empty(T, 3 * D, device=dev, dtype=dt)
    att = torch.empty(T, D, device=dev, dtype=dt)
    f = torch.empty(T, I, device=dev, dtype=dt)
    ws, wsb, mk = _sk_args(dev)
    _lib.call("ull_clip_layers_" + _SFX[dt], stack.refresh(), n_layers, _p(h), _p(h_mid), _p(y), _p(qkv), _p(att), _p(f), n_img, S, H, hd, I, float(eps),
              ws, wsb, mk, _zeros(dev).data_ptr(), _stream())


def sam_blocks(stack: LayerStack, x: torch.Tensor, B: int, g: int, nH: int, hd: int, I: int, eps: float = 1e-6):
    _chk(x, "x")
    T, C = x.shape
    dev, dt = x.device, x.dtype
    x_mid = torch.empty(T, C, device=dev, dtype=dt)
    y = torch.empty(T, C, device=dev, dtype=dt)
    qkv = torch.empty(T, 3 * C, device=dev, dtype=dt)
    att = torch.empty(T, C, device=dev, dtype=dt)
    f = torch.empty(T, I, device=dev, dtype=dt)
    ws, wsb, mk = _sk_args(dev)
    _lib.call("ull_sam_blocks_" + _SFX[dt], stack.refresh(), len(stack.layers), _p(x), _p(x_mid), _p(y), _p(qkv), _p(att), _p(f), B, g, nH, hd, I, float(eps),
              ws, wsb, mk, _zeros(dev).data_ptr(), _stream())
```

Measured before the change: 141.3 images/sec (whole job, all GPUs).

## Write RMSNorm and SwiGLU outputs in tile-major layout for LLaMA prefill GEMMs

The LLaMA prefill layers now have RMSNorm write its output directly in the 256x64 tile-major layout the big GEMM reads via X_TILED. The gate/up SwiGLU GEMM writes its activation in the same tiled layout (new C_TILED epilogue flag), so the down projection can consume it as tiled input. The intent is cheaper, more contiguous A-operand loads in the 256-tile GEMMs, with no extra layout-conversion pass. It adds padded scratch buffers and a shared tile256 predicate, and C_TILED is restricted to the waves4 direct path, which errors if dispatch picks otherwise.

```diff
diff --git a/include/ullava_hip.h b/include/ullava_hip.h
--- a/include/ullava_hip.h
+++ b/include/ullava_hip.h
@@ -24,6 +24,7 @@
 #define ULL_EPI_OUT_F32 32
 #define ULL_EPI_W_TILED 64
 #define ULL_EPI_X_TILED 128
+#define ULL_EPI_C_TILED 1024
 #define ULL_EPI_BIAS_ROUNDED 256
 
 #define ULL_GEMM_TUNE_GROUP_M(g) (((g) & 15) << 16)
@@ -40,6 +41,8 @@
 
 int ull_rope_table_bf16(const void* positions, const void* inv_freq, int64_t tokens, int64_t half, void* cos_out, void* sin_out,
                         void* stream);
+
+int ull_gemm_tile256(int64_t M, int64_t N, int64_t K, int flags);
 
 int64_t ull_gemm_streamk_ws_bytes(void);
 
@@ -93,6 +96,7 @@
                             int64_t n, void* K_out, int64_t k_pitch, void* Vt_out, int64_t vt_pitch, void* stream);
 
 int ull_rmsnorm_bf16(const void* x, int64_t ldx, const void* w, void* y, int64_t ldy, int64_t rows, int64_t D, float eps, void* stream);
+int ull_rmsnorm_tiled_bf16(const void* x, int64_t ldx, const void* w, void* y, int64_t rows, int64_t D, float eps, void* stream);
 
 int ull_shifted_cross_entropy_bf16(const void* logits, int64_t ld, const void* labels, int64_t B, int64_t S, int64_t V, void* out,
                                    void* stream);
@@ -344,6 +348,7 @@
 int ull_gemv_rmsnorm_f16(const void* X, int64_t ldx, const void* norm_w, float eps, const void* W, int64_t ldw, void* C, int64_t ldc, const void* bias, const void* R, int64_t ldr, int64_t M, int64_t N, int64_t K, int flags, void* stream);
 int ull_gemv_qkv_rope_append_f16(const void* X, int64_t ldx, const void* norm_w, float eps, const void* W, int64_t ldw, void* Q_out, int64_t ldq, const void* cos_tab, const void* sin_tab, void* k_cache, void* vt_cache, int64_t B, int64_t S, int64_t H, int64_t hd, int64_t K, int64_t smax, int64_t past, void* stream);
 int ull_rmsnorm_f16(const void* x, int64_t ldx, const void* w, void* y, int64_t ldy, int64_t rows, int64_t D, float eps, void* stream);
+int ull_rmsnorm_tiled_f16(const void* x, int64_t ldx, const void* w, void* y, int64_t rows, int64_t D, float eps, void* stream);
 int ull_shifted_cross_entropy_f16(const void* logits, int64_t ld, const void* labels, int64_t B, int64_t S, int64_t V, void* out, void* stream);
 int ull_layernorm_f16(const void* x, int64_t ldx, const void* w, const void* b, void* y, int64_t ldy, int64_t rows, int64_t D, float eps, void* stream);
 int ull_clip_embed_ln_f16(const void* patch, int64_t ldp, const void* cls, const void* pos, const void* w, const void* b, void* y, int64_t ldy, int64_t n_img, int64_t tokens, int64_t D, float eps, void* stream);
diff --git a/u-llava_amd/_lib.py b/u-llava_amd/_lib.py
--- a/u-llava_amd/_lib.py
+++ b/u-llava_amd/_lib.py
@@ -30,6 +30,7 @@
 SIGNATURES = {
     "ull_gemm_bf16": [_ptr, _i64, _ptr, _i64, _ptr, _i64, _ptr, _ptr, _i64, _i64, _i64, _i64, _i32, _ptr, _i64, _ptr],
     "ull_gemm_streamk_ws_bytes": [],
+    "ull_gemm_tile256": [_i64, _i64, _i64, _i32],
     "ull_gemm_qkv_rope_bf16": [_ptr, _i64, _ptr, _i64, _ptr, _i64, _i64, _i64, _i64, _ptr, _ptr, _i64, _i64, _i32, _ptr, _i64, _ptr],
     "ull_rope_table_bf16": [_ptr, _ptr, _i64, _i64, _ptr, _ptr, _ptr],
     "ull_sam_self_attn_heads_bf16": [_ptr, _ptr, _i64, _i64, _i32] + [_ptr] * 7 + [_ptr],
@@ -67,6 +68,7 @@
     "ull_gemv_qkv_rope_append_bf16": [_ptr, _i64, _ptr, _f32, _ptr, _i64, _ptr, _i64, _ptr, _ptr, _ptr, _ptr, _i64, _i64, _i64, _i64, _i64, _i64, _i64,
                                       _ptr],
     "ull_rmsnorm_bf16": [_ptr, _i64, _ptr, _ptr, _i64, _i64, _i64, _f32, _ptr],
+    "ull_rmsnorm_tiled_bf16": [_ptr, _i64, _ptr, _ptr, _i64, _i64, _f32, _ptr],
     "ull_llama_prefill_layers_bf16": [_ptr, _i64, _ptr, _ptr, _ptr, _ptr, _ptr, _ptr, _ptr, _ptr, _ptr, _ptr, _i64, _i64, _i64, _i64, _i64, _f32, _ptr,
                                       _i64, _i64, _ptr, _ptr],
     "ull_llama_decode_layers_bf16": [_ptr, _i64, _ptr, _ptr, _ptr, _ptr, _ptr, _ptr, _ptr, _ptr, _ptr, _ptr, _ptr, _ptr, _i64, _i64, _i64, _i64, _i64,
@@ -137,7 +139,7 @@
 
 SIGNATURES["ull_neck_layernorm2d_f32in_f16"] = [_ptr, _ptr, _f32, _ptr, _ptr, _ptr, _ptr, _i64, _i64, _f32, _ptr]
 
-VALUE_RETURNING = {"ull_gemm_streamk_ws_bytes": _i64}
+VALUE_RETURNING = {"ull_gemm_streamk_ws_bytes": _i64, "ull_gemm_tile256": _i32}
 
 ERRORS = {-1: "ULL_ERR_ARG (null pointer / bad size)", -2: "ULL_ERR_SHAPE (alignment or shape constraint)",
           -3: "ULL_ERR_LAUNCH (HIP launch failed)", -4: "ULL_ERR_LDS (does not fit the LDS budget)"}
diff --git a/u-llava_amd/csrc/f32.hip b/u-llava_amd/csrc/f32.hip
--- a/u-llava_amd/csrc/f32.hip
+++ b/u-llava_amd/csrc/f32.hip
@@ -9,6 +9,7 @@
 #define ULL_EPI_SWIGLU 16
 #define ULL_EPI_W_TILED 64
 #define ULL_EPI_X_TILED 128
+#define ULL_EPI_C_TILED 1024
 
 namespace {
 
@@ -502,7 +503,7 @@
     (void)ws; (void)ws_bytes;
     if (!X || !W || !C || M <= 0 || N <= 0 || K <= 0) return ULL_ERR_ARG;
     if (((flags & ULL_EPI_BIAS) && !bias) || ((flags & ULL_EPI_RESID) && !R)) return ULL_ERR_ARG;
-    if (flags & (ULL_EPI_W_TILED | ULL_EPI_X_TILED)) return ULL_ERR_SHAPE;
+    if (flags & (ULL_EPI_W_TILED | ULL_EPI_X_TILED | ULL_EPI_C_TILED)) return ULL_ERR_SHAPE;
     if ((flags & ULL_EPI_SWIGLU) && (N % 32)) return ULL_ERR_SHAPE;
     hipLaunchKernelGGL(gemm_f32_kernel, dim3((unsigned)((N + 63) / 64), (unsigned)((M + 63) / 64)), dim3(256), 0, ST, (const float*)X, (long)ldx,
                        (const float*)W, (long)ldw, (float*)C, (long)ldc, (const float*)bias, (flags & ULL_EPI_RESID) ? (const float*)R : nullptr, (long)ldr,
diff --git a/u-llava_amd/csrc/gemm.hip b/u-llava_amd/csrc/gemm.hip
--- a/u-llava_amd/csrc/gemm.hip
+++ b/u-llava_amd/csrc/gemm.hip
@@ -13,6 +13,7 @@
 constexpr int EPI_BIAS = 1, EPI_ACT_SHIFT = 1, EPI_ACT_MASK = 3 << 1;
 constexpr int EPI_RESID = 8, EPI_SWIGLU = 16, EPI_OUT_F32 = 32;
 constexpr int EPI_W_TILED = 64, EPI_X_TILED = 128;
+constexpr int EPI_C_TILED = 1024;
 constexpr int EPI_BIAS_ROUNDED = 256;
 constexpr int ULL_W4_FORCE_STAGED = 512;
 
@@ -853,7 +854,10 @@
     const int fr = lane & 15, fg = lane >> 4;
     if constexpr (SWIGLU) {
         const int n_out = p.N / 2, nb = nw0 / 2 + 8 * fg;
-        elem_t* cb = (elem_t*)p.C + nb;
+        const bool c_tiled = p.flags & EPI_C_TILED;
+        const long ldc = c_tiled ? 64 : p.ldc;
+        elem_t* cb = c_tiled ? (elem_t*)p.C + ((long)(mrow0 >> 8) * (n_out >> 6) + (nb >> 6)) * 16384 - (long)(mrow0 & ~255) * 64 + (nb & 63)
+                             : (elem_t*)p.C + nb;
 #pragma clang loop unroll(full)
         for (int j = 0; j < 8; ++j) {
             const int m = mrow0 + j * 16 + fr;
@@ -870,7 +874,7 @@
                         v[4 * pp + r] = rnd(act_silu(g)) * u;
                     }
                 }
-                if (m < p.M && nb + h * 32 + 8 <= n_out) *(uint4*)(cb + (long)m * p.ldc + h * 32) = pack8(v);
+                if (m < p.M && nb + h * 32 + 8 <= n_out) *(uint4*)(cb + (long)m * ldc + h * 32) = pack8(v);
             }
             __builtin_amdgcn_sched_barrier(0);
         }
@@ -1578,6 +1582,8 @@
             float t = v[r];
             if (flags & EPI_RESID) t = rnd(e2f(p.R[(long)m * p.ldr + n + r]) + t);
             if (out_f32) ((float*)p.C)[(long)m * p.ldc + n + r] = t;
+            else if (flags & EPI_C_TILED)
+                ((elem_t*)p.C)[((long)(m >> 8) * (n_out_total >> 6) + ((n + r) >> 6)) * 16384 + (m & 255) * 64 + ((n + r) & 63)] = f2e(t);
             else ((elem_t*)p.C)[(long)m * p.ldc + n + r] = f2e(t);
         }
     }
@@ -1622,6 +1628,15 @@
 extern "C" int64_t ull_gemm_streamk_ws_bytes(void) { return (int64_t)256 * big::BM * big::BN * sizeof(float); }
 #endif
 
+#ifndef ULL_ELEM_F16
+extern "C" int ull_gemm_tile256(int64_t M, int64_t N, int64_t K, int flags) {
+    const bool short_and_few = K <= 768 && ((M + 255) / 256) * ((N + 255) / 256) < 512 && !(flags & (EPI_W_TILED | EPI_X_TILED | EPI_C_TILED));
+    return !(flags & (1 << 20)) && !short_and_few && M >= 1024 && N >= 512 && K >= 128;
+}
+#else
+extern "C" int ull_gemm_tile256(int64_t M, int64_t N, int64_t K, int flags);
+#endif
+
 static int gemm_dispatch(const void* X, int64_t ldx, const void* W, int64_t ldw, void* C, int64_t ldc, const void* bias, const void* R,
                          int64_t ldr, int64_t M, int64_t N, int64_t K, int flags, void* ws, int64_t ws_bytes, void* stream,
                          const elem_t* rope_cos, const elem_t* rope_sin, int rope_cols) {
@@ -1635,10 +1650,12 @@
     if (const int rc = gemm_device_state(&n_cu)) return rc;
     const int tune_group_m = (flags >> 16) & 15;
     const bool force_small = flags & (1 << 20);
+    const bool tile256 = ull_gemm_tile256(M, N, K, flags);
     const bool force_waves8 = flags & (1 << 21);
     const bool force_waves4 = (flags & (1 << 22)) && ldx < (1 << 21) && ldw < (1 << 21);
     flags &= 0xffff;
     if ((flags & EPI_BIAS_ROUNDED) && (flags & EPI_SWIGLU)) return ULL_ERR_SHAPE;
+    if ((flags & EPI_C_TILED) && (!(flags & EPI_SWIGLU) || (N & 127) || ((uintptr_t)C & 15))) return ULL_ERR_SHAPE;
     GemmArgs a;
     a.X = (const elem_t*)X; a.W = (const elem_t*)W; a.C = C;
     a.bias = (const elem_t*)bias; a.R = (const elem_t*)R;
@@ -1646,8 +1663,7 @@
     a.M = (int)M; a.N = (int)N; a.K = (int)K; a.flags = flags;
     a.rope_cos = rope_cos; a.rope_sin = rope_sin; a.rope_cols = rope_cols;
     const bool rope = rope_cos != nullptr;
-    const bool short_and_few = K <= 768 && ((M + 255) / 256) * ((N + 255) / 256) < 512 && !(flags & (EPI_W_TILED | EPI_X_TILED));
-    if (!force_small && !short_and_few && M >= 1024 && N >= 512 && K >= 128) {
+    if (tile256) {
         a.nbm = (int)((M + big::BM - 1) / big::BM); a.nbn = (int)((N + big::BN - 1) / big::BN);
         constexpr long SLAB = (long)big::BM * big::BN * sizeof(float);
         const int max_slabs = ws ? (int)(ws_bytes / SLAB < 4096 ? ws_bytes / SLAB : 4096) : 0;
@@ -1674,6 +1690,7 @@
         const bool waves4 = force_waves4 || (!force_waves8 && fits32 && (direct || (K >= 3072 && c_rows_aligned)));
         const bool waves8_direct = !force_waves4 && !force_waves8 && direct && !rope && !(flags & EPI_SWIGLU) && (flags & EPI_ACT_MASK) &&
                                    ((flags & EPI_ACT_MASK) >> EPI_ACT_SHIFT) != 3 && K < 3072;
+        if ((flags & EPI_C_TILED) && !(waves4 && direct)) return ULL_ERR_SHAPE;
         if (waves8_direct) {
             hipLaunchKernelGGL(big::gemm256d_kernel, dim3(grid), dim3(512), big::LDS_BYTES_W4, (hipStream_t)stream, a);
         } else if (waves4) {
@@ -1692,7 +1709,7 @@
         if (a.sk > 1) hipLaunchKernelGGL((big::splitk_finalize_any_kernel<big::BM, big::BN, false>), dim3(32, rem), dim3(256), 0, (hipStream_t)stream, a);
         return ull_check_launch();
     }
-    if (flags & (EPI_W_TILED | EPI_X_TILED)) return ULL_ERR_SHAPE;
+    if (flags & (EPI_W_TILED | EPI_X_TILED | EPI_C_TILED)) return ULL_ERR_SHAPE;
     a.nbm = (int)((M + BM - 1) / BM); a.nbn = (int)((N + BN - 1) / BN);
     a.t_full = 0; a.sk = 1; a.ws = nullptr; a.group_m = GROUP_M;
     const int T = a.nbm * a.nbn, nk = (int)(K / BK), slots = 2 * n_cu;
diff --git a/u-llava_amd/csrc/layers.hip b/u-llava_amd/csrc/layers.hip
--- a/u-llava_amd/csrc/layers.hip
+++ b/u-llava_amd/csrc/layers.hip
@@ -30,7 +30,7 @@
     int64_t wsb;
 };
 inline Tiled tiled(const ull_linear* L, int64_t M, const SK& sk) {
-    const bool big = M >= 1024 && L->n >= 512 && L->k >= 128;
+    const bool big = ull_gemm_tile256(M, L->n, L->k, ULL_EPI_W_TILED);
     Tiled t{L->w, L->ldw, 0, nullptr, 0};
     if (big && L->w_tiled) { t.w = L->w_tiled; t.ldw = L->k; t.flags = ULL_EPI_W_TILED; }
     if (big && sk.min_k >= 0 && L->k >= sk.min_k) { t.ws = sk.ws; t.wsb = sk.bytes; }
@@ -43,6 +43,10 @@
     if (L->bias) flags |= ULL_EPI_BIAS;
     if (R) flags |= ULL_EPI_RESID;
     return FN(ull_gemm_)(x, ldx, t.w, t.ldw, out, ldc, L->bias, R, ldr, M, L->n, L->k, flags | t.flags, t.ws, t.wsb, stream);
+}
+
+inline int norm(const void* x, const void* w, void* y, int64_t rows, int64_t D, float eps, int x_tiled, void* stream) {
+    return x_tiled ? FN(ull_rmsnorm_tiled_)(x, D, w, y, rows, D, eps, stream) : FN(ull_rmsnorm_)(x, D, w, y, D, rows, D, eps, stream);
 }
 
 inline bool quantized(const ull_linear* L) { return L->format != ULL_WF_ELEM; }
@@ -122,22 +126,24 @@
     const float scale = 1.0f / sqrtf((float)hd);
     const char* q = (const char*)qkv;
     const void* x = x_in;
+    const auto x_tiled = [&](const ull_linear* L) { return ull_gemm_tile256(T, L->n, L->k, tiled(L, T, sk).flags) ? ULL_EPI_X_TILED : 0; };
     for (int64_t l = 0; l < n_layers; ++l) {
         const ull_llama_layer& w = layers[l];
         if (w.qkv.n != 3 * D || w.qkv.k != D || w.o.n != D || w.o.k != D || w.gu.n != 2 * I || w.gu.k != D || w.down.n != D || w.down.k != I || !x_out[l] ||
             quantized(&w.qkv) || quantized(&w.o) || quantized(&w.gu) || quantized(&w.down))
             return ULL_ERR_ARG;
-        TRY(FN(ull_rmsnorm_)(x, D, w.ln1, xn, D, T, D, eps, stream));
+        const int xt_qkv = x_tiled(&w.qkv), xt_gu = x_tiled(&w.gu), xt_down = xt_gu ? x_tiled(&w.down) : 0;
+        TRY(norm(x, w.ln1, xn, T, D, eps, xt_qkv, stream));
         {
             const Tiled t = tiled(&w.qkv, T, sk);
-            TRY(FN(ull_gemm_qkv_rope_)(xn, D, t.w, t.ldw, qkv, 3 * D, T, 3 * D, D, rope_cos, rope_sin, 2 * D, hd, t.flags, t.ws, t.wsb, stream));
+            TRY(FN(ull_gemm_qkv_rope_)(xn, D, t.w, t.ldw, qkv, 3 * D, T, 3 * D, D, rope_cos, rope_sin, 2 * D, hd, t.flags | xt_qkv, t.ws, t.wsb, stream));
         }
         TRY(FN(ull_attention_)(q, S * 3 * D, hd, 3 * D, q + D * 2, S * 3 * D, hd, 3 * D, q + 2 * D * 2, S * 3 * D, hd, 3 * D, 0, att, S * D, hd, D, key_mask,
                                B, H, S, S, hd, 1, 1, scale, 1.0f, nullptr, nullptr, 0, 0, 0, zeros, stream));
         TRY(lin(att, D, &w.o, x_mid, D, x, D, T, 0, sk, stream));
-        TRY(FN(ull_rmsnorm_)(x_mid, D, w.ln2, xn, D, T, D, eps, stream));
-        TRY(lin(xn, D, &w.gu, act, I, nullptr, 0, T, ULL_EPI_SWIGLU, sk, stream));
-        TRY(lin(act, I, &w.down, x_out[l], D, x_mid, D, T, 0, sk, stream));
+        TRY(norm(x_mid, w.ln2, xn, T, D, eps, xt_gu, stream));
+        TRY(lin(xn, D, &w.gu, act, I, nullptr, 0, T, ULL_EPI_SWIGLU | xt_gu | (xt_down ? ULL_EPI_C_TILED : 0), sk, stream));
+        TRY(lin(act, I, &w.down, x_out[l], D, x_mid, D, T, xt_down, sk, stream));
         x = x_out[l];
     }
     return ULL_OK;
diff --git a/u-llava_amd/csrc/norm.hip b/u-llava_amd/csrc/norm.hip
--- a/u-llava_amd/csrc/norm.hip
+++ b/u-llava_amd/csrc/norm.hip
@@ -2,7 +2,7 @@
 
 namespace {
 
-template <int NCH, int MODE>
+template <int NCH, int MODE, bool TILED = false>
 __global__ __launch_bounds__(256) void rownorm_kernel(const elem_t* __restrict__ x, long ldx, const elem_t* __restrict__ w,
                                                       const elem_t* __restrict__ b, elem_t* __restrict__ y, long ldy,
                                                       long rows, int D, float eps, int lpr,
@@ -64,7 +64,7 @@
         rstd = 1.0f / sqrtf(q * invD + eps);
     }
     if (!row_ok) return;
-    elem_t* yr = y + row * ldy;
+    elem_t* yr = TILED ? y + (row >> 8) * (256L * D) + (row & 255) * 64 : y + row * ldy;
 #pragma unroll
     for (int i = 0; i < NCH; ++i) {
         const int c = sub + i * lpr;
@@ -80,22 +80,24 @@
 #pragma unroll
                 for (int j = 0; j < 8; ++j) o[j] = ((v[i][j] - mean) * rstd) * wv[j] + bv[j];
             }
-            *(uint4*)(yr + c * 8) = pack8(o);
+            if (TILED) *(uint4*)(yr + (c >> 3) * 16384 + (c & 7) * 8) = pack8(o);
+            else *(uint4*)(yr + c * 8) = pack8(o);
         }
     }
 }
 
-template <int MODE>
+template <int MODE, bool TILED = false>
 int launch_rownorm(const elem_t* x, long ldx, const elem_t* w, const elem_t* b, elem_t* y, long ldy, long rows, int D, float eps,
                    const elem_t* cls, const elem_t* pos, int tokens, hipStream_t st) {
     if (D <= 0 || (D & 7) || (ldx & 7) || (ldy & 7) || rows <= 0) return ULL_ERR_SHAPE;
+    if (TILED && (D & 63)) return ULL_ERR_SHAPE;
     const int nchunk = D >> 3;
     int lpr = 1;
     while (lpr < 64 && lpr < nchunk) lpr <<= 1;
     const int nch = (nchunk + lpr - 1) / lpr;
     const long rows_per_block = 4 * (64 / lpr);
     const dim3 grid((unsigned)((rows + rows_per_block - 1) / rows_per_block));
-#define ULL_RN(N) hipLaunchKernelGGL((rownorm_kernel<N, MODE>), grid, dim3(256), 0, st, x, ldx, w, b, y, ldy, rows, D, eps, lpr, cls, pos, tokens)
+#define ULL_RN(N) hipLaunchKernelGGL((rownorm_kernel<N, MODE, TILED>), grid, dim3(256), 0, st, x, ldx, w, b, y, ldy, rows, D, eps, lpr, cls, pos, tokens)
     if (nch <= 1) ULL_RN(1);
     else if (nch <= 2) ULL_RN(2);
     else if (nch <= 4) ULL_RN(4);
@@ -113,6 +115,13 @@
     if (!x || !w || !y) return ULL_ERR_ARG;
     return launch_rownorm<0>((const elem_t*)x, ldx, (const elem_t*)w, nullptr, (elem_t*)y, ldy, rows, (int)D, eps, nullptr, nullptr, 0,
                              (hipStream_t)stream);
+}
+
+extern "C" int ULL_FN(ull_rmsnorm_tiled_)(const void* x, int64_t ldx, const void* w, void* y, int64_t rows, int64_t D, float eps, void* stream) {
+    if (!x || !w || !y) return ULL_ERR_ARG;
+    if (((uintptr_t)y & 15)) return ULL_ERR_SHAPE;
+    return launch_rownorm<0, true>((const elem_t*)x, ldx, (const elem_t*)w, nullptr, (elem_t*)y, 0, rows, (int)D, eps, nullptr, nullptr, 0,
+                                   (hipStream_t)stream);
 }
 
 extern "C" int ULL_FN(ull_layernorm_)(const void* x, int64_t ldx, const void* w, const void* b, void* y, int64_t ldy, int64_t rows, int64_t D,
diff --git a/u-llava_amd/ops.py b/u-llava_amd/ops.py
--- a/u-llava_amd/ops.py
+++ b/u-llava_amd/ops.py
@@ -74,6 +74,8 @@
 
 
 EPI_W_TILED = 64
+EPI_X_TILED = 128
+EPI_C_TILED = 1024
 _TILED = {}
 
 
@@ -1327,10 +1329,11 @@
     T, D = x_in.shape
     dev, dt = x_in.device, x_in.dtype
     x_mid = torch.empty(T, D, device=dev, dtype=dt)
-    xn = torch.empty(T, D, device=dev, dtype=dt)
     qkv = torch.empty(T, 3 * D, device=dev, dtype=dt)
     att = torch.empty(T, D, device=dev, dtype=dt)
-    act = torch.empty(T, I, device=dev, dtype=dt)
+    Tp = (T + 255) // 256 * 256
+    xn = torch.empty(Tp, D, device=dev, dtype=dt)
+    act = torch.empty(Tp, I, device=dev, dtype=dt)
     ws, wsb, mk = _sk_args(dev)
     _lib.call("ull_llama_prefill_layers_" + _SFX[dt], stack.refresh(), len(stack.layers), _p(x_in), _ptr_array(x_out), _p(x_mid), _p(xn), _p(qkv), _p(att),
               _p(act), _p(rope_cos), _p(rope_sin), _p(key_mask), B, S, H, hd, I, float(eps), ws, wsb, mk, _zeros(dev).data_ptr(), _stream())
```

Measured after the change: 141.5 images/sec (whole job, all GPUs) (median of 6 runs). No clear change (+0.2%).
